# tudocomp/tudocomp

Hardware: AMD Instinct MI355X
Metric: input MB/s end-to-end lcpcomp+huffman (higher is better)
Workload: dtype u32

## Files before the change

include/tdc_gpu.h:

```cpp
#ifndef TDC_GPU_H
#define TDC_GPU_H

#include <stddef.h>
#include <stdint.h>

#ifdef __cplusplus
extern "C" {
#endif

typedef enum {
    TDC_GPU_OK = 0,
    TDC_GPU_ERR_HIP = -1,
    TDC_GPU_ERR_ARG = -2,
    TDC_GPU_ERR_NO_SENTINEL = -3,
    TDC_GPU_ERR_TOO_LARGE = -4,
    TDC_GPU_ERR_OOM = -5,
    TDC_GPU_ERR_UNSUPPORTED = -6,
    TDC_GPU_ERR_INTERNAL = -7
} tdc_gpu_status;

enum { TDC_GPU_CODER_HUFF = 0, TDC_GPU_CODER_GAMMA = 1, TDC_GPU_CODER_ARITH = 2, TDC_GPU_CODER_ASCII = 3, TDC_GPU_CODER_SLE = 4,
       TDC_GPU_CODER_BIT = 5 , TDC_GPU_CODER_DELTA = 6  };
#define TDC_GPU_CODER_SLE_K(K) (TDC_GPU_CODER_SLE | ((K) << 8))
enum { TDC_GPU_COMP_ARRAYS = 0, TDC_GPU_COMP_PLCPPEAKS = 1, TDC_GPU_COMP_MAXLCP = 2, TDC_GPU_COMP_HEAP = 3 };
// ... 45 lines not shown
    uint32_t rebuilds;
    float ms_round_first, ms_round_last, ms_round_tie;
    float reserved1;
} tdc_gpu_stats;

int  tdc_gpu_ctx_create(int device, tdc_gpu_ctx** ctx);
void tdc_gpu_ctx_destroy(tdc_gpu_ctx* ctx);
int tdc_gpu_ctx_set_option(tdc_gpu_ctx* ctx, const char* name, long value);
int tdc_gpu_option_count(void);
const char* tdc_gpu_option_name(int i);
int  tdc_gpu_ctx_reserve(tdc_gpu_ctx* ctx, size_t n);
size_t tdc_gpu_arena_bytes(size_t n);
int  tdc_gpu_device_memory(int device, size_t* free_bytes, size_t* total_bytes);
int  tdc_gpu_ctx_set_profiling(tdc_gpu_ctx* ctx, int enabled);
void tdc_gpu_ctx_reset_profile(tdc_gpu_ctx* ctx);
const char* tdc_gpu_ctx_kernel_profile(const tdc_gpu_ctx* ctx, int idx, double* ms, uint64_t* launches, uint64_t* bytes);
const char* tdc_gpu_strerror(int status);
const char* tdc_gpu_last_error(const tdc_gpu_ctx* ctx);
void tdc_gpu_free(void* p);

int tdc_gpu_lcpcomp_compress(tdc_gpu_ctx* ctx, const uint8_t* text, size_t n, uint32_t threshold, int flatten,
                             int coder, uint8_t** out, size_t* out_len, tdc_gpu_stats* stats);
int tdc_gpu_lcpcomp_compress_comp(tdc_gpu_ctx* ctx, const uint8_t* text, size_t n, uint32_t threshold, int flatten, int coder,
                                  int comp, uint8_t** out, size_t* out_len, tdc_gpu_stats* stats);

int tdc_gpu_lcpcomp_compress_into(tdc_gpu_ctx* ctx, const uint8_t* text, size_t n, uint32_t threshold, int flatten, int coder,
                                  int comp, uint8_t* out, size_t out_cap, size_t* out_len, tdc_gpu_stats* stats);
int tdc_gpu_lcpcomp_compress_keep(tdc_gpu_ctx* ctx, const uint8_t* text, size_t n, uint32_t threshold, int flatten, int coder,
                                  int comp, size_t* out_len, tdc_gpu_stats* stats);
int tdc_gpu_stream_fetch(tdc_gpu_ctx* ctx, uint8_t* dst, size_t cap, size_t* len);
int tdc_gpu_stream_fetch_dev(tdc_gpu_ctx* ctx, void* d_dst, size_t cap, size_t* len);
int tdc_gpu_host_register(void* p, size_t bytes);
int tdc_gpu_host_unregister(void* p);
void* tdc_gpu_host_alloc(size_t bytes);
void  tdc_gpu_host_free(void* p);

int tdc_gpu_lcpcomp_compress_raw(tdc_gpu_ctx* ctx, const uint8_t* data, size_t n, uint32_t threshold, int flatten,
                                 int coder, uint8_t** out, size_t* out_len, tdc_gpu_stats* stats);
int tdc_gpu_lcpcomp_compress_dev(tdc_gpu_ctx* ctx, const void* d_text, size_t n, uint32_t threshold, int flatten,
                                 int coder, void* d_out, size_t out_cap, size_t* out_len, tdc_gpu_stats* stats);
size_t tdc_gpu_lcpcomp_bound(size_t n);
size_t tdc_gpu_lcpcomp_bound_coder(size_t n, int coder);

size_t tdc_gpu_blocks_count(size_t n, size_t block_size);
int tdc_gpu_blocks_compress(const int* devices, int ndev, const uint8_t* data, size_t n, size_t block_size, uint32_t threshold,
                            int flatten, int coder, uint8_t** out, size_t* out_len, tdc_gpu_stats* per_block);
int tdc_gpu_blocks_decompress(tdc_gpu_ctx* ctx, const uint8_t* container, size_t len, int coder, uint8_t** out, size_t* out_len);
int tdc_gpu_device_count(void);

int tdc_gpu_lz78_compress(tdc_gpu_ctx* ctx, const uint8_t* in, size_t n, int coder, uint8_t** out, size_t* out_len,
                          tdc_gpu_stats* stats);

int tdc_gpu_lzss_lcp_compress(tdc_gpu_ctx* ctx, const uint8_t* text, size_t n, uint32_t threshold, int coder,
                              uint8_t** out, size_t* out_len, tdc_gpu_stats* stats);
int tdc_gpu_lzss_lcp_compress_into(tdc_gpu_ctx* ctx, const uint8_t* text, size_t n, uint32_t threshold, int coder,
                                   uint8_t* out, size_t out_cap, size_t* out_len, tdc_gpu_stats* stats);
size_t tdc_gpu_lzss_lcp_bound(size_t n, int coder);
int tdc_gpu_lzss_lcp_decompress(tdc_gpu_ctx* ctx, const uint8_t* stream, size_t len, int coder, uint8_t** out, size_t* out_len,
                                uint64_t* factors, uint32_t* rounds);
int tdc_gpu_lzss_lcp_decompress_into(tdc_gpu_ctx* ctx, const uint8_t* stream, size_t len, int coder, uint8_t* out, size_t out_cap,
                                     size_t* out_len, uint64_t* factors, uint32_t* rounds);
int tdc_gpu_lzss_lcp_factorize(tdc_gpu_ctx* ctx, const uint8_t* text, size_t n, uint32_t threshold,
                               uint32_t** pos, uint32_t** src, uint32_t** len, size_t* z);

int tdc_gpu_sort_pairs_u64(tdc_gpu_ctx* ctx, uint64_t* keys, uint32_t* vals, size_t n, int algo);
int tdc_gpu_suffix_array(tdc_gpu_ctx* ctx, const uint8_t* text, size_t n, uint32_t* sa, uint32_t* isa);
int tdc_gpu_textds(tdc_gpu_ctx* ctx, const uint8_t* text, size_t n, uint32_t* sa, uint32_t* isa, uint32_t* phi,
                   uint32_t* plcp, uint32_t* lcp, uint32_t* maxlcp);
int tdc_gpu_lcpcomp_factorize(tdc_gpu_ctx* ctx, const uint8_t* text, size_t n, uint32_t threshold, int flatten,
                              uint32_t** pos, uint32_t** src, uint32_t** len, size_t* z, tdc_gpu_stats* stats);
int tdc_gpu_flatten(tdc_gpu_ctx* ctx, size_t n, const uint32_t* pos, uint32_t* src, const uint32_t* len, size_t z,
                    uint64_t* num_flattened, uint64_t* max_depth_lb);
int tdc_gpu_prim_scan(tdc_gpu_ctx* ctx, int op, void* data, size_t n, int in_place, void* total);
int tdc_gpu_prim_sort_pairs(tdc_gpu_ctx* ctx, int kind, void* keys, uint32_t* vals, size_t n, int begin_bit, int end_bit);
int tdc_gpu_prim_bucketed_scatter(tdc_gpu_ctx* ctx, const uint32_t* idx, const uint32_t* val, size_t m, uint32_t* dst, size_t n_dst,
                                  uint32_t fill, int permutation, int second_tmp, int offset);
int tdc_gpu_prim_msd_partition(tdc_gpu_ctx* ctx, uint32_t* idx, uint32_t* val, size_t m, int bits, int db);
int tdc_gpu_prim_select(tdc_gpu_ctx* ctx, const uint8_t* cls, uint8_t want, size_t m, const uint32_t* srcA, const uint64_t* srcB,
                        uint32_t fillA, uint64_t fillB, uint32_t* outA, uint64_t* outB, uint32_t* count);
int tdc_gpu_prim_select_counts(tdc_gpu_ctx* ctx, const uint8_t* cls, uint8_t want, size_t m, const uint32_t* srcA, const uint32_t* tile_counts,
                               uint32_t fillA, uint32_t* outA, uint32_t* count);
int tdc_gpu_prim_mark_orbit(tdc_gpu_ctx* ctx, const uint32_t* next, size_t n, uint8_t* mark);
int tdc_gpu_prim_tile_entries(tdc_gpu_ctx* ctx, const uint16_t* exit0, size_t ntiles, uint32_t states, uint16_t* entry0);
int tdc_gpu_prim_arena_fill(tdc_gpu_ctx* ctx, int byte, uint64_t* base, uint64_t* size);

int tdc_gpu_lcpcomp_decompress(tdc_gpu_ctx* ctx, const uint8_t* stream, size_t len, uint8_t** out, size_t* out_len,
                               uint64_t* factors, uint32_t* rounds);
int tdc_gpu_lcpcomp_decompress_coder(tdc_gpu_ctx* ctx, const uint8_t* stream, size_t len, int coder, uint8_t** out, size_t* out_len,
                                     uint64_t* factors, uint32_t* rounds);
int tdc_gpu_lcpcomp_decompress_into(tdc_gpu_ctx* ctx, const uint8_t* stream, size_t len, int coder, uint8_t* out, size_t out_cap,
                                    size_t* out_len, uint64_t* factors, uint32_t* rounds);
int tdc_gpu_ctx_last_decode_on_device(const tdc_gpu_ctx* ctx);

int tdc_gpu_lz78_decompress(tdc_gpu_ctx* ctx, const uint8_t* stream, size_t len, int coder, uint8_t** out, size_t* out_len,
                            uint64_t* phrases, uint32_t* rounds);
int tdc_gpu_lz78_decompress_into(tdc_gpu_ctx* ctx, const uint8_t* stream, size_t len, int coder, uint8_t* out, size_t out_cap,
                                 size_t* out_len, uint64_t* phrases, uint32_t* rounds);

int tdc_gpu_lzw_compress(tdc_gpu_ctx* ctx, const uint8_t* in, size_t n, int coder, uint8_t** out, size_t* out_len,
                         tdc_gpu_stats* stats);
int tdc_gpu_lzw_decompress(tdc_gpu_ctx* ctx, const uint8_t* stream, size_t len, int coder, uint8_t** out, size_t* out_len,
                           uint64_t* codes, uint32_t* rounds);
int tdc_gpu_lzw_decompress_into(tdc_gpu_ctx* ctx, const uint8_t* stream, size_t len, int coder, uint8_t* out, size_t out_cap,
                                size_t* out_len, uint64_t* codes, uint32_t* rounds);

int tdc_gpu_lzss_sw_compress(tdc_gpu_ctx* ctx, const uint8_t* in, size_t n, uint32_t window, uint32_t threshold, int coder,
                             uint8_t** out, size_t* out_len, tdc_gpu_stats* stats);
int tdc_gpu_lzss_sw_compress_into(tdc_gpu_ctx* ctx, const uint8_t* in, size_t n, uint32_t window, uint32_t threshold, int coder,
                                  uint8_t* out, size_t out_cap, size_t* out_len, tdc_gpu_stats* stats);
size_t tdc_gpu_lzss_sw_bound(size_t n, uint32_t window, int coder);
int tdc_gpu_lzss_sw_factorize(tdc_gpu_ctx* ctx, const uint8_t* in, size_t n, uint32_t window, uint32_t threshold,
                              uint32_t** pos, uint32_t** src, uint32_t** len, size_t* z);
int tdc_gpu_lzss_sw_decompress(tdc_gpu_ctx* ctx, const uint8_t* stream, size_t len, int coder, uint32_t window,
                               uint8_t** out, size_t* out_len, uint64_t* factors, uint32_t* rounds);
int tdc_gpu_lzss_sw_decompress_into(tdc_gpu_ctx* ctx, const uint8_t* stream, size_t len, int coder, uint32_t window,
                                    uint8_t* out, size_t out_cap, size_t* out_len, uint64_t* factors, uint32_t* rounds);

int tdc_gpu_lzss_sw_compress_batch(tdc_gpu_ctx* ctx, const uint8_t* in, const uint64_t* in_off, size_t count,
                                   uint32_t window, uint32_t threshold, int coder,
                                   uint8_t* out, size_t out_cap, uint64_t* out_off , uint64_t* out_len ,
                                   int32_t* status , tdc_gpu_stats* stats);
size_t tdc_gpu_lzss_sw_batch_bound(const uint64_t* in_off, size_t count, uint32_t window, int coder);
int tdc_gpu_lzss_sw_decompress_batch(tdc_gpu_ctx* ctx, const uint8_t* streams, const uint64_t* s_off, const uint64_t* s_len,
                                     size_t count, int coder, uint32_t window,
                                     uint8_t* out, size_t out_cap, uint64_t* out_off ,
                                     int32_t* status , tdc_gpu_stats* stats);

int tdc_gpu_lzw_compress_batch(tdc_gpu_ctx* ctx, const uint8_t* in, const uint64_t* in_off, size_t count, int coder,
                               uint8_t* out, size_t out_cap, uint64_t* out_off , uint64_t* out_len ,
                               int32_t* status , tdc_gpu_stats* stats);
int tdc_gpu_lz78_compress_batch(tdc_gpu_ctx* ctx, const uint8_t* in, const uint64_t* in_off, size_t count, int coder,
                                uint8_t* out, size_t out_cap, uint64_t* out_off , uint64_t* out_len ,
                                int32_t* status , tdc_gpu_stats* stats);
size_t tdc_gpu_lzw_batch_bound(const uint64_t* in_off, size_t count, int coder);
size_t tdc_gpu_lz78_batch_bound(const uint64_t* in_off, size_t count, int coder);
int tdc_gpu_lz_parse_batch(tdc_gpu_ctx* ctx, const uint8_t* in, const uint64_t* in_off, size_t count, int lzw,
                           uint32_t* items , uint8_t* chars , uint64_t* item_off , int32_t* status );

int tdc_gpu_lzw_decompress_batch(tdc_gpu_ctx* ctx, const uint8_t* streams, const uint64_t* s_off, const uint64_t* s_len,
                                 size_t count, int coder, uint8_t* out, size_t out_cap, uint64_t* out_off ,
                                 int32_t* status , tdc_gpu_stats* stats);
int tdc_gpu_lz78_decompress_batch(tdc_gpu_ctx* ctx, const uint8_t* streams, const uint64_t* s_off, const uint64_t* s_len,
                                  size_t count, int coder, uint8_t* out, size_t out_cap, uint64_t* out_off ,
                                  int32_t* status , tdc_gpu_stats* stats);

int tdc_gpu_repair_compress(tdc_gpu_ctx* ctx, const uint8_t* in, size_t n, uint64_t max_rules, int coder, uint8_t** out, size_t* out_len,
                            tdc_gpu_stats* stats);
int tdc_gpu_repair_compress_into(tdc_gpu_ctx* ctx, const uint8_t* in, size_t n, uint64_t max_rules, int coder, uint8_t* out, size_t out_cap,
                                 size_t* out_len, tdc_gpu_stats* stats);
size_t tdc_gpu_repair_bound(size_t n, int coder);
int tdc_gpu_repair_grammar(tdc_gpu_ctx* ctx, const uint8_t* in, size_t n, uint64_t max_rules, uint64_t** rules, size_t* nrules,
                           uint32_t** start, size_t* nstart, tdc_gpu_stats* stats);
int tdc_gpu_repair_compress_batch(tdc_gpu_ctx* ctx, const uint8_t* in, const uint64_t* in_off, size_t count, uint64_t max_rules, int coder,
                                  uint8_t* out, size_t out_cap, uint64_t* out_off , uint64_t* out_len ,
                                  int32_t* status , tdc_gpu_stats* stats);
size_t tdc_gpu_repair_batch_bound(const uint64_t* in_off, size_t count, int coder);
int tdc_gpu_repair_grammar_batch(tdc_gpu_ctx* ctx, const uint8_t* in, const uint64_t* in_off, size_t count, uint64_t max_rules,
                                 uint64_t* rules , uint64_t* rule_off ,
                                 uint32_t* start , uint64_t* start_off , int32_t* status );

int tdc_gpu_repair_decompress(tdc_gpu_ctx* ctx, const uint8_t* stream, size_t len, int coder, uint8_t** out, size_t* out_len);
int tdc_gpu_repair_decompress_into(tdc_gpu_ctx* ctx, const uint8_t* stream, size_t len, int coder, uint8_t* out, size_t out_cap, size_t* out_len);
int tdc_gpu_repair_decompress_stats(tdc_gpu_ctx* ctx, const uint8_t* stream, size_t len, int coder, uint8_t* out, size_t out_cap, size_t* out_len,
                                    tdc_gpu_stats* stats);
int tdc_gpu_repair_decompress_batch(tdc_gpu_ctx* ctx, const uint8_t* streams, const uint64_t* s_off, const uint64_t* s_len,
                                    size_t count, int coder, uint8_t* out, size_t out_cap, uint64_t* out_off ,
// ... 77 lines not shown
```

tudocomp_amd/__init__.py:

```python
import ctypes

import numpy as np

from . import _native
from ._native import Stats, Stage, LIB_PATH, SYMBOLS

CODER_HUFF = 0
CODER_GAMMA = 1
CODER_ARITH = 2
CODER_ASCII = 3
CODER_SLE = 4
CODER_BIT = 5
CODER_DELTA = 6
COMP_ARRAYS = 0
COMP_PLCPPEAKS = 1
COMP_MAXLCP = 2
COMP_HEAP = 3
STAGE_BWT = 0
STAGE_RLE = 1
STAGE_MTF = 2
STAGE_HUFF = 3
STAGE_SLE = 4


# ... 786 lines not shown
        v = np.ascontiguousarray(vals, dtype=np.uint32).copy()
        self._check(self._L.tdc_gpu_sort_pairs_u64(self._h, _ptr(k), _ptr(v), len(k), int(algo)))
        return k, v

    _SCAN_OPS = {"sum_u32": (0, np.uint32), "sum_u64": (1, np.uint64), "max_u32": (2, np.uint32)}
    _SORT_KINDS = {"u32": (0, np.uint32), "u64": (1, np.uint64), "distinct": (2, np.uint64)}

    def prim_scan(self, op, data, in_place=False, want_total=True):
        code, dt = self._SCAN_OPS[op]
        a = np.ascontiguousarray(data, dtype=dt).copy()
        tot = np.zeros(1, dtype=dt) if want_total and code != 2 else None
        self._check(self._L.tdc_gpu_prim_scan(self._h, code, _ptr(a), len(a), int(bool(in_place)), _ptr(tot) if tot is not None else None))
        return a, (int(tot[0]) if tot is not None else None)

    def prim_sort_pairs(self, kind, keys, vals, begin_bit, end_bit):
        code, dt = self._SORT_KINDS[kind]
        k = np.ascontiguousarray(keys, dtype=dt).copy()
        v = np.ascontiguousarray(vals, dtype=np.uint32).copy()
        if len(k) != len(v):
            raise ValueError("keys and vals differ in length")
        self._check(self._L.tdc_gpu_prim_sort_pairs(self._h, code, _ptr(k), _ptr(v), len(k), int(begin_bit), int(end_bit)))
        return k, v

    def prim_bucketed_scatter(self, idx, val, n_dst, fill=0xFFFFFFFF, permutation=False, second_tmp=True, offset=0):
        i = np.ascontiguousarray(idx, dtype=np.uint32)
        v = np.ascontiguousarray(val, dtype=np.uint32)
        if len(i) != len(v):
            raise ValueError("idx and val differ in length")
        dst = np.empty(int(n_dst), dtype=np.uint32)
        self._check(self._L.tdc_gpu_prim_bucketed_scatter(self._h, _ptr(i), _ptr(v), len(i), _ptr(dst), int(n_dst), int(fill),
                                                          int(bool(permutation)), int(bool(second_tmp)), int(offset)))
        return dst

    def prim_msd_partition(self, idx, val, bits, db):
        i = np.ascontiguousarray(idx, dtype=np.uint32).copy()
        v = np.ascontiguousarray(val, dtype=np.uint32).copy()
        if len(i) != len(v):
            raise ValueError("idx and val differ in length")
        self._check(self._L.tdc_gpu_prim_msd_partition(self._h, _ptr(i), _ptr(v), len(i), int(bits), int(db)))
        return i, v

    def prim_select(self, cls, want, src_a=None, src_b=None, fill_a=0xFFFFFFFF, fill_b=0xFFFFFFFFFFFFFFFF):
        c = np.ascontiguousarray(cls, dtype=np.uint8)
        m = len(c)
        a = None if src_a is None else np.ascontiguousarray(src_a, dtype=np.uint32)
        b = None if src_b is None else np.ascontiguousarray(src_b, dtype=np.uint64)
        if (a is not None and len(a) != m) or (b is not None and len(b) != m):
            raise ValueError("cls, src_a and src_b differ in length")
        oa = np.empty(m, dtype=np.uint32)
        ob = None if b is None else np.empty(m, dtype=np.uint64)
        cnt = ctypes.c_uint32(0)
        self._check(self._L.tdc_gpu_prim_select(self._h, _ptr(c), int(want), m, None if a is None else _ptr(a), None if b is None else _ptr(b),
                                                int(fill_a), int(fill_b), _ptr(oa), None if ob is None else _ptr(ob), ctypes.byref(cnt)))
        return oa, ob, cnt.value

    def prim_select_counts(self, cls, want, tile_counts, src_a=None, fill_a=0xFFFFFFFF):
        c = np.ascontiguousarray(cls, dtype=np.uint8)
        m = len(c)
        t = np.ascontiguousarray(tile_counts, dtype=np.uint32)
        if len(t) != (m + 2047) // 2048:
            raise ValueError("one count per tile of 2048 classes")
        a = None if src_a is None else np.ascontiguousarray(src_a, dtype=np.uint32)
        if a is not None and len(a) != m:
            raise ValueError("cls and src_a differ in length")
        oa = np.empty(m, dtype=np.uint32)
        cnt = ctypes.c_uint32(0)
        self._check(self._L.tdc_gpu_prim_select_counts(self._h, _ptr(c), int(want), m, None if a is None else _ptr(a), _ptr(t),
                                                       int(fill_a), _ptr(oa), ctypes.byref(cnt)))
        return oa, cnt.value

    def prim_mark_orbit(self, nxt):
        a = np.ascontiguousarray(nxt, dtype=np.uint32)
        mark = np.empty(len(a), dtype=np.uint8)
        self._check(self._L.tdc_gpu_prim_mark_orbit(self._h, _ptr(a), len(a), _ptr(mark)))
        return mark

    def prim_tile_entries(self, exits):
        a = np.ascontiguousarray(exits, dtype=np.uint16)
        ntiles, states = a.shape
        entry = np.empty(ntiles, dtype=np.uint16)
        self._check(self._L.tdc_gpu_prim_tile_entries(self._h, _ptr(a), ntiles, states, _ptr(entry)))
        return entry

    def prim_arena_fill(self, byte=None):
        base, size = ctypes.c_uint64(), ctypes.c_uint64()
        self._check(self._L.tdc_gpu_prim_arena_fill(self._h, -1 if byte is None else int(byte), ctypes.byref(base), ctypes.byref(size)))
        return base.value, size.value

    def suffix_array(self, text):
        a = _u8(text)
        sa = np.empty(len(a), dtype=np.uint32)
        isa = np.empty(len(a), dtype=np.uint32)
        self._check(self._L.tdc_gpu_suffix_array(self._h, _ptr(a), len(a), _ptr(sa), _ptr(isa)))
        return sa, isa

    def textds(self, text):
        a = _u8(text)
        n = len(a)
        arrs = {k: np.empty(n, dtype=np.uint32) for k in ("sa", "isa", "phi", "plcp", "lcp")}
        m = ctypes.c_uint32()
        self._check(self._L.tdc_gpu_textds(self._h, _ptr(a), n, _ptr(arrs["sa"]), _ptr(arrs["isa"]), _ptr(arrs["phi"]),
                                           _ptr(arrs["plcp"]), _ptr(arrs["lcp"]), ctypes.byref(m)))
        arrs["maxlcp"] = m.value
        return arrs

    def lcpcomp_decompress(self, stream, coder=CODER_HUFF):
        a = _u8(stream)
        p, n = ctypes.c_void_p(), ctypes.c_size_t()
        f, r = ctypes.c_uint64(), ctypes.c_uint32()
        self._check(self._L.tdc_gpu_lcpcomp_decompress_coder(self._h, _ptr(a), len(a), coder, ctypes.byref(p), ctypes.byref(n),
                                                             ctypes.byref(f), ctypes.byref(r)))
        return self._take(p, n.value), {"factors": f.value, "rounds": r.value,
                                        "device_parse": int(self._L.tdc_gpu_ctx_last_decode_on_device(self._h))}

    def lcpcomp_decompress_into(self, stream, out, coder=CODER_HUFF):
        a = stream.a if isinstance(stream, PinnedBuffer) else _u8(stream)
        oa = out.a if isinstance(out, PinnedBuffer) else out
        n = ctypes.c_size_t()
        f, r = ctypes.c_uint64(), ctypes.c_uint32()
        self._check(self._L.tdc_gpu_lcpcomp_decompress_into(self._h, _ptr(a), len(a), coder, _ptr(oa), oa.size, ctypes.byref(n),
                                                            ctypes.byref(f), ctypes.byref(r)))
        return n.value, {"factors": f.value, "rounds": r.value, "device_parse": int(self._L.tdc_gpu_ctx_last_decode_on_device(self._h))}

    def lz78_decompress(self, stream, coder=CODER_GAMMA):
        a = stream.a if isinstance(stream, PinnedBuffer) else _u8(stream)
        p, n = ctypes.c_void_p(), ctypes.c_size_t()
        f, r = ctypes.c_uint64(), ctypes.c_uint32()
        self._check(self._L.tdc_gpu_lz78_decompress(self._h, _ptr(a), len(a), coder, ctypes.byref(p), ctypes.byref(n),
                                                    ctypes.byref(f), ctypes.byref(r)))
        return self._take(p, n.value), {"phrases": f.value, "rounds": r.value}

    def lz78_decompress_into(self, stream, out, coder=CODER_GAMMA):
        a = stream.a if isinstance(stream, PinnedBuffer) else _u8(stream)
        oa = out.a if isinstance(out, PinnedBuffer) else out
        n = ctypes.c_size_t()
        f, r = ctypes.c_uint64(), ctypes.c_uint32()
        rc = self._L.tdc_gpu_lz78_decompress_into(self._h, _ptr(a), len(a), coder, _ptr(oa), oa.size, ctypes.byref(n),
                                                  ctypes.byref(f), ctypes.byref(r))
        if rc:
            err = TdcGpuError(rc, self._L.tdc_gpu_last_error(self._h).decode())
            err.required = n.value if rc == -5 else None
            raise err
        return n.value, {"phrases": f.value, "rounds": r.value}

    def lzw_decompress(self, stream, coder=CODER_BIT):
        a = stream.a if isinstance(stream, PinnedBuffer) else _u8(stream)
        p, n = ctypes.c_void_p(), ctypes.c_size_t()
        f, r = ctypes.c_uint64(), ctypes.c_uint32()
        self._check(self._L.tdc_gpu_lzw_decompress(self._h, _ptr(a) if len(a) else None, len(a), coder, ctypes.byref(p), ctypes.byref(n),
                                                   ctypes.byref(f), ctypes.byref(r)))
        return self._take(p, n.value), {"codes": f.value, "rounds": r.value,
                                        "device_parse": int(self._L.tdc_gpu_ctx_last_decode_on_device(self._h))}

    def lzw_decompress_into(self, stream, out, coder=CODER_BIT):
        a = stream.a if isinstance(stream, PinnedBuffer) else _u8(stream)
        oa = out.a if isinstance(out, PinnedBuffer) else out
        n = ctypes.c_size_t()
        f, r = ctypes.c_uint64(), ctypes.c_uint32()
        rc = self._L.tdc_gpu_lzw_decompress_into(self._h, _ptr(a) if len(a) else None, len(a), coder, _ptr(oa), oa.size, ctypes.byref(n),
                                                 ctypes.byref(f), ctypes.byref(r))
        if rc:
            self._raise_required(rc, n.value)
        return n.value, {"codes": f.value, "rounds": r.value, "device_parse": int(self._L.tdc_gpu_ctx_last_decode_on_device(self._h))}

    def _raise_required(self, rc, n):
        err = TdcGpuError(rc, self._L.tdc_gpu_last_error(self._h).decode())
# ... 517 lines not shown
```

tudocomp_amd/_native.py:

```python
import ctypes
import os

_HERE = os.path.dirname(os.path.abspath(__file__))
LIB_PATH = os.environ.get("TDC_GPU_LIB") or os.path.join(_HERE, "lib", "libtdc_gpu.so")

SYMBOLS = [
    "tdc_gpu_ctx_create", "tdc_gpu_ctx_destroy", "tdc_gpu_ctx_reserve", "tdc_gpu_strerror", "tdc_gpu_last_error",
    "tdc_gpu_ctx_set_profiling", "tdc_gpu_ctx_reset_profile", "tdc_gpu_ctx_kernel_profile",
    "tdc_gpu_free", "tdc_gpu_lcpcomp_compress", "tdc_gpu_lcpcomp_compress_raw", "tdc_gpu_lcpcomp_compress_dev",
    "tdc_gpu_lcpcomp_bound", "tdc_gpu_lcpcomp_bound_coder", "tdc_gpu_lcpcomp_compress_into", "tdc_gpu_host_alloc", "tdc_gpu_host_free",
    "tdc_gpu_lz78_compress", "tdc_gpu_lzss_lcp_compress", "tdc_gpu_lzss_lcp_factorize",
    "tdc_gpu_sort_pairs_u64", "tdc_gpu_suffix_array", "tdc_gpu_textds", "tdc_gpu_lcpcomp_factorize", "tdc_gpu_flatten", "tdc_gpu_encode_huff",
    "tdc_gpu_prim_scan", "tdc_gpu_prim_sort_pairs", "tdc_gpu_prim_bucketed_scatter", "tdc_gpu_prim_msd_partition", "tdc_gpu_prim_select", "tdc_gpu_prim_select_counts",
    "tdc_gpu_prim_mark_orbit", "tdc_gpu_prim_tile_entries", "tdc_gpu_prim_arena_fill",
    "tdc_gpu_lcpcomp_decompress",
    "tdc_gpu_lcpcomp_compress_comp",
    "tdc_gpu_encode_arith",
    "tdc_gpu_encode_ascii",
    "tdc_gpu_encode_sle",
    "tdc_gpu_lcpcomp_decompress_coder", "tdc_gpu_ctx_last_decode_on_device", "tdc_gpu_lcpcomp_decompress_into",
    "tdc_gpu_ctx_set_option", "tdc_gpu_option_count", "tdc_gpu_option_name", "tdc_escape", "tdc_unescape", "tdc_lz78_factors", "tdc_huffman_table", "tdc_huffman_selfcheck", "tdc_gpu_blocks_count", "tdc_gpu_blocks_compress", "tdc_gpu_blocks_decompress", "tdc_gpu_device_count", "tdc_gen_english", "tdc_gen_dna",
    "tdc_gpu_arena_bytes", "tdc_gpu_device_memory",
    "tdc_gpu_lcpcomp_compress_keep", "tdc_gpu_stream_fetch", "tdc_gpu_stream_fetch_dev", "tdc_gpu_host_register", "tdc_gpu_host_unregister",
    "tdc_gpu_lz78_decompress", "tdc_gpu_lz78_decompress_into",
    "tdc_gpu_bwt_compress", "tdc_gpu_bwt_compress_into", "tdc_gpu_bwt_decompress", "tdc_gpu_bwt_decompress_into", "tdc_gpu_bwt_inverse_stage",
    "tdc_gpu_pipeline_bound", "tdc_gpu_pipeline_compress", "tdc_gpu_pipeline_compress_into", "tdc_gpu_pipeline_compress_batch", "tdc_gpu_pipeline_batch_bound", "tdc_gpu_pipeline_decompress",
    "tdc_gpu_pipeline_decompress_into", "tdc_gpu_pipeline_decompress_stats", "tdc_rle_decode", "tdc_mtf_decode", "tdc_huff_decode_literals", "tdc_sle_decode",
    "tdc_gpu_lzw_compress", "tdc_gpu_lzw_decompress", "tdc_gpu_lzw_decompress_into", "tdc_lzw_factors", "tdc_lzw_decode",
    "tdc_gpu_lzss_lcp_compress_into", "tdc_gpu_lzss_lcp_bound", "tdc_gpu_lzss_lcp_decompress", "tdc_gpu_lzss_lcp_decompress_into", "tdc_lzss_decode",
    "tdc_gpu_lzss_sw_compress", "tdc_gpu_lzss_sw_compress_into", "tdc_gpu_lzss_sw_bound", "tdc_gpu_lzss_sw_factorize", "tdc_lzss_sw_factors",
    "tdc_lzss_sw_decode", "tdc_gpu_lzss_sw_decompress", "tdc_gpu_lzss_sw_decompress_into",
    "tdc_gpu_lzss_sw_compress_batch", "tdc_gpu_lzss_sw_batch_bound", "tdc_gpu_lzss_sw_decompress_batch",
    "tdc_gpu_lzw_compress_batch", "tdc_gpu_lzw_batch_bound", "tdc_gpu_lz78_compress_batch", "tdc_gpu_lz78_batch_bound", "tdc_gpu_lz_parse_batch",
    "tdc_gpu_lzw_decompress_batch", "tdc_gpu_lz78_decompress_batch",
    "tdc_gpu_repair_compress", "tdc_gpu_repair_compress_into", "tdc_gpu_repair_bound", "tdc_gpu_repair_grammar", "tdc_gpu_repair_decompress",
    "tdc_gpu_repair_decompress_into", "tdc_gpu_repair_decompress_stats", "tdc_repair_grammar", "tdc_repair_decode",
    "tdc_gpu_repair_compress_batch", "tdc_gpu_repair_batch_bound", "tdc_gpu_repair_grammar_batch", "tdc_gpu_repair_decompress_batch",
    "tdc_gpu_bwt_compress_batch", "tdc_gpu_bwt_decompress_batch", "tdc_gpu_suffix_array_batch",
]


class Stats(ctypes.Structure):
    _fields_ = (
        [(k, ctypes.c_uint64) for k in ("n", "out_len", "factors", "maxlcp", "entries", "num_flattened", "max_depth_lb",
                                        "flen_min", "flen_max", "fdist_max", "pushes")] +
        [(k, ctypes.c_uint32) for k in ("sa_rounds", "sa_init_syms", "levels", "mis_rounds", "flatten_rounds", "sigma")] +
        [(k, ctypes.c_uint64) for k in ("sa_sorted_elems", "arena_bytes")] +
        [(k, ctypes.c_float) for k in ("ms_h2d", "ms_sa", "ms_phi", "ms_plcp", "ms_factorize", "ms_flatten", "ms_encode",
                                       "ms_d2h", "ms_total")] +
        [(k, ctypes.c_uint32) for k in ("small_levels", "purges", "window_pass", "window_lcut",
                                        "sa_key_words", "sa_text_rounds", "sa_mode", "sa_overlapped", "eager_levels", "eager_phases", "sa_star_chains",
                                        "probes", "max_push_targets")] +
        [("d2h_early", ctypes.c_uint64)] +
        [("pipe_stages", ctypes.c_uint32), ("pipe_dev", ctypes.c_uint32), ("pipe_len", ctypes.c_uint64 * 8), ("pipe_ms", ctypes.c_float * 8),
         ("ranges_early", ctypes.c_uint32), ("len_rounds", ctypes.c_uint32),
         ("rules", ctypes.c_uint64), ("replaced", ctypes.c_uint64), ("tie_rounds", ctypes.c_uint32), ("rebuilds", ctypes.c_uint32),
         ("ms_round_first", ctypes.c_float), ("ms_round_last", ctypes.c_float), ("ms_round_tie", ctypes.c_float), ("reserved1", ctypes.c_float)])

    def as_dict(self):
        d = {k: getattr(self, k) for k, _ in self._fields_}
        d["pipe_len"] = list(self.pipe_len)[:self.pipe_stages]
        d["pipe_ms"] = list(self.pipe_ms)[:self.pipe_stages]
        return d


class Stage(ctypes.Structure):
    _fields_ = [("kind", ctypes.c_int), ("param", ctypes.c_uint64)]


_lib = None


def load():
    global _lib
    if _lib is not None:
        return _lib
    if not os.path.exists(LIB_PATH):
        raise RuntimeError("tudocomp_amd: %s is missing -- build it with `make -C tudocomp_amd/csrc` "
                           "(there is no CPU fallback)" % LIB_PATH)
    L = ctypes.CDLL(LIB_PATH)
    vp, sz, u32, i32 = ctypes.c_void_p, ctypes.c_size_t, ctypes.c_uint32, ctypes.c_int
    pvp, psz = ctypes.POINTER(vp), ctypes.POINTER(sz)
    L.tdc_gpu_ctx_create.argtypes = [i32, pvp]
    L.tdc_gpu_ctx_destroy.argtypes = [vp]
    L.tdc_gpu_ctx_destroy.restype = None
    L.tdc_gpu_ctx_reserve.argtypes = [vp, sz]
    L.tdc_gpu_ctx_set_profiling.argtypes = [vp, i32]
    L.tdc_gpu_ctx_reset_profile.argtypes = [vp]
    L.tdc_gpu_ctx_reset_profile.restype = None
    L.tdc_gpu_ctx_kernel_profile.argtypes = [vp, i32, ctypes.POINTER(ctypes.c_double), ctypes.POINTER(ctypes.c_uint64),
                                             ctypes.POINTER(ctypes.c_uint64)]
    L.tdc_gpu_ctx_kernel_profile.restype = ctypes.c_char_p
    L.tdc_gpu_strerror.argtypes = [i32]
    L.tdc_gpu_strerror.restype = ctypes.c_char_p
    L.tdc_gpu_last_error.argtypes = [vp]
    L.tdc_gpu_last_error.restype = ctypes.c_char_p
    L.tdc_gpu_free.argtypes = [vp]
    L.tdc_gpu_free.restype = None
    L.tdc_gpu_lcpcomp_compress.argtypes = [vp, vp, sz, u32, i32, i32, pvp, psz, ctypes.POINTER(Stats)]
    L.tdc_gpu_lcpcomp_compress_comp.argtypes = [vp, vp, sz, u32, i32, i32, i32, pvp, psz, ctypes.POINTER(Stats)]
    L.tdc_gpu_lcpcomp_compress_raw.argtypes = [vp, vp, sz, u32, i32, i32, pvp, psz, ctypes.POINTER(Stats)]
    L.tdc_gpu_lcpcomp_compress_dev.argtypes = [vp, vp, sz, u32, i32, i32, vp, sz, psz, ctypes.POINTER(Stats)]
    L.tdc_gpu_lz78_compress.argtypes = [vp, vp, sz, i32, pvp, psz, ctypes.POINTER(Stats)]
    L.tdc_gpu_lzss_lcp_compress.argtypes = [vp, vp, sz, u32, i32, pvp, psz, ctypes.POINTER(Stats)]
    L.tdc_gpu_lzss_lcp_compress_into.argtypes = [vp, vp, sz, u32, i32, vp, sz, psz, ctypes.POINTER(Stats)]
    L.tdc_gpu_lzss_lcp_bound.argtypes = [sz, i32]
    L.tdc_gpu_lzss_lcp_bound.restype = sz
    L.tdc_gpu_lzss_lcp_decompress.argtypes = [vp, vp, sz, i32, pvp, psz, ctypes.POINTER(ctypes.c_uint64), ctypes.POINTER(ctypes.c_uint32)]
    L.tdc_gpu_lzss_lcp_decompress_into.argtypes = [vp, vp, sz, i32, vp, sz, psz, ctypes.POINTER(ctypes.c_uint64), ctypes.POINTER(ctypes.c_uint32)]
    L.tdc_lzss_decode.argtypes = [vp, sz, i32, vp, sz, psz]
    L.tdc_gpu_lzss_lcp_factorize.argtypes = [vp, vp, sz, u32, pvp, pvp, pvp, psz]
    L.tdc_gpu_arena_bytes.argtypes = [sz]
    L.tdc_gpu_arena_bytes.restype = sz
    L.tdc_gpu_device_memory.argtypes = [i32, psz, psz]
    L.tdc_gpu_lcpcomp_bound.argtypes = [sz]
    L.tdc_gpu_lcpcomp_bound.restype = sz
    L.tdc_gpu_lcpcomp_bound_coder.argtypes = [sz, i32]
    L.tdc_gpu_lcpcomp_bound_coder.restype = sz
    L.tdc_gpu_lcpcomp_compress_into.argtypes = [vp, vp, sz, u32, i32, i32, i32, vp, sz, psz, ctypes.POINTER(Stats)]
    L.tdc_gpu_lcpcomp_compress_keep.argtypes = [vp, vp, sz, u32, i32, i32, i32, psz, ctypes.POINTER(Stats)]
    L.tdc_gpu_stream_fetch.argtypes = [vp, vp, sz, psz]
    L.tdc_gpu_stream_fetch_dev.argtypes = [vp, vp, sz, psz]
    L.tdc_gpu_ctx_last_decode_on_device.argtypes = [vp]
    L.tdc_gpu_lcpcomp_decompress_into.argtypes = [vp, vp, sz, i32, vp, sz, psz, ctypes.POINTER(ctypes.c_uint64), ctypes.POINTER(ctypes.c_uint32)]
    L.tdc_gpu_host_register.argtypes = [vp, sz]
    L.tdc_gpu_host_unregister.argtypes = [vp]
    L.tdc_gpu_blocks_count.argtypes = [sz, sz]
    L.tdc_gpu_blocks_count.restype = sz
    L.tdc_gpu_blocks_compress.argtypes = [ctypes.POINTER(i32), i32, vp, sz, sz, u32, i32, i32, pvp, psz, ctypes.POINTER(Stats)]
    L.tdc_gpu_blocks_decompress.argtypes = [vp, vp, sz, i32, pvp, psz]
    L.tdc_gpu_host_alloc.argtypes = [sz]
    L.tdc_gpu_host_alloc.restype = vp
    L.tdc_gpu_host_free.argtypes = [vp]
    L.tdc_gpu_host_free.restype = None
    L.tdc_gpu_sort_pairs_u64.argtypes = [vp, vp, vp, sz, i32]
    L.tdc_gpu_prim_scan.argtypes = [vp, i32, vp, sz, i32, vp]
    L.tdc_gpu_prim_sort_pairs.argtypes = [vp, i32, vp, vp, sz, i32, i32]
    L.tdc_gpu_prim_bucketed_scatter.argtypes = [vp, vp, vp, sz, vp, sz, u32, i32, i32, i32]
    L.tdc_gpu_prim_msd_partition.argtypes = [vp, vp, vp, sz, i32, i32]
    L.tdc_gpu_prim_select.argtypes = [vp, vp, ctypes.c_uint8, sz, vp, vp, u32, ctypes.c_uint64, vp, vp, ctypes.POINTER(u32)]
    L.tdc_gpu_prim_select_counts.argtypes = [vp, vp, ctypes.c_uint8, sz, vp, vp, u32, vp, ctypes.POINTER(u32)]
    L.tdc_gpu_prim_mark_orbit.argtypes = [vp, vp, sz, vp]
    L.tdc_gpu_prim_tile_entries.argtypes = [vp, vp, sz, u32, vp]
    L.tdc_gpu_prim_arena_fill.argtypes = [vp, i32, ctypes.POINTER(ctypes.c_uint64), ctypes.POINTER(ctypes.c_uint64)]
    L.tdc_gpu_suffix_array.argtypes = [vp, vp, sz, vp, vp]
    L.tdc_gpu_textds.argtypes = [vp, vp, sz, vp, vp, vp, vp, vp, ctypes.POINTER(u32)]
    L.tdc_gpu_lcpcomp_factorize.argtypes = [vp, vp, sz, u32, i32, pvp, pvp, pvp, psz, ctypes.POINTER(Stats)]
    L.tdc_gpu_flatten.argtypes = [vp, sz, vp, vp, vp, sz, ctypes.POINTER(ctypes.c_uint64), ctypes.POINTER(ctypes.c_uint64)]
    L.tdc_gpu_encode_huff.argtypes = [vp, vp, sz, vp, vp, vp, sz, pvp, psz]
    L.tdc_gpu_lcpcomp_decompress.argtypes = [vp, vp, sz, pvp, psz, ctypes.POINTER(ctypes.c_uint64), ctypes.POINTER(ctypes.c_uint32)]
    L.tdc_gpu_lz78_decompress.argtypes = [vp, vp, sz, i32, pvp, psz, ctypes.POINTER(ctypes.c_uint64), ctypes.POINTER(ctypes.c_uint32)]
    L.tdc_gpu_lz78_decompress_into.argtypes = [vp, vp, sz, i32, vp, sz, psz, ctypes.POINTER(ctypes.c_uint64), ctypes.POINTER(ctypes.c_uint32)]
    L.tdc_gpu_bwt_compress.argtypes = [vp, vp, sz, pvp, psz, ctypes.POINTER(Stats)]
    L.tdc_gpu_bwt_compress_into.argtypes = [vp, vp, sz, vp, sz, psz, ctypes.POINTER(Stats)]
    L.tdc_gpu_bwt_decompress.argtypes = [vp, vp, sz, pvp, psz, ctypes.POINTER(ctypes.c_uint32)]
    L.tdc_gpu_bwt_decompress_into.argtypes = [vp, vp, sz, vp, sz, psz, ctypes.POINTER(ctypes.c_uint32)]
    L.tdc_gpu_bwt_inverse_stage.argtypes = [vp, vp, sz, u32, u32, vp, vp, ctypes.POINTER(ctypes.c_uint64), ctypes.POINTER(ctypes.c_uint32)]
    pst = ctypes.POINTER(Stage)
    L.tdc_gpu_pipeline_bound.argtypes = [pst, i32, sz]
    L.tdc_gpu_pipeline_bound.restype = sz
    L.tdc_gpu_pipeline_compress.argtypes = [vp, pst, i32, vp, sz, pvp, psz, ctypes.POINTER(Stats)]
    L.tdc_gpu_pipeline_compress_into.argtypes = [vp, pst, i32, vp, sz, vp, sz, psz, ctypes.POINTER(Stats)]
    L.tdc_gpu_pipeline_compress_batch.argtypes = [vp, pst, i32, vp, vp, sz, vp, sz, vp, vp, vp, ctypes.POINTER(Stats)]
    L.tdc_gpu_pipeline_batch_bound.argtypes = [pst, i32, vp, sz]
    L.tdc_gpu_pipeline_batch_bound.restype = sz
    L.tdc_gpu_pipeline_decompress.argtypes = [vp, pst, i32, vp, sz, pvp, psz]
    L.tdc_gpu_pipeline_decompress_into.argtypes = [vp, pst, i32, vp, sz, vp, sz, psz]
    L.tdc_gpu_pipeline_decompress_stats.argtypes = [vp, pst, i32, vp, sz, vp, sz, psz, ctypes.POINTER(Stats)]
    L.tdc_rle_decode.argtypes = [vp, sz, ctypes.c_uint64, vp, sz, psz]
    L.tdc_mtf_decode.argtypes = [vp, sz, vp, sz, psz]
    L.tdc_huff_decode_literals.argtypes = [vp, sz, vp, sz, psz]
    L.tdc_sle_decode.argtypes = [vp, sz, ctypes.c_uint32, vp, sz, psz]
    L.tdc_gpu_lcpcomp_decompress_coder.argtypes = [vp, vp, sz, ctypes.c_int, pvp, psz, ctypes.POINTER(ctypes.c_uint64), ctypes.POINTER(ctypes.c_uint32)]
    L.tdc_gpu_encode_arith.argtypes = [vp, vp, sz, vp, vp, vp, sz, pvp, psz]
    L.tdc_gpu_encode_ascii.argtypes = [vp, vp, sz, vp, vp, vp, sz, pvp, psz]
    L.tdc_gpu_encode_sle.argtypes = [vp, vp, sz, vp, vp, vp, sz, ctypes.c_uint32, pvp, psz]
    L.tdc_escape.argtypes = [vp, sz, vp]
    L.tdc_escape.restype = sz
    L.tdc_unescape.argtypes = [vp, sz, vp]
    L.tdc_unescape.restype = sz
    L.tdc_lz78_factors.argtypes = [vp, sz, pvp, pvp, psz]
    L.tdc_lzw_factors.argtypes = [vp, sz, pvp, psz]
    L.tdc_lzw_decode.argtypes = [vp, sz, i32, vp, sz, psz]
    L.tdc_gpu_lzw_compress.argtypes = [vp, vp, sz, i32, pvp, psz, ctypes.POINTER(Stats)]
    L.tdc_gpu_lzw_decompress.argtypes = [vp, vp, sz, i32, pvp, psz, ctypes.POINTER(ctypes.c_uint64), ctypes.POINTER(ctypes.c_uint32)]
    L.tdc_gpu_lzw_decompress_into.argtypes = [vp, vp, sz, i32, vp, sz, psz, ctypes.POINTER(ctypes.c_uint64), ctypes.POINTER(ctypes.c_uint32)]
    L.tdc_gpu_lzss_sw_compress.argtypes = [vp, vp, sz, u32, u32, i32, pvp, psz, ctypes.POINTER(Stats)]
    L.tdc_gpu_lzss_sw_compress_into.argtypes = [vp, vp, sz, u32, u32, i32, vp, sz, psz, ctypes.POINTER(Stats)]
    L.tdc_gpu_lzss_sw_bound.argtypes = [sz, u32, i32]
    L.tdc_gpu_lzss_sw_bound.restype = sz
    L.tdc_gpu_lzss_sw_factorize.argtypes = [vp, vp, sz, u32, u32, pvp, pvp, pvp, psz]
    L.tdc_lzss_sw_factors.argtypes = [vp, sz, u32, u32, pvp, pvp, pvp, psz]
    L.tdc_lzss_sw_decode.argtypes = [vp, sz, i32, u32, vp, sz, psz]
    u64 = ctypes.c_uint64
    L.tdc_gpu_repair_compress.argtypes = [vp, vp, sz, u64, i32, pvp, psz, ctypes.POINTER(Stats)]
    L.tdc_gpu_repair_compress_into.argtypes = [vp, vp, sz, u64, i32, vp, sz, psz, ctypes.POINTER(Stats)]
    L.tdc_gpu_repair_bound.argtypes = [sz, i32]
    L.tdc_gpu_repair_bound.restype = sz
    L.tdc_gpu_repair_grammar.argtypes = [vp, vp, sz, u64, pvp, psz, pvp, psz, ctypes.POINTER(Stats)]
    L.tdc_gpu_repair_decompress.argtypes = [vp, vp, sz, i32, pvp, psz]
    L.tdc_gpu_repair_decompress_into.argtypes = [vp, vp, sz, i32, vp, sz, psz]
    L.tdc_gpu_repair_decompress_stats.argtypes = [vp, vp, sz, i32, vp, sz, psz, ctypes.POINTER(Stats)]
    L.tdc_repair_grammar.argtypes =[vp, sz, u64, pvp, psz, pvp, psz]
    L.tdc_repair_decode.argtypes = [vp, sz, i32, vp, sz, psz]
    L.tdc_gpu_repair_compress_batch.argtypes = [vp, vp, vp, sz, u64, i32, vp, sz, vp, vp, vp, ctypes.POINTER(Stats)]
    L.tdc_gpu_bwt_compress_batch.argtypes = [vp, vp, vp, sz, vp, sz, vp, ctypes.POINTER(Stats)]
    L.tdc_gpu_bwt_decompress_batch.argtypes = [vp, vp, vp, sz, vp, sz, vp, ctypes.POINTER(Stats)]
    L.tdc_gpu_suffix_array_batch.argtypes = [vp, vp, vp, sz, vp, vp]
    L.tdc_gpu_repair_batch_bound.argtypes = [vp, sz, i32]
    L.tdc_gpu_repair_batch_bound.restype = sz
    L.tdc_gpu_repair_grammar_batch.argtypes = [vp, vp, vp, sz, u64, vp, vp, vp, vp, vp]
    L.tdc_gpu_repair_decompress_batch.argtypes = [vp, vp, vp, vp, sz, i32, vp, sz, vp, vp, ctypes.POINTER(Stats)]
    L.tdc_gpu_lzss_sw_decompress.argtypes = [vp, vp, sz, i32, u32, pvp, psz, ctypes.POINTER(ctypes.c_uint64), ctypes.POINTER(ctypes.c_uint32)]
    L.tdc_gpu_lzss_sw_decompress_into.argtypes = [vp, vp, sz, i32, u32, vp, sz, psz, ctypes.POINTER(ctypes.c_uint64), ctypes.POINTER(ctypes.c_uint32)]
    L.tdc_gpu_lzss_sw_compress_batch.argtypes = [vp, vp, vp, sz, u32, u32, i32, vp, sz, vp, vp, vp, ctypes.POINTER(Stats)]
    L.tdc_gpu_lzss_sw_batch_bound.argtypes = [vp, sz, u32, i32]
    L.tdc_gpu_lzss_sw_batch_bound.restype = sz
    L.tdc_gpu_lzss_sw_decompress_batch.argtypes = [vp, vp, vp, vp, sz, i32, u32, vp, sz, vp, vp, ctypes.POINTER(Stats)]
    for name in ("lzw", "lz78"):
        getattr(L, "tdc_gpu_%s_compress_batch" % name).argtypes = [vp, vp, vp, sz, i32, vp, sz, vp, vp, vp, ctypes.POINTER(Stats)]
        getattr(L, "tdc_gpu_%s_batch_bound" % name).argtypes = [vp, sz, i32]
        getattr(L, "tdc_gpu_%s_batch_bound" % name).restype = sz
        getattr(L, "tdc_gpu_%s_decompress_batch" % name).argtypes = [vp, vp, vp, vp, sz, i32, vp, sz, vp, vp, ctypes.POINTER(Stats)]
    L.tdc_gpu_lz_parse_batch.argtypes = [vp, vp, vp, sz, i32, vp, vp, vp, vp]
    L.tdc_gpu_ctx_set_option.argtypes = [vp, ctypes.c_char_p, ctypes.c_long]
    L.tdc_gpu_option_count.argtypes = []
# ... 8 lines not shown
```

tudocomp_amd/csrc/api_prims.hip:

```cpp
#include "api.hpp"
#include "tile_chain.hpp"

#include <algorithm>
#include <vector>

using namespace tdc;

namespace {
[[noreturn]] void bad(const char* msg) { throw ArgError{TDC_GPU_ERR_ARG, msg}; }

void check_count(size_t n) {
    if (n >= 0xFFFFFFFFull) throw ArgError{TDC_GPU_ERR_TOO_LARGE, "at most 2^32 - 2 elements"};
}

template <typename T>
T* upload(Ctx& c, const T* src, size_t n, size_t offset = 0) {
    T* d = c.arena.get<T>(n + offset + 4) + offset;
    if (n) HIP_TRY(hipMemcpyAsync(d, src, n * sizeof(T), hipMemcpyHostToDevice, c.stream));
    return d;
}
template <typename T>
void download(Ctx& c, T* dst, const T* d_src, size_t n) {
    if (n) HIP_TRY(hipMemcpyAsync(dst, d_src, n * sizeof(T), hipMemcpyDeviceToHost, c.stream));
}
// ... 126 lines not shown
        if (m && ((srcB != nullptr) != (outB != nullptr))) bad("srcB and outB go together");
        check_count(m);
        Ctx& c = ctx->c;
        reserve_arena(c, 32 * m + ((size_t)64 << 20));
        const u8* d_cls = upload(c, cls, m);
        const u32* d_a = srcA ? upload(c, srcA, m) : nullptr;
        const u64* d_b = srcB ? upload(c, srcB, m) : nullptr;
        u32* d_oa = c.arena.get<u32>(m + 4);
        u64* d_ob = srcB ? c.arena.get<u64>(m + 4) : nullptr;
        u32* d_count = c.arena.get<u32>(1);
        fill_u32(c, d_oa, m, fillA);
        if (d_ob) {
            std::vector<u64> f(m, fillB);
            if (m) HIP_TRY(hipMemcpyAsync(d_ob, f.data(), m * 8, hipMemcpyHostToDevice, c.stream));
            HIP_TRY(hipStreamSynchronize(c.stream));
        }
        select_by_class(c, d_cls, want, m, d_a, d_oa, d_b, d_ob, d_count);
        download(c, outA, d_oa, m);
        if (d_ob) download(c, outB, d_ob, m);
        download(c, count, d_count, 1);
        HIP_TRY(hipStreamSynchronize(c.stream));
    });
}

int tdc_gpu_prim_select_counts(tdc_gpu_ctx* ctx, const uint8_t* cls, uint8_t want, size_t m, const uint32_t* srcA, const uint32_t* tile_counts,
                               uint32_t fillA, uint32_t* outA, uint32_t* count) {
    return guarded(ctx, [&] {
        if (m && (!cls || !outA || !tile_counts)) bad("cls/outA/tile_counts is NULL");
        if (!count) bad("count is NULL");
        check_count(m);
        const size_t tiles = (m + SEL_TILE_CLASSES - 1) / SEL_TILE_CLASSES;
        for (size_t t = 0; t < tiles; ++t) {
            const size_t e = std::min(m, (t + 1) * SEL_TILE_CLASSES);
            if ((size_t)std::count(cls + t * SEL_TILE_CLASSES, cls + e, want) != tile_counts[t]) bad("tile_counts[t] is not the count of tile t");
        }
        Ctx& c = ctx->c;
        reserve_arena(c, 32 * m + ((size_t)64 << 20));
        const u8* d_cls = upload(c, cls, m);
        const u32* d_a = srcA ? upload(c, srcA, m) : nullptr;
        const u32* d_tc = upload(c, tile_counts, tiles);
        u32* d_oa = c.arena.get<u32>(m + 4);
        u32* d_count = c.arena.get<u32>(1);
        fill_u32(c, d_oa, m, fillA);
        select_by_class(c, d_cls, want, m, d_a, d_oa, nullptr, nullptr, d_count, d_tc);
        download(c, outA, d_oa, m);
        download(c, count, d_count, 1);
        HIP_TRY(hipStreamSynchronize(c.stream));
    });
}

int tdc_gpu_prim_mark_orbit(tdc_gpu_ctx* ctx, const uint32_t* next, size_t n, uint8_t* mark) {
    return guarded(ctx, [&] {
        if (n && (!next || !mark)) bad("next/mark is NULL");
        check_count(n);
        for (size_t i = 0; i < n; ++i) if (next[i] <= i || next[i] > n) bad("i < next[i] <= n required");
        if (n == 0) return;
        Ctx& c = ctx->c;
        reserve_arena(c, 16 * n + ((size_t)64 << 20));
        const u32* d_next = upload(c, next, n);
        u8* d_mark = c.arena.get<u8>(n + 4);
        u32* s1 = c.arena.get<u32>(n + 4); u32* s2 = c.arena.get<u32>(n + 4);
        mark_orbit_u32(c, d_next, n, d_mark, s1, s2);
        download(c, mark, d_mark, n);
        HIP_TRY(hipStreamSynchronize(c.stream));
    });
}

int tdc_gpu_prim_tile_entries(tdc_gpu_ctx* ctx, const uint16_t* exit0, size_t ntiles, uint32_t states, uint16_t* entry0) {
    return guarded(ctx, [&] {
        if (ntiles && (!exit0 || !entry0)) bad("exit0/entry0 is NULL");
        if (states == 0 || states >= DX_NONE) bad("1 <= states < 0xFFFF required");
        if (ntiles > ((size_t)1 << 27)) throw ArgError{TDC_GPU_ERR_TOO_LARGE, "at most 2^27 tiles"};
        for (size_t i = 0; i < ntiles * states; ++i) if (exit0[i] >= states && exit0[i] != DX_NONE) bad("every exit must be < states or 0xFFFF");
        if (ntiles == 0) return;
        Ctx& c = ctx->c;
        reserve_arena(c, 2 * ntiles * states + dx_entries_scratch((u32)ntiles, states) + ((size_t)64 << 20));
        const u16* d_exit = upload(c, exit0, ntiles * states);
        const u16* d_entry = dx_entries(c, d_exit, (u32)ntiles, states, c.arena.alloc(dx_entries_scratch((u32)ntiles, states)));
        download(c, entry0, d_entry, ntiles);
        HIP_TRY(hipStreamSynchronize(c.stream));
    });
}

int tdc_gpu_prim_arena_fill(tdc_gpu_ctx* ctx, int byte, uint64_t* base, uint64_t* size) {
    return guarded(ctx, [&] {
        if (!base || !size) bad("base/size is NULL");
        if (byte > 255) bad("byte must be 0 .. 255, or negative to fill nothing");
        Ctx& c = ctx->c;
        *base = (uint64_t)(uintptr_t)c.arena.base;
        *size = c.arena.base ? (uint64_t)c.arena.size : 0;
        if (byte < 0 || *size == 0) return;
        HIP_TRY(hipMemsetAsync(c.arena.base, byte, c.arena.size, c.stream));
        HIP_TRY(hipStreamSynchronize(c.stream));
    });
}

}
```

tudocomp_amd/csrc/fused.hip:

```cpp
#include "stages.hpp"
#include "prim.hpp"

#include <type_traits>

namespace tdc {

constexpr int FS_TILE = 4096;
constexpr int FS_ITEMS = 16;
constexpr u32 FS_WMAX = 8192;

struct FSLevel {
    const u32* idx_in; const void* rp_in; const u32* prev_in; const u8* lcp_in;
    u32* idx_out; void* rp_out; u8* lcp_out;
    u32* counts; const u32* blk_seg; const u32* blk_start; const u32* seg_start;
    u32 nseg, R, per_xcd; int shift;
    int lsh;
};
__device__ __forceinline__ bool fs_row(const FSLevel& P, u32 row, size_t& base, u32& cnt) {
    const u32 blk = row / P.R;
    if (blk >= P.blk_start[P.nseg]) return false;
    const u32 s = P.blk_seg[blk];
    const u64 t = (u64)(blk - P.blk_start[s]) * P.R + row % P.R;
    const u32 s0 = P.seg_start[s], s1 = P.seg_start[s + 1];
    const u64 off = t * FS_TILE;
// ... 216 lines not shown
                    if (cf.flen8) *(u32*)(cf.flen8 + q) = 0u; else *(uint4*)(cf.flen + q) = make_uint4(0, 0, 0, 0);
                } else {
                    for (u32 j = 0; j < nv; ++j) {
                        cf.cls[q + j] = (u8)(cw >> (8 * j));
                        if (cf.res8) cf.res8[q + j] = (u8)(rw >> (8 * j));
                        if (cf.flen8) cf.flen8[q + j] = 0; else cf.flen[q + j] = 0;
                    }
                }
            }
            if (cf.tilecnt) {
                const u32 wsum = wave_reduce_sum((u32)__popc(cw));
                if (lane_id() == 0 && wsum) atomicAdd(&cf.tilecnt[q / SEL_TILE_CLASSES], wsum);
            }
        }
        ncand = wave_reduce_sum(ncand);
        if (lane_id() == 0) scf[wave_id()] = ncand;
    }
    mx = wave_reduce_max(mx);
    if (lane_id() == 0) smx[wave_id()] = mx;
    __syncthreads();
    if (wave_id() == 0) {
        u32 v = (lane_id() < FS_IMG_T / 64) ? smx[lane_id()] : 0u;
        v = wave_reduce_max(v);
        if (lane_id() == 0 && v) atomicMax(d_max, v);
    }
    if constexpr (CF) {
        u32* acc = cf.acc + (size_t)(blockIdx.x % CF_COPIES) * CF_ACC;
        if (threadIdx.x < 64) { if (shist[threadIdx.x]) atomicAdd(&acc[threadIdx.x], shist[threadIdx.x]); }
        else if (threadIdx.x == 64) { u32 t = 0; for (int i = 0; i < FS_IMG_T / 64; ++i) t += scf[i]; if (t) atomicAdd(&acc[64], t); }
    }
}
__global__ void fs_cand_fold_kernel(const u32* __restrict__ acc, u32* __restrict__ out) {
    if (threadIdx.x > 64) return;
    u32 t = 0;
    for (u32 k = 0; k < CF_COPIES; ++k) t += acc[(size_t)k * CF_ACC + threadIdx.x];
    out[threadIdx.x] = t;
}

__global__ void fs_first_kernel(const u32* __restrict__ sa, size_t n, u32* __restrict__ isa, u32* __restrict__ phi, u32* __restrict__ plcp, FSCand cf) {
    const u32 p = sa[0];
    isa[p] = 0; if (phi) phi[p] = sa[n - 1]; plcp[p] = 0;
    if (cf.cls) {
        cf.cls[p] = 0;
        if (cf.res8) cf.res8[p] = 0;
        if (cf.flen8) cf.flen8[p] = 0; else cf.flen[p] = 0;
    }
}
__global__ void fs_direct_kernel(const u32* __restrict__ sa, const u8* __restrict__ lcp8, size_t n, u32* __restrict__ isa, u32* __restrict__ phi,
                                 u32* __restrict__ plcp, u32* __restrict__ d_max) {
    const size_t i = (size_t)blockIdx.x * blockDim.x + threadIdx.x;
    u32 l = 0;
    if (i < n) {
        const u32 p = sa[i];
        isa[p] = (u32)i;
        if (phi) phi[p] = (i == 0) ? sa[n - 1] : sa[i - 1];
        l = (i == 0) ? 0u : (u32)lcp8[i];
        plcp[p] = l;
    }
    l = wave_reduce_max(l);
    if (lane_id() == 0 && l) atomicMax(d_max, l);
}

bool fused_scatter_has_image(const Ctx& c, size_t n) { return n >= ((size_t)1 << 20) && c.bucket_scatter; }

void build_isa_phi_plcp_fused(Ctx& c, const u32* sa, const u8* lcp8, size_t n, u32* isa, u32* phi, u32* plcp, u32* d_maxlcp, CandFused* cf) {
    hipStream_t s = c.stream;
    if (cf) cf->filled = false;
    HIP_TRY(hipMemsetAsync(d_maxlcp, 0, sizeof(u32), s));
    if (!n) return;
    const int bits = (int)bits_for(n - 1);
    if (!fused_scatter_has_image(c, n)) {
        Ctx::ProfScope prof(c, K_PHI, (u64)n * 17);
        fs_direct_kernel<<<cdiv(n, 256), 256, 0, s>>>(sa, lcp8, n, isa, phi, plcp, d_maxlcp);
        LAUNCH_CHECK();
        return;
    }
    const size_t mark = c.arena.mark();
    const size_t m = n - 1;
    const int db = (bits - 16 > 13) ? 9 : 8;
    const u32 D = 1u << db;
    u32* idx[2] = { c.arena.get<u32>(m), c.arena.get<u32>(m) };
    const bool wp = phi != nullptr;
    void* rp[2] = { c.arena.alloc(m * (wp ? 8 : 4)), c.arena.alloc(m * (wp ? 8 : 4)) };
    const u32* seg_start = ss_first_segment(c, m);
    u32 nseg = 1;
    for (int l = 0; l < 2; ++l) {
        u32* nstart = c.arena.get<u32>((size_t)nseg * D + 1);
        const size_t lm = c.arena.mark();
        SegTables Tb;
        ss_level_tables(c, seg_start, nseg, m, D, Tb);
        FSLevel P;
        if (l == 0) { P.idx_in = sa + 1; P.rp_in = nullptr; P.prev_in = sa; P.lcp_in = lcp8 + 1; }
        else { P.idx_in = idx[0]; P.rp_in = rp[0]; P.prev_in = nullptr; P.lcp_in = nullptr; }
        P.idx_out = idx[l]; P.rp_out = rp[l]; P.lcp_out = nullptr;
        P.lsh = bits - db;
        P.counts = Tb.counts; P.blk_seg = Tb.blk_seg; P.blk_start = Tb.blk_start; P.seg_start = seg_start;
        P.nseg = nseg; P.R = Tb.R; P.shift = bits - db * (l + 1);
        const u32 rows = Tb.rows;
        P.per_xcd = (c.xcd_remap == 1 && rows >= 64) ? cdiv(rows, 8) : 0u;
        const u32 grid = P.per_xcd ? 8 * P.per_xcd : rows;
        {
            const int pc = c.prof_begin(K_RS_COUNT, (u64)m * 4);
            if (db == 9) fs_count_kernel<9><<<grid, 256, 0, s>>>(P, rows); else fs_count_kernel<8><<<grid, 256, 0, s>>>(P, rows);
            LAUNCH_CHECK();
            c.prof_end(pc);
        }
        ss_level_offsets(c, Tb, seg_start, nseg, D, nstart, m);
        {
            const int ps = c.prof_begin(K_RS_SCATTER_U32, (u64)m * (wp ? (l == 0 ? 5 + 12 : 24) : (l == 0 ? 5 + 8 : 16)));
            const bool pair = (Tb.R % 2) == 0 && c.fs_pair;
            FSLevel P2 = P;
            const u32 groups = pair ? (rows + 1) / 2 : rows;
            P2.per_xcd = (c.xcd_remap == 1 && groups >= 64) ? cdiv(groups, 8) : 0u;
            const u32 grid2 = P2.per_xcd ? 8 * P2.per_xcd : groups;
            auto launch = [&](auto wpc) {
                constexpr bool WPC = decltype(wpc)::value;
                if (pair) {
                    if (l == 0) { if (db == 9) fs_scatter_kernel<9, true, 2, WPC><<<grid2, 512, 0, s>>>(P2, rows); else fs_scatter_kernel<8, true, 2, WPC><<<grid2, 512, 0, s>>>(P2, rows); }
                    else { if (db == 9) fs_scatter_kernel<9, false, 2, WPC><<<grid2, 512, 0, s>>>(P2, rows); else fs_scatter_kernel<8, false, 2, WPC><<<grid2, 512, 0, s>>>(P2, rows); }
                } else {
                    if (l == 0) { if (db == 9) fs_scatter_kernel<9, true, 1, WPC><<<grid, 256, 0, s>>>(P, rows); else fs_scatter_kernel<8, true, 1, WPC><<<grid, 256, 0, s>>>(P, rows); }
                    else { if (db == 9) fs_scatter_kernel<9, false, 1, WPC><<<grid, 256, 0, s>>>(P, rows); else fs_scatter_kernel<8, false, 1, WPC><<<grid, 256, 0, s>>>(P, rows); }
                }
            };
            if (wp) launch(std::true_type{}); else launch(std::false_type{});
            LAUNCH_CHECK();
            c.prof_end(ps);
        }
        c.arena.release(lm);
        seg_start = nstart;
        nseg *= D;
    }
    {
        const u32 W = 1u << (bits - 2 * db);
        if (W > FS_WMAX) throw HipError{hipErrorUnknown, "fused scatter: window larger than the LDS image", (int)__LINE__};
        if (W < 16) throw HipError{hipErrorUnknown, "fused scatter: window smaller than a thread's group of positions", (int)__LINE__};
        FSCand fc{};
        if (cf) {
            if (!cf->cls || !cf->acc || !cf->lvlhist || (!cf->flen8 && !cf->flen) || (cf->lcut && !cf->res8))
                throw HipError{hipErrorUnknown, "fused scatter: candidate arrays missing", (int)__LINE__};
            fc.threshold = cf->threshold; fc.lcut = cf->lcut;
            fc.cls = cf->cls; fc.res8 = cf->lcut ? cf->res8 : nullptr; fc.flen8 = cf->flen8; fc.flen = cf->flen; fc.tilecnt = cf->tilecnt; fc.acc = cf->acc;
            HIP_TRY(hipMemsetAsync(cf->acc, 0, (size_t)CF_COPIES * CF_ACC * sizeof(u32), s));
            if (cf->tilecnt) HIP_TRY(hipMemsetAsync(cf->tilecnt, 0, (size_t)cdiv(n, SEL_TILE_CLASSES) * sizeof(u32), s));
        }
        Ctx::ProfScope prof(c, K_FS_IMAGE, (u64)m * (wp ? 24 : 16) + (cf ? (u64)m * ((cf->lcut ? 2 : 1) + (cf->flen8 ? 1 : 4)) : 0));
        if (cf) {
            if (wp) fs_image_kernel<true, true><<<cdiv(m, W), FS_IMG_T, 0, s>>>(idx[1], rp[1], bits - db, m, W, isa, phi, plcp, d_maxlcp, fc);
            else fs_image_kernel<false, true><<<cdiv(m, W), FS_IMG_T, 0, s>>>(idx[1], rp[1], bits - db, m, W, isa, phi, plcp, d_maxlcp, fc);
        } else {
            if (wp) fs_image_kernel<true, false><<<cdiv(m, W), FS_IMG_T, 0, s>>>(idx[1], rp[1], bits - db, m, W, isa, phi, plcp, d_maxlcp, fc);
            else fs_image_kernel<false, false><<<cdiv(m, W), FS_IMG_T, 0, s>>>(idx[1], rp[1], bits - db, m, W, isa, phi, plcp, d_maxlcp, fc);
        }
        LAUNCH_CHECK();
        fs_first_kernel<<<1, 1, 0, s>>>(sa, n, isa, phi, plcp, fc);
        LAUNCH_CHECK();
        if (cf) {
            fs_cand_fold_kernel<<<1, 128, 0, s>>>(cf->acc, cf->lvlhist);
            LAUNCH_CHECK();
            cf->filled = true;
        }
    }
    c.arena.release(mark);
}

}
```

tudocomp_amd/csrc/prim.hpp:

```cpp
#pragma once
#include "common.hpp"

namespace tdc {

void exclusive_sum_u32(Ctx& c, const u32* in, u32* out, size_t n, u32* d_total);
void exclusive_sum_u64(Ctx& c, const u64* in, u64* out, size_t n, u64* d_total);
void inclusive_max_u32(Ctx& c, const u32* in, u32* out, size_t n);

int radix_sort_pairs_u64(Ctx& c, u64* keys[2], u32* vals[2], size_t n, int begin_bit, int end_bit);
int radix_sort_pairs_u32(Ctx& c, u32* keys[2], u32* vals[2], size_t n, int begin_bit, int end_bit);

struct TextKeyGen { const u8* text; size_t n; u32 sigma; int k, chunk; u64 top ; u8 code[256]; };
int radix_sort_text_keys_u64(Ctx& c, const TextKeyGen& g, u64* keys[2], u32* vals[2], int end_bit);

struct SplitSortStats { u32 levels = 0, range_leaves = 0, samples = 0, units = 0, large_leaves = 0, wide_units = 0; u64 large_pairs = 0; };
bool splitter_sort_applicable(size_t n);
int splitter_sort_pairs_u64(Ctx& c, u64* keys[2], u32* vals[2], size_t n, const TextKeyGen* gen, SplitSortStats* st);

void msd_partition_pairs_u32(Ctx& c, const u32* idx, const u32* val, size_t m, int bits, int db, u32* out_idx, u32* out_val, u32* tmp_idx, u32* tmp_val);

struct SegTables { u32* blk_start; u32* blk_seg; u32* counts; u32* bs; u32 R, blocks_ub, rows; };
struct UnitTables { u32* unit_rng; u32* cls_list; u32* large; u32 cap, large_cap; u32 hc[6];  int wide_classes = 0;  u32 whc[16] = {0, 0, 0, 0, 0, 0, 0, 0, 0, 0, 0, 0, 0, 0, 0, 0};  };
constexpr int WIDE_NCLS = 10;
__host__ __device__ inline u32 wide_class(u32 m) {
    if (m <= 2048u) return m <= 1024u ? 0u : (m - 769u) / 256u;
    if (m <= 4096u) return 5u + (m <= 2560u ? 0u : (m - 2049u) / 512u);
    return 9u;
}
u32* ss_first_segment(Ctx& c, size_t n);
void ss_level_tables(Ctx& c, const u32* seg_start, u32 nseg, size_t n, u32 D, SegTables& T);
void ss_level_offsets(Ctx& c, const SegTables& T, const u32* seg_start, u32 nseg, u32 D, u32* nstart, size_t n);
void ss_level_offsets_sub(Ctx& c, const SegTables& T, u32 nsub, const u32* blk_super, const u32* out_start, u32 nsuper, u32 D, u32* nstart, size_t n);
void ss_build_units(Ctx& c, const u32* leaf_start, u32 nleaf, UnitTables& U, u32 small = 0);
void ss_fanouts(Ctx& c, size_t n, int& L, u32 F[3], u32& os, u32 leaf3 = 0, int wide2 = 0);

struct WKeyGen { const u8* text; size_t n; int b, s, pad; u32 inv ; u8 code[256]; };
struct WSortStats { u32 levels = 0, range_leaves = 0, samples = 0, units = 0, large_leaves = 0, kw = 0, refined_units = 0, trunc_units = 0, longrun_units = 0, leaf_stages = 0, wave_runs = 0; u64 large_pairs = 0; u64 nonheads = 0; };
struct WPre {
    bool begun = false, active = false;
    const u8* text = nullptr; size_t n = 0;
    int KW = 0; WKeyGen g;
    int L = 0; u32 F[3] = { 1, 1, 1 }; u32 os = 0, NLr = 0, NS = 0, S = 0;
    u64* K1[2] = { nullptr, nullptr }; u64* K2[2] = { nullptr, nullptr }; u32* V[2] = { nullptr, nullptr };
    u16* digits = nullptr; u64* sp1 = nullptr; u64* sp2 = nullptr;
    u32 nchunks = 0; size_t chunk_off[33] = {};
    u32* nstart_all = nullptr;
    const u32* dig2_counts[32] = {}; const u32* dig2_blk[32] = {}; u32 dig2_R[32] = {};
    bool dig2 = false; u32 dig2_chunks = 0;
    u32 present[8] = { 0, 0, 0, 0, 0, 0, 0, 0 };
};
bool wsort_pre_begin(Ctx& c, WPre& P, const u8* text, size_t n, const size_t* chunk_off, u32 nchunks, const u32* hist0);
void wsort_pre_chunk(Ctx& c, WPre& P, u32 q);
void wsort_pre_finish(Ctx& c, WPre& P, const u32* hist_full);
bool wsort_applicable(const Ctx& c, size_t n);
void wsort_make_keygen(const Ctx& c, const u8* text, size_t n, u32 sigma, const u8* code, int& KW, WKeyGen& g);
int wsort_result_index(Ctx& c, size_t n);
int wsort_suffixes(Ctx& c, int KW, const WKeyGen& g, u64* K1[2], u64* K2[2], u32* V[2], size_t n, u8* flags, u8* lcp8, WSortStats* st);
void wsort_suffixes_pre(Ctx& c, const WPre& P, u32* v_final, u8* flags, u8* lcp8, WSortStats* st);
int wsort_records(Ctx& c, u64* K1[2], u64* K2[2], u32* V[2], size_t m, int k1_bits, WSortStats* st);
bool wsort_sorted_runs(Ctx& c, const u64* k1, u64* k2, u32* v, size_t m, int k1_bits);
bool wsort_sorted_runs_from_text(Ctx& c, const u32* a_sa, const u32* a_r1, size_t m, const WKeyGen& g, u32 h, u64* k1, u64* k2, u32* v, int k1_bits);

int sort_pairs_u64_distinct(Ctx& c, u64* keys[2], u32* vals[2], size_t n, int begin_bit, int end_bit);

void bucketed_scatter_u32(Ctx& c, const u32* idx, const u32* val, size_t m, u32* dst, size_t n_dst, u32* tmp_idx, u32* tmp_val,
                          u32* tmp_idx2, u32* tmp_val2, bool permutation = false);

constexpr size_t SEL_TILE_CLASSES = 2048;
void select_by_class(Ctx& c, const u8* cls, u8 want, size_t m, const u32* srcA, u32* outA, const u64* srcB, u64* outB,
                     u32* d_count, const u32* tile_counts = nullptr);

void mark_orbit_u32(Ctx& c, const u32* next, size_t n, u8* mark, u32* scratch1, u32* scratch2);

void fill_u32(Ctx& c, u32* p, size_t n, u32 v);
void fill_u8(Ctx& c, u8* p, size_t n, u8 v);

}
```

tudocomp_amd/csrc/ssort.hip:

```cpp
#include "prim.hpp"

#include <vector>

namespace tdc {

constexpr int SS_TILE = 4096;
constexpr int SS_ITEMS = 16;
constexpr int SS_SMALL = 4096;
constexpr int SS_UNIT_MAX = 8192;
constexpr int SS_GEN_HALO = 32;

struct SSLevel {
    const u64* keys_in; const u32* vals_in;
    u64* keys_out; u32* vals_out;
    u32* counts;
    const u32* blk_seg;
    const u32* blk_start;
    const u32* seg_start;
    const u64* sp;
    u16* digits;
    u32 nseg, F, stride, R, D, per_xcd;
};

__device__ __forceinline__ bool ss_row(const SSLevel& P, u32 row, u32& s, size_t& base, u32& cnt) {
// ... 29 lines not shown
    if (LAST) return 2 * lo + (spl[lo] == x ? 1u : 0u);
    return lo;
}

__device__ __forceinline__ void ss_gen_stage(const TextKeyGen& g, size_t t0, const u8* __restrict__ code, u8* __restrict__ sy) {
    const size_t p = t0 + (size_t)threadIdx.x * 16;
    u8 b[16];
    if (p + 16 <= g.n && (((size_t)g.text) & 15) == 0) {
        const uint4 v = *(const uint4*)(g.text + p);
        const u32 wv[4] = { v.x, v.y, v.z, v.w };
#pragma unroll
        for (int i = 0; i < 16; ++i) b[i] = (u8)(wv[i >> 2] >> (8 * (i & 3)));
    } else {
#pragma unroll
        for (int i = 0; i < 16; ++i) b[i] = (p + i < g.n) ? g.text[p + i] : (u8)0;
    }
    u32 o[4] = { 0, 0, 0, 0 };
#pragma unroll
    for (int i = 0; i < 16; ++i) o[i >> 2] |= (u32)((p + i < g.n) ? code[b[i]] : (u8)0) << (8 * (i & 3));
    *(uint4*)(sy + (size_t)threadIdx.x * 16) = make_uint4(o[0], o[1], o[2], o[3]);
    if (threadIdx.x < SS_GEN_HALO) {
        const size_t q = t0 + SS_TILE + threadIdx.x;
        sy[SS_TILE + threadIdx.x] = (q < g.n) ? code[g.text[q]] : (u8)0;
    }
}
__device__ __forceinline__ u64 ss_gen_key(const TextKeyGen& g, const u8* sy, int lb) {
    u64 key = 0;
    for (int j0 = 0; j0 < g.k; j0 += g.chunk) {
        const int len = (g.k - j0 < g.chunk) ? g.k - j0 : g.chunk;
        u32 acc = 0, scale = 1;
        for (int t = 0; t < len; ++t) { acc = acc * g.sigma + sy[lb + j0 + t]; scale *= g.sigma; }
        key = (j0 == 0) ? (u64)acc : key * scale + acc;
    }
    return key;
}

__device__ __forceinline__ size_t ss_sample_pos(u32 i, size_t n) {
    const u64 h = ((u64)i + 1) * 0x9E3779B97F4A7C15ull;
    return (size_t)(((unsigned __int128)(h ^ (h >> 29)) * n) >> 64);
}
template <bool GEN>
__global__ __launch_bounds__(256) void ss_sample_kernel(const u64* __restrict__ keys, TextKeyGen g, size_t n, u32 S, u64* __restrict__ out,
                                                        u32* __restrict__ dummy) {
    __shared__ u8 code[256];
    if (GEN) { code[threadIdx.x] = g.code[threadIdx.x]; __syncthreads(); }
    const u32 i = blockIdx.x * 256 + threadIdx.x;
    if (i >= S) return;
    const size_t p = ss_sample_pos(i, n);
    u64 key;
    if (GEN) {
        key = 0;
        for (int j0 = 0; j0 < g.k; j0 += g.chunk) {
            const int len = (g.k - j0 < g.chunk) ? g.k - j0 : g.chunk;
            u32 acc = 0, scale = 1;
            for (int t = 0; t < len; ++t) {
                const size_t q = p + j0 + t;
                acc = acc * g.sigma + ((q < n) ? code[g.text[q]] : 0u);
                scale *= g.sigma;
            }
            key = (j0 == 0) ? (u64)acc : key * scale + acc;
        }
    } else key = keys[p];
    out[i] = key;
    dummy[i] = i;
}
__global__ void ss_pick_kernel(const u64* __restrict__ sorted, u32 NS, u32 os, u64* __restrict__ sp) {
    const u32 i = blockIdx.x * blockDim.x + threadIdx.x;
    if (i < NS) sp[i] = sorted[(size_t)(i + 1) * os - 1];
    else if (i == NS) sp[i] = ~0ull;
}

__global__ void ss_nblk_kernel(const u32* __restrict__ seg_start, u32 nseg, u32 R, u32* __restrict__ nblk) {
    const u32 s = blockIdx.x * blockDim.x + threadIdx.x;
    if (s > nseg) return;
    if (s == nseg) { nblk[s] = 0; return; }
    const u64 size = seg_start[s + 1] - seg_start[s];
    nblk[s] = (u32)((size + (u64)SS_TILE * R - 1) / ((u64)SS_TILE * R));
}
__global__ void ss_blkseg_kernel(const u32* __restrict__ blk_start, u32 nseg, u32* __restrict__ blk_seg) {
    const u32 s = blockIdx.x * blockDim.x + threadIdx.x;
    if (s >= nseg) return;
    for (u32 b = blk_start[s]; b < blk_start[s + 1]; ++b) blk_seg[b] = s;
}

template <bool GEN, bool LAST>
__global__ __launch_bounds__(256) void ss_count_kernel(SSLevel P, TextKeyGen g, u32 rows) {
    __shared__ u32 hist[512];
    __shared__ u64 spl[256];
    __shared__ u8 code[256];
    __shared__ __align__(16) u8 sy[GEN ? SS_TILE + SS_GEN_HALO : 16];
    const u32 row = xcd_tile(blockIdx.x, P.per_xcd);
    if (row >= rows) return;
    u32 s, cnt; size_t base;
    if (!ss_row(P, row, s, base, cnt)) return;
    for (u32 i = threadIdx.x; i < P.D; i += 256) hist[i] = 0;
    if (cnt == 0) {
        for (u32 i = threadIdx.x; i < P.D; i += 256) P.counts[(size_t)row * P.D + i] = 0;
        return;
    }
    ss_load_splitters<LAST>(P, s, spl);
    if (GEN) code[threadIdx.x] = g.code[threadIdx.x];
    __syncthreads();
    if (GEN) { ss_gen_stage(g, base, code, sy); __syncthreads(); }
    if (GEN) {
        const int lb = wave_id() * (64 * SS_ITEMS) + lane_id() * SS_ITEMS;
        u64 key = ss_gen_key(g, sy, lb);
        u32 pk[SS_ITEMS / 2];
#pragma unroll
        for (int j = 0; j < SS_ITEMS; ++j) {
            const bool valid = (u32)(lb + j) < cnt;
            const u32 d = valid ? ss_digit<LAST>(spl, key) : 0u;
            key = (key - (u64)sy[lb + j] * g.top) * g.sigma + sy[lb + j + g.k];
            pk[j >> 1] = (j & 1) ? (pk[j >> 1] | (d << 16)) : d;
            const u32 d0 = __builtin_amdgcn_readfirstlane(d);
            if (__all(valid && d == d0)) { if (lane_id() == 0) atomicAdd(&hist[d0], 64u); }
            else if (valid) atomicAdd(&hist[d], 1u);
        }
        uint4* dp = (uint4*)(P.digits + base + lb);
        dp[0] = make_uint4(pk[0], pk[1], pk[2], pk[3]);
        dp[1] = make_uint4(pk[4], pk[5], pk[6], pk[7]);
    } else {
        const u32 lb = wave_id() * (64 * SS_ITEMS) + lane_id();
        const u64* kp = P.keys_in + base + lb;
        u16* dgp = P.digits + base + lb;
        u64 kk[SS_ITEMS];
#pragma unroll
        for (int j = 0; j < SS_ITEMS; ++j) kk[j] = (lb + (u32)j * 64 < cnt) ? kp[j * 64] : 0ull;
#pragma unroll 4
        for (int j = 0; j < SS_ITEMS; ++j) {
            const u32 e = lb + (u32)j * 64;
            const bool valid = e < cnt;
            const u32 d = valid ? ss_digit<LAST>(spl, kk[j]) : 0u;
            if (valid) dgp[j * 64] = (u16)d;
            const u32 d0 = __builtin_amdgcn_readfirstlane(d);
            if (__all(valid && d == d0)) { if (lane_id() == 0) atomicAdd(&hist[d0], 64u); }
            else if (valid) atomicAdd(&hist[d], 1u);
        }
    }
    __syncthreads();
    for (u32 i = threadIdx.x; i < P.D; i += 256) P.counts[(size_t)row * P.D + i] = hist[i];
}

__global__ __launch_bounds__(256) void ss_blocksum_kernel(const u32* __restrict__ counts, const u32* __restrict__ blk_start, u32 nseg,
                                                          u32 R, u32 D, u32* __restrict__ bs) {
    const u32 b = blockIdx.x;
    if (b >= blk_start[nseg]) return;
    for (u32 d = threadIdx.x; d < D; d += 256) {
        u32 acc = 0;
        for (u32 r = 0; r < R; ++r) acc += counts[((size_t)b * R + r) * D + d];
        bs[(size_t)b * D + d] = acc;
    }
}
__global__ __launch_bounds__(1024) void ss_segbase_kernel(u32* __restrict__ bs, const u32* __restrict__ blk_start, const u32* __restrict__ seg_start,
                                                          u32 D, u32* __restrict__ next_start) {
    __shared__ u32 part[4][2048];
    __shared__ u32 dstart[2048];
    __shared__ u32 wsum[16];
    const u32 s = blockIdx.x;
    const u32 b0 = blk_start[s], b1 = blk_start[s + 1];
    const u32 t = threadIdx.x & 255u, g = threadIdx.x >> 8;
    const u32 nb = b1 - b0, per = (nb + 3) / 4;
    const u32 lo = b0 + (g * per < nb ? g * per : nb);
    const u32 hi = (lo + per < b1) ? lo + per : b1;
    for (u32 d = t; d < D; d += 256) {
        u32 acc = 0;
        u32 b = lo;
        for (; b + 8 <= hi; b += 8) {
            u32 v[8];
#pragma unroll
            for (int i = 0; i < 8; ++i) v[i] = bs[(size_t)(b + i) * D + d];
#pragma unroll
            for (int i = 0; i < 8; ++i) acc += v[i];
        }
        for (; b < hi; ++b) acc += bs[(size_t)b * D + d];
        part[g][d] = acc;
    }
    __syncthreads();
    const u32 d0 = 2 * threadIdx.x, d1 = d0 + 1;
    const u32 tot0 = d0 < D ? part[0][d0] + part[1][d0] + part[2][d0] + part[3][d0] : 0u;
    const u32 tot1 = d1 < D ? part[0][d1] + part[1][d1] + part[2][d1] + part[3][d1] : 0u;
    const u32 tot = tot0 + tot1;
    u32 inc = wave_inclusive_sum(tot);
    if (lane_id() == 63) wsum[wave_id()] = inc;
    __syncthreads();
    {
        u32 run = 0;
        for (int w = 0; w < wave_id(); ++w) run += wsum[w];
        const u32 st = seg_start[s] + run + inc - tot;
        if (d0 < D) { dstart[d0] = st; next_start[(size_t)s * D + d0] = st; }
        if (d1 < D) { dstart[d1] = st + tot0; next_start[(size_t)s * D + d1] = st + tot0; }
    }
    __syncthreads();
    for (u32 d = t; d < D; d += 256) {
        u32 run = dstart[d];
        for (u32 k = 0; k < g; ++k) run += part[k][d];
        u32 b = lo;
        for (; b + 8 <= hi; b += 8) {
            u32 v[8];
#pragma unroll
            for (int i = 0; i < 8; ++i) v[i] = bs[(size_t)(b + i) * D + d];
#pragma unroll
            for (int i = 0; i < 8; ++i) { bs[(size_t)(b + i) * D + d] = run; run += v[i]; }
        }
        for (; b < hi; ++b) { const u32 v = bs[(size_t)b * D + d]; bs[(size_t)b * D + d] = run; run += v; }
    }
}
__global__ __launch_bounds__(256) void ss_apply_kernel(u32* __restrict__ counts, const u32* __restrict__ blk_start, u32 nseg, u32 R, u32 D,
                                                       const u32* __restrict__ bs) {
    const u32 b = blockIdx.x;
    if (b >= blk_start[nseg]) return;
    for (u32 d = threadIdx.x; d < D; d += 256) {
        u32 run = bs[(size_t)b * D + d];
        for (u32 r = 0; r < R; ++r) {
            const size_t i = ((size_t)b * R + r) * D + d;
            const u32 v = counts[i];
            counts[i] = run;
            run += v;
        }
    }
}
__global__ void ss_set_word_kernel(u32* p, u32 v) { *p = v; }

template <bool GEN, bool LAST>
__global__ __launch_bounds__(256) __attribute__((amdgpu_waves_per_eu(4, 4))) void ss_scatter_kernel(SSLevel P, TextKeyGen g, u32 rows) {
    constexpr int DMAX = LAST ? 512 : 256;
    __shared__ u32 tcnt[DMAX];
    __shared__ u32 gbase[DMAX];
    __shared__ __align__(16) u64 stage[SS_TILE];
    __shared__ u32 scan_sm[5];
    __shared__ u8 code[GEN ? 256 : 4];
    const int lane = lane_id(), w = wave_id();
    const u32 row = xcd_tile(blockIdx.x, P.per_xcd);
    if (row >= rows) return;
    u32 s, cnt; size_t base;
    if (!ss_row(P, row, s, base, cnt) || cnt == 0) return;
    u8* sy = (u8*)stage;
    u16* stage_d = (u16*)(stage + 2048);
    u32* stage32 = (u32*)stage;
    for (int i = threadIdx.x; i < DMAX; i += 256) tcnt[i] = 0;
    if (GEN) code[threadIdx.x] = g.code[threadIdx.x];
    __syncthreads();
    if (GEN) { ss_gen_stage(g, base, code, sy); __syncthreads(); }

    u64 k[SS_ITEMS];
    u32 v[SS_ITEMS];
    u32 ld[SS_ITEMS];
    const u32 lbs = GEN ? (u32)(w * (64 * SS_ITEMS) + lane * SS_ITEMS) : (u32)(w * (64 * SS_ITEMS) + lane);
    u64 gkey = 0;
    u32 pk[SS_ITEMS / 2];
    if (GEN) {
        gkey = ss_gen_key(g, sy, (int)lbs);
        const uint4* dp = (const uint4*)(P.digits + base + lbs);
        const uint4 q0 = dp[0], q1 = dp[1];
        pk[0] = q0.x; pk[1] = q0.y; pk[2] = q0.z; pk[3] = q0.w; pk[4] = q1.x; pk[5] = q1.y; pk[6] = q1.z; pk[7] = q1.w;
    }
    const u64* kp = GEN ? nullptr : P.keys_in + base + lbs;
    const u32* vp = GEN ? nullptr : P.vals_in + base + lbs;
    const u16* dgp = P.digits + base + lbs;
#pragma unroll
    for (int j = 0; j < SS_ITEMS; ++j) {
        const u32 e = GEN ? lbs + (u32)j : lbs + (u32)j * 64;
        const bool valid = e < cnt;
        if (GEN) {
            k[j] = gkey; v[j] = (u32)(base + e);
            gkey = (gkey - (u64)sy[lbs + j] * g.top) * g.sigma + sy[lbs + j + g.k];
            ld[j] = (pk[j >> 1] >> (16 * (j & 1))) & 0xFFFFu;
        } else {
            k[j] = valid ? kp[j * 64] : 0ull;
            v[j] = valid ? vp[j * 64] : 0u;
            ld[j] = valid ? (u32)dgp[j * 64] : 0u;
        }
    }
#pragma unroll
    for (int j = 0; j < SS_ITEMS; ++j) {
        const u32 e = GEN ? lbs + (u32)j : lbs + (u32)j * 64;
        const bool valid = e < cnt;
        const u32 d = valid ? ld[j] : 0u;
        u32 rank = 0;
        {
            u64 rem = __ballot(valid);
            bool done = !valid;
#pragma unroll
            for (int it = 0; it < 2; ++it) {
                if (!rem) break;
                const int lead = __ffsll((long long)rem) - 1;
                const u32 dl = __shfl(d, lead, 64);
                const u64 grp = __ballot(!done && d == dl);
                const u32 c = (u32)__popcll(grp);
                if (c < 8) break;
                u32 b0 = 0;
                if (lane == lead) b0 = atomicAdd(&tcnt[dl], c);
                b0 = __shfl(b0, lead, 64);
                if ((grp >> lane) & 1ull) { rank = b0 + (u32)__popcll(grp & ((1ull << lane) - 1)); done = true; }
                rem &= ~grp;
            }
            if (!done) rank = atomicAdd(&tcnt[d], 1u);
        }
        ld[j] = (d << 16) | rank;
    }
    __syncthreads();
    {
        const u32 t = threadIdx.x;
        u32 tot[DMAX / 256], sum = 0;
#pragma unroll
// ... 210 lines not shown
        else if (valid) atomicAdd(&hist[d], 1u);
    }
    __syncthreads();
    for (u32 i = threadIdx.x; i < D; i += 256) P.counts[(size_t)row * D + i] = hist[i];
}
template <int DB>
__global__ __launch_bounds__(256) __attribute__((amdgpu_waves_per_eu(4, 4))) void ps_scatter_kernel(PSLevel P, u32 rows) {
    constexpr u32 D = 1u << DB;
    __shared__ u32 tcnt[D];
    __shared__ u32 gbase[D];
    __shared__ u32 stage_i[SS_TILE];
    __shared__ u32 stage_v[SS_TILE];
    __shared__ u32 scan_sm[5];
    const int lane = lane_id();
    const u32 row = xcd_tile(blockIdx.x, P.per_xcd);
    if (row >= rows) return;
    size_t base; u32 cnt;
    if (!ps_row(P, row, base, cnt) || cnt == 0) return;
    for (u32 i = threadIdx.x; i < D; i += 256) tcnt[i] = 0;
    __syncthreads();
    const u32 lb = wave_id() * (64 * SS_ITEMS) + lane;
    const u32* ip = P.idx_in + base + lb;
    const u32* vp = P.val_in + base + lb;
    u32 k[SS_ITEMS], v[SS_ITEMS], ld[SS_ITEMS];
#pragma unroll
    for (int j = 0; j < SS_ITEMS; ++j) {
        const bool valid = lb + (u32)j * 64 < cnt;
        k[j] = valid ? ip[j * 64] : 0u;
        v[j] = valid ? vp[j * 64] : 0u;
    }
#pragma unroll
    for (int j = 0; j < SS_ITEMS; ++j) {
        const bool valid = lb + (u32)j * 64 < cnt;
        const u32 d = (k[j] >> P.shift) & (D - 1);
        const u32 d0 = __builtin_amdgcn_readfirstlane(d);
        u32 rank = 0;
        if (__all(valid && d == d0)) {
            if (lane == 0) rank = atomicAdd(&tcnt[d0], 64u);
            rank = __builtin_amdgcn_readfirstlane(rank) + (u32)lane;
        } else if (valid) rank = atomicAdd(&tcnt[d], 1u);
        ld[j] = rank;
    }
    __syncthreads();
    {
        const u32 t = threadIdx.x;
        u32 tot[D / 256], sum = 0;
#pragma unroll
        for (u32 q = 0; q < D / 256; ++q) { tot[q] = tcnt[t * (D / 256) + q]; sum += tot[q]; }
        u32 total;
        u32 start = block_exclusive_sum<u32, 4>(sum, scan_sm, total);
#pragma unroll
        for (u32 q = 0; q < D / 256; ++q) {
            const u32 d = t * (D / 256) + q;
            tcnt[d] = start;
            gbase[d] = P.counts[(size_t)row * D + d] - start;
            start += tot[q];
        }
    }
    __syncthreads();
#pragma unroll
    for (int j = 0; j < SS_ITEMS; ++j) {
        if (lb + (u32)j * 64 < cnt) {
            const u32 pos = ld[j] + tcnt[(k[j] >> P.shift) & (D - 1)];
            stage_i[pos] = k[j]; stage_v[pos] = v[j];
        }
    }
    __syncthreads();
#pragma unroll
    for (int r = 0; r < SS_ITEMS; ++r) {
        const u32 sp = (u32)r * 256 + threadIdx.x;
        if (sp < cnt) {
            const u32 key = stage_i[sp];
            const u32 dst = gbase[(key >> P.shift) & (D - 1)] + sp;
            P.idx_out[dst] = key;
            P.val_out[dst] = stage_v[sp];
        }
    }
}

void msd_partition_pairs_u32(Ctx& c, const u32* idx, const u32* val, size_t m, int bits, int db, u32* out_idx, u32* out_val, u32* tmp_idx, u32* tmp_val) {
    hipStream_t s = c.stream;
    const size_t mark = c.arena.mark();
    const u32 D = 1u << db;
    u32* seg_start = c.arena.get<u32>(2);
    ss_set_word_kernel<<<1, 1, 0, s>>>(seg_start, 0u);
    LAUNCH_CHECK();
    ss_set_word_kernel<<<1, 1, 0, s>>>(seg_start + 1, (u32)m);
    LAUNCH_CHECK();
    u32 nseg = 1;
    const u64 tiles = (m + SS_TILE - 1) / SS_TILE;
    for (int l = 0; l < 2; ++l) {
        u32 R = 128;
        while (R > 1 && (u64)nseg * R > tiles / 8 + 64) R >>= 1;
        const u32 blocks_ub = (u32)((tiles + R - 1) / R) + nseg;
        const u32 rows = blocks_ub * R;
        u32* nstart = c.arena.get<u32>((size_t)nseg * D + 1);
        const size_t lm = c.arena.mark();
        u32* blk_start = c.arena.get<u32>((size_t)nseg + 1);
        u32* blk_seg = c.arena.get<u32>(blocks_ub);
        u32* counts = c.arena.get<u32>((size_t)rows * D);
        u32* bs = c.arena.get<u32>((size_t)blocks_ub * D);
        ss_nblk_kernel<<<cdiv((size_t)nseg + 1, 256), 256, 0, s>>>(seg_start, nseg, R, blk_start);
        LAUNCH_CHECK();
        exclusive_sum_u32(c, blk_start, blk_start, (size_t)nseg + 1, nullptr);
        ss_blkseg_kernel<<<cdiv(nseg, 256), 256, 0, s>>>(blk_start, nseg, blk_seg);
        LAUNCH_CHECK();
        PSLevel P;
        P.idx_in = l == 0 ? idx : tmp_idx; P.val_in = l == 0 ? val : tmp_val;
        P.idx_out = l == 0 ? tmp_idx : out_idx; P.val_out = l == 0 ? tmp_val : out_val;
        P.counts = counts; P.blk_seg = blk_seg; P.blk_start = blk_start; P.seg_start = seg_start;
        P.nseg = nseg; P.R = R; P.shift = bits - db * (l + 1);
        P.per_xcd = (c.xcd_remap == 1 && rows >= 64) ? cdiv(rows, 8) : 0u;
        const u32 grid = P.per_xcd ? 8 * P.per_xcd : rows;
        {
            const int pc = c.prof_begin(K_RS_COUNT, (u64)m * 4);
            if (db == 9) ps_count_kernel<9><<<grid, 256, 0, s>>>(P, rows); else ps_count_kernel<8><<<grid, 256, 0, s>>>(P, rows);
            LAUNCH_CHECK();
            c.prof_end(pc);
        }
        {
            Ctx::ProfScope prof(c, K_SCAN, (u64)rows * D * 12);
            ss_blocksum_kernel<<<blocks_ub, 256, 0, s>>>(counts, blk_start, nseg, R, D, bs);
            LAUNCH_CHECK();
            ss_segbase_kernel<<<nseg, 1024, 0, s>>>(bs, blk_start, seg_start, D, nstart);
            LAUNCH_CHECK();
            ss_set_word_kernel<<<1, 1, 0, s>>>(nstart + (size_t)nseg * D, (u32)m);
            LAUNCH_CHECK();
            ss_apply_kernel<<<blocks_ub, 256, 0, s>>>(counts, blk_start, nseg, R, D, bs);
            LAUNCH_CHECK();
        }
        {
            const int ps = c.prof_begin(K_RS_SCATTER_U32, (u64)m * 16);
            if (db == 9) ps_scatter_kernel<9><<<grid, 256, 0, s>>>(P, rows); else ps_scatter_kernel<8><<<grid, 256, 0, s>>>(P, rows);
            LAUNCH_CHECK();
            c.prof_end(ps);
        }
        c.arena.release(lm);
        seg_start = nstart;
        nseg *= D;
    }
    c.arena.release(mark);
}

__device__ __forceinline__ u32 ss_leaf_class(const u32* __restrict__ leaf_start, u32 l, u32 small = SS_SMALL) {
    const u32 size = leaf_start[l + 1] - leaf_start[l];
    if (size <= small) return 0;
    if (l & 1u) return 2;
    return size <= SS_UNIT_MAX ? 1u : 3u;
}
__device__ __forceinline__ bool ss_unit_first(const u32* __restrict__ leaf_start, u32 l, u32 cls, u32 small = SS_SMALL) {
    if (cls == 1) return true;
    if (cls != 0) return false;
    if (l == 0) return true;
    return ss_leaf_class(leaf_start, l - 1, small) != 0 || (leaf_start[l] / small) != (leaf_start[l - 1] / small);
}
__global__ void ss_unit_flag_kernel(const u32* __restrict__ leaf_start, u32 nleaf, u32* __restrict__ flag, u32* __restrict__ large_list,
                                    u32* __restrict__ large_count, u32 large_cap, u32 small = SS_SMALL) {
    const u32 l = blockIdx.x * blockDim.x + threadIdx.x;
    if (l >= nleaf) return;
    const u32 cls = ss_leaf_class(leaf_start, l, small);
    flag[l] = ss_unit_first(leaf_start, l, cls, small) ? 1u : 0u;
    if (cls == 3) { const u32 i = atomicAdd(large_count, 1u); if (i < large_cap) large_list[i] = l; }
}
__global__ void ss_unit_fill_kernel(const u32* __restrict__ leaf_start, u32 nleaf, const u32* __restrict__ uidx, u32* __restrict__ unit_rng, u32 small = SS_SMALL) {
    const u32 l = blockIdx.x * blockDim.x + threadIdx.x;
    if (l >= nleaf) return;
    const u32 cls = ss_leaf_class(leaf_start, l, small);
    if (cls > 1) return;
    const bool first = ss_unit_first(leaf_start, l, cls, small);
    const u32 u = uidx[l] - (first ? 0u : 1u);
    if (first) unit_rng[2 * u] = leaf_start[l];
    bool last = (cls == 1) || (l + 1 == nleaf);
    if (!last) {
        const u32 c2 = ss_leaf_class(leaf_start, l + 1, small);
        last = c2 != 0 || (leaf_start[l + 1] / small) != (leaf_start[l] / small);
    }
    if (last) unit_rng[2 * u + 1] = leaf_start[l + 1];
}

constexpr int LS_NW = 8;
__device__ __forceinline__ u32 ls_rank(u32 d, bool valid, u32* mycnt, unsigned long long* M, u64 lanebit, u64 lt_mask) {
    const u64 peers = wave_match_lds(M, d, valid, lanebit);
    const u32 prefix = lds_load(&mycnt[d]);
    const u32 rank = (u32)__popcll(peers & lt_mask);
    if (valid && rank == 0) lds_store(&mycnt[d], prefix + (u32)__popcll(peers));
    return prefix + rank;
}
__device__ __forceinline__ void ls_digit_starts(u32 (*wcnt)[256], int lane) {
    uint4 c[LS_NW];
    u32 t0 = 0, t1 = 0, t2 = 0, t3 = 0;
#pragma unroll
    for (int i = 0; i < LS_NW; ++i) {
        c[i] = *(const uint4*)&wcnt[i][4 * lane];
        t0 += c[i].x; t1 += c[i].y; t2 += c[i].z; t3 += c[i].w;
    }
    const u32 sum = t0 + t1 + t2 + t3;
    u32 r0 = wave_inclusive_sum(sum) - sum;
    u32 r1 = r0 + t0, r2 = r1 + t1, r3 = r2 + t2;
#pragma unroll
    for (int i = 0; i < LS_NW; ++i) {
        *(uint4*)&wcnt[i][4 * lane] = make_uint4(r0, r1, r2, r3);
        r0 += c[i].x; r1 += c[i].y; r2 += c[i].z; r3 += c[i].w;
    }
}
template <int ROWS>
__global__ __launch_bounds__(LS_NW * 64) __attribute__((amdgpu_waves_per_eu(4, 4))) void ss_leaf_comp_kernel(u64* __restrict__ keys, u32* __restrict__ vals, const u32* __restrict__ unit_rng,
                                                                   const u32* __restrict__ list, u32 count, u32* __restrict__ d_err, u32* __restrict__ wide_list) {
    __shared__ __align__(16) u32 wcnt[LS_NW][256];
    __shared__ u64 stage[ROWS * LS_NW * 64];
    __shared__ u64 red[2][LS_NW];
    if (blockIdx.x >= count) return;
    const u32 u = list[blockIdx.x];
    const u32 a = unit_rng[2 * u], b = unit_rng[2 * u + 1];
// ... 130 lines not shown
    }
}

constexpr int UC_T = 1024;
__global__ __launch_bounds__(UC_T) void ss_unit_class_kernel(const u32* __restrict__ unit_rng, const u32* __restrict__ d_nunits, u32* __restrict__ cls_count,
                                                            u32* __restrict__ cls_list, u32 cap, int wide = 0) {
    __shared__ u32 wcnt[UC_T / 64][16];
    __shared__ u32 wbase[16];
    const u32 u = blockIdx.x * blockDim.x + threadIdx.x;
    const u32 ncls = wide ? (u32)WIDE_NCLS : 4u;
    u32 c = 15u;
    if (u < *d_nunits) {
        const u32 m = unit_rng[2 * u + 1] - unit_rng[2 * u];
        if (m > 1 && m <= SS_UNIT_MAX) c = wide ? wide_class(m) : (m - 1) / 2048;
    }
    const int lane = lane_id(), w = wave_id();
    u32 below = 0;
    for (u32 q = 0; q < ncls; ++q) {
        const u64 mask = __ballot(c == q);
        if (lane == 0) wcnt[w][q] = (u32)__popcll(mask);
        if (c == q) below = (u32)__popcll(mask & ((1ull << lane) - 1));
    }
    __syncthreads();
    if (threadIdx.x < ncls) {
        const u32 q = threadIdx.x;
        u32 tot = 0;
        for (int i = 0; i < UC_T / 64; ++i) { const u32 t = wcnt[i][q]; wcnt[i][q] = tot; tot += t; }
        wbase[q] = tot ? atomicAdd(&cls_count[q], tot) : 0u;
    }
    __syncthreads();
    if (c < ncls) cls_list[(size_t)c * cap + wbase[c] + wcnt[w][c] + below] = u;
}

static u32 pow2_ceil(u64 x) { u32 p = 1; while ((u64)p < x) p <<= 1; return p; }

bool splitter_sort_applicable(size_t n) { return n >= ((size_t)1 << 20) && n < ((size_t)1 << 32); }

int splitter_sort_pairs_u64(Ctx& c, u64* keys[2], u32* vals[2], size_t n, const TextKeyGen* gen, SplitSortStats* st) {
    SplitSortStats local;
    if (!st) st = &local;
    *st = SplitSortStats();
    hipStream_t s = c.stream;
    const size_t mark = c.arena.mark();
    TextKeyGen g;
    if (gen) g = *gen; else memset(&g, 0, sizeof(g));

    int L = n <= (size_t)256 * 3072 ? 1 : ((n + 65535) / 65536 <= 4352 ? 2 : 3);
    if (c.ssort_levels >= 1 && c.ssort_levels <= 3) L = c.ssort_levels;
    u32 F[3] = { 1, 1, 1 };
    u32 os;
    {
        const u32 cap = L == 1 ? 256u : (L == 2 ? 65536u : (1u << 24));
        u32 nl = pow2_ceil((n + (L == 3 ? 2047 : 3071)) / (L == 3 ? 2048 : 3072));
        if (nl > cap) nl = cap;
        if (nl < (2u << (L - 1))) nl = 2u << (L - 1);
        const u32 lastF = nl > 256 ? 256u : (L == 1 ? nl : nl >> (L - 1));
        F[L - 1] = lastF;
        u32 rest = nl / lastF;
        if (L == 2) F[0] = rest;
        if (L == 3) { F[0] = 1; while ((u64)F[0] * F[0] < rest) F[0] <<= 1; F[1] = rest / F[0]; if (F[1] < 2) { F[1] = 2; } }
        const u64 avg = (n + nl - 1) / nl;
        os = avg > 3072 ? 64 : (avg > 2304 ? 32 : 16);
    }
    const u32 NLr = F[0] * F[1] * F[2];
    const u32 NS = NLr - 1;
    const u32 S = os * NLr;
    st->levels = (u32)L; st->range_leaves = NLr; st->samples = S;

    u64* sp = c.arena.get<u64>((size_t)NS + 1);
    {
        const size_t m2 = c.arena.mark();
        u64* sk[2] = { c.arena.get<u64>(S), c.arena.get<u64>(S) };
        u32* sv[2] = { c.arena.get<u32>(S), c.arena.get<u32>(S) };
        if (gen) ss_sample_kernel<true><<<cdiv(S, 256), 256, 0, s>>>(nullptr, g, n, S, sk[0], sv[0]);
        else ss_sample_kernel<false><<<cdiv(S, 256), 256, 0, s>>>(keys[0], g, n, S, sk[0], sv[0]);
        LAUNCH_CHECK();
        const int x = radix_sort_pairs_u64(c, sk, sv, S, 0, 64);
        ss_pick_kernel<<<cdiv((size_t)NS + 1, 256), 256, 0, s>>>(sk[x], NS, os, sp);
        LAUNCH_CHECK();
        c.arena.release(m2);
    }

    u16* digits = c.arena.get<u16>(align_up(n, SS_TILE) + SS_TILE);
    u32* seg_start = c.arena.get<u32>(2);
    ss_set_word_kernel<<<1, 1, 0, s>>>(seg_start, 0u);
    LAUNCH_CHECK();
    ss_set_word_kernel<<<1, 1, 0, s>>>(seg_start + 1, (u32)n);
    LAUNCH_CHECK();
    u32 nseg = 1;
    int cur = gen ? -1 : 0;
    for (int l = 0; l < L; ++l) {
        const bool last = (l == L - 1);
        const bool gl = gen && l == 0;
        const u32 D = last ? 2 * F[l] : F[l];
        u32 stride = 1;
        for (int q = l + 1; q < L; ++q) stride *= F[q];
        const u64 tiles = (n + SS_TILE - 1) / SS_TILE;
        u32 R = 128;
        while (R > 1 && (u64)nseg * R > tiles / 8 + 64) R >>= 1;
        const u32 blocks_ub = (u32)((tiles + R - 1) / R) + nseg;
        const u32 rows = blocks_ub * R;
        u32* nstart = c.arena.get<u32>((size_t)nseg * D + 1);
        const size_t lm2 = c.arena.mark();
        u32* blk_start = c.arena.get<u32>((size_t)nseg + 1);
        u32* blk_seg = c.arena.get<u32>(blocks_ub);
        u32* counts = c.arena.get<u32>((size_t)rows * D);
        u32* bs = c.arena.get<u32>((size_t)blocks_ub * D);
        ss_nblk_kernel<<<cdiv((size_t)nseg + 1, 256), 256, 0, s>>>(seg_start, nseg, R, blk_start);
        LAUNCH_CHECK();
        exclusive_sum_u32(c, blk_start, blk_start, (size_t)nseg + 1, nullptr);
        ss_blkseg_kernel<<<cdiv(nseg, 256), 256, 0, s>>>(blk_start, nseg, blk_seg);
        LAUNCH_CHECK();
        SSLevel P;
        P.keys_in = cur >= 0 ? keys[cur] : nullptr; P.vals_in = cur >= 0 ? vals[cur] : nullptr;
        const int nxt = cur < 0 ? 0 : (cur ^ 1);
        P.keys_out = keys[nxt]; P.vals_out = vals[nxt];
        P.digits = digits;
        P.counts = counts; P.blk_seg = blk_seg; P.blk_start = blk_start; P.seg_start = seg_start; P.sp = sp;
        P.nseg = nseg; P.F = F[l]; P.stride = stride; P.R = R; P.D = D;
        P.per_xcd = (c.xcd_remap == 1 && rows >= 64) ? cdiv(rows, 8) : 0u;
        const u32 grid = P.per_xcd ? 8 * P.per_xcd : rows;
        {
            const int pc = c.prof_begin(K_RS_COUNT, (u64)n * (gl ? 1 : 8));
            if (gl && last) ss_count_kernel<true, true><<<grid, 256, 0, s>>>(P, g, rows);
            else if (gl) ss_count_kernel<true, false><<<grid, 256, 0, s>>>(P, g, rows);
            else if (last) ss_count_kernel<false, true><<<grid, 256, 0, s>>>(P, g, rows);
            else ss_count_kernel<false, false><<<grid, 256, 0, s>>>(P, g, rows);
            LAUNCH_CHECK();
            c.prof_end(pc);
        }
        {
            Ctx::ProfScope prof(c, K_SCAN, (u64)rows * D * 12);
            ss_blocksum_kernel<<<blocks_ub, 256, 0, s>>>(counts, blk_start, nseg, R, D, bs);
            LAUNCH_CHECK();
            ss_segbase_kernel<<<nseg, 1024, 0, s>>>(bs, blk_start, seg_start, D, nstart);
            LAUNCH_CHECK();
            ss_set_word_kernel<<<1, 1, 0, s>>>(nstart + (size_t)nseg * D, (u32)n);
            LAUNCH_CHECK();
            ss_apply_kernel<<<blocks_ub, 256, 0, s>>>(counts, blk_start, nseg, R, D, bs);
            LAUNCH_CHECK();
        }
        {
            const int ps = c.prof_begin(K_RS_SCATTER_U64, (u64)n * (gl ? 13 : 24));
            if (gl && last) ss_scatter_stable_kernel<true, true><<<grid, 256, 0, s>>>(P, g, rows);
            else if (gl) ss_scatter_kernel<true, false><<<grid, 256, 0, s>>>(P, g, rows);
            else if (last) ss_scatter_stable_kernel<false, true><<<grid, 256, 0, s>>>(P, g, rows);
            else ss_scatter_kernel<false, false><<<grid, 256, 0, s>>>(P, g, rows);
            LAUNCH_CHECK();
            c.prof_end(ps);
        }
        c.arena.release(lm2);
        seg_start = nstart;
        nseg = nseg * D;
        cur = nxt;
    }
    const u32 nleaf = nseg;
    const u32* leaf_start = seg_start;

    constexpr u32 LARGE_CAP = 1024;
    u32* flag = c.arena.get<u32>((size_t)nleaf + 1);
    u32* unit_rng = c.arena.get<u32>(2 * ((size_t)nleaf + 1));
    u32* large = c.arena.get<u32>(LARGE_CAP + 6);
    u32* wide_list = c.arena.get<u32>((size_t)nleaf + 2);
    u32* cls_list = c.arena.get<u32>(4 * ((size_t)nleaf + 1));
    HIP_TRY(hipMemsetAsync(large, 0, 6 * sizeof(u32), s));
    HIP_TRY(hipMemsetAsync(wide_list, 0, sizeof(u32), s));
    ss_unit_flag_kernel<<<cdiv(nleaf, 256), 256, 0, s>>>(leaf_start, nleaf, flag, large + 6, large, LARGE_CAP);
    LAUNCH_CHECK();
    exclusive_sum_u32(c, flag, flag, nleaf, large + 1);
    ss_unit_fill_kernel<<<cdiv(nleaf, 256), 256, 0, s>>>(leaf_start, nleaf, flag, unit_rng);
    LAUNCH_CHECK();
    ss_unit_class_kernel<<<cdiv((size_t)nleaf + 1, UC_T), UC_T, 0, s>>>(unit_rng, large + 1, large + 2, cls_list, nleaf + 1);
    LAUNCH_CHECK();
    u32 hc[6];
    c.read_n(large, hc, 6);
    const u32 nlarge = hc[0], nunits = hc[1];
    st->units = nunits; st->large_leaves = nlarge;
    {
        Ctx::ProfScope prof(c, K_SS_LEAF, (u64)n * 24);
        u64* K = keys[cur]; u32* V = vals[cur];
        const u32 cap = nleaf + 1;
        if (hc[2]) { ss_leaf_comp_kernel<4><<<hc[2], LS_NW * 64, 0, s>>>(K, V, unit_rng, cls_list, hc[2], c.d_err, wide_list); LAUNCH_CHECK(); }
        if (hc[3]) { ss_leaf_comp_kernel<8><<<hc[3], LS_NW * 64, 0, s>>>(K, V, unit_rng, cls_list + (size_t)cap, hc[3], c.d_err, wide_list); LAUNCH_CHECK(); }
        if (hc[4]) { ss_leaf_comp_kernel<12><<<hc[4], LS_NW * 64, 0, s>>>(K, V, unit_rng, cls_list + 2 * (size_t)cap, hc[4], c.d_err, wide_list); LAUNCH_CHECK(); }
        if (hc[5]) { ss_leaf_comp_kernel<16><<<hc[5], LS_NW * 64, 0, s>>>(K, V, unit_rng, cls_list + 3 * (size_t)cap, hc[5], c.d_err, wide_list); LAUNCH_CHECK(); }
        const u32 nwide = (hc[2] | hc[3] | hc[4] | hc[5]) ? c.read(wide_list) : 0u;
        if (nwide) {
            ss_leaf_wide_kernel<<<nwide, LS_NW * 64, 0, s>>>(K, V, unit_rng, wide_list, nwide, c.d_err);
            LAUNCH_CHECK();
            st->wide_units = nwide;
        }
    }
    if (nlarge) {
        if (nlarge > LARGE_CAP) throw HipError{hipErrorUnknown, "splitter sort: too many oversized leaves", (int)__LINE__};
        std::vector<u32> ll(nlarge), ls((size_t)nleaf + 1);
        HIP_TRY(hipMemcpyAsync(ll.data(), large + 6, nlarge * sizeof(u32), hipMemcpyDeviceToHost, s));
        HIP_TRY(hipMemcpyAsync(ls.data(), leaf_start, ((size_t)nleaf + 1) * sizeof(u32), hipMemcpyDeviceToHost, s));
        HIP_TRY(hipStreamSynchronize(s));
        for (u32 i = 0; i < nlarge; ++i) {
            const size_t a = ls[ll[i]], b = ls[ll[i] + 1];
            u64* kk[2] = { keys[cur] + a, keys[cur ^ 1] + a };
            u32* vv[2] = { vals[cur] + a, vals[cur ^ 1] + a };
            const int y = radix_sort_pairs_u64(c, kk, vv, b - a, 0, 64);
            if (y == 1) {
                HIP_TRY(hipMemcpyAsync(kk[0], kk[1], (b - a) * sizeof(u64), hipMemcpyDeviceToDevice, s));
                HIP_TRY(hipMemcpyAsync(vv[0], vv[1], (b - a) * sizeof(u32), hipMemcpyDeviceToDevice, s));
            }
            st->large_pairs += b - a;
        }
    }
    c.arena.release(mark);
    return cur;
}

void ss_level_tables(Ctx& c, const u32* seg_start, u32 nseg, size_t n, u32 D, SegTables& T) {
    hipStream_t s = c.stream;
    const u64 tiles = (n + SS_TILE - 1) / SS_TILE;
    u32 R = 128;
    while (R > 1 && (u64)nseg * R > tiles / 8 + 64) R >>= 1;
    T.R = R;
    T.blocks_ub = (u32)((tiles + R - 1) / R) + nseg;
    T.rows = T.blocks_ub * R;
    T.blk_start = c.arena.get<u32>((size_t)nseg + 1);
    T.blk_seg = c.arena.get<u32>(T.blocks_ub);
    T.counts = c.arena.get<u32>((size_t)T.rows * D);
    T.bs = c.arena.get<u32>((size_t)T.blocks_ub * D);
    ss_nblk_kernel<<<cdiv((size_t)nseg + 1, 256), 256, 0, s>>>(seg_start, nseg, R, T.blk_start);
    LAUNCH_CHECK();
    exclusive_sum_u32(c, T.blk_start, T.blk_start, (size_t)nseg + 1, nullptr);
    ss_blkseg_kernel<<<cdiv(nseg, 256), 256, 0, s>>>(T.blk_start, nseg, T.blk_seg);
    LAUNCH_CHECK();
}
void ss_level_offsets(Ctx& c, const SegTables& T, const u32* seg_start, u32 nseg, u32 D, u32* nstart, size_t n) {
    hipStream_t s = c.stream;
    Ctx::ProfScope prof(c, K_SCAN, (u64)T.rows * D * 12);
    ss_blocksum_kernel<<<T.blocks_ub, 256, 0, s>>>(T.counts, T.blk_start, nseg, T.R, D, T.bs);
    LAUNCH_CHECK();
    ss_segbase_kernel<<<nseg, 1024, 0, s>>>(T.bs, T.blk_start, seg_start, D, nstart);
    LAUNCH_CHECK();
    ss_set_word_kernel<<<1, 1, 0, s>>>(nstart + (size_t)nseg * D, (u32)n);
    LAUNCH_CHECK();
    ss_apply_kernel<<<T.blocks_ub, 256, 0, s>>>(T.counts, T.blk_start, nseg, T.R, D, T.bs);
    LAUNCH_CHECK();
}
void ss_level_offsets_sub(Ctx& c, const SegTables& T, u32 nsub, const u32* blk_super, const u32* out_start, u32 nsuper, u32 D, u32* nstart, size_t n) {
    hipStream_t s = c.stream;
    Ctx::ProfScope prof(c, K_SCAN, (u64)T.rows * D * 12);
    ss_blocksum_kernel<<<T.blocks_ub, 256, 0, s>>>(T.counts, T.blk_start, nsub, T.R, D, T.bs);
    LAUNCH_CHECK();
    ss_segbase_kernel<<<nsuper, 1024, 0, s>>>(T.bs, blk_super, out_start, D, nstart);
    LAUNCH_CHECK();
    ss_set_word_kernel<<<1, 1, 0, s>>>(nstart + (size_t)nsuper * D, (u32)n);
    LAUNCH_CHECK();
    ss_apply_kernel<<<T.blocks_ub, 256, 0, s>>>(T.counts, T.blk_start, nsub, T.R, D, T.bs);
    LAUNCH_CHECK();
}
u32* ss_first_segment(Ctx& c, size_t n) {
    u32* seg_start = c.arena.get<u32>(2);
    ss_set_word_kernel<<<1, 1, 0, c.stream>>>(seg_start, 0u);
    LAUNCH_CHECK();
    ss_set_word_kernel<<<1, 1, 0, c.stream>>>(seg_start + 1, (u32)n);
    LAUNCH_CHECK();
    return seg_start;
}
void ss_build_units(Ctx& c, const u32* leaf_start, u32 nleaf, UnitTables& U, u32 small) {
    if (small == 0) small = SS_SMALL;
    hipStream_t s = c.stream;
    constexpr u32 LARGE_CAP = 1024;
    U.large_cap = LARGE_CAP;
    u32* flag = c.arena.get<u32>((size_t)nleaf + 1);
    U.unit_rng = c.arena.get<u32>(2 * ((size_t)nleaf + 1));
    U.large = c.arena.get<u32>(LARGE_CAP + 6);
    U.cls_list = c.arena.get<u32>((U.wide_classes ? (size_t)WIDE_NCLS : 4) * ((size_t)nleaf + 1));
    u32* wcnt = U.wide_classes ? c.arena.get<u32>(16) : nullptr;
    if (wcnt) HIP_TRY(hipMemsetAsync(wcnt, 0, 16 * sizeof(u32), s));
    U.cap = nleaf + 1;
    HIP_TRY(hipMemsetAsync(U.large, 0, 6 * sizeof(u32), s));
    ss_unit_flag_kernel<<<cdiv(nleaf, 256), 256, 0, s>>>(leaf_start, nleaf, flag, U.large + 6, U.large, LARGE_CAP, small);
    LAUNCH_CHECK();
    exclusive_sum_u32(c, flag, flag, nleaf, U.large + 1);
    ss_unit_fill_kernel<<<cdiv(nleaf, 256), 256, 0, s>>>(leaf_start, nleaf, flag, U.unit_rng, small);
    LAUNCH_CHECK();
    ss_unit_class_kernel<<<cdiv((size_t)nleaf + 1, UC_T), UC_T, 0, s>>>(U.unit_rng, U.large + 1, wcnt ? wcnt : U.large + 2, U.cls_list, nleaf + 1, U.wide_classes);
    LAUNCH_CHECK();
    c.read_n(U.large, U.hc, 6);
    if (wcnt) c.read_n(wcnt, U.whc, 16);
}
void ss_fanouts(Ctx& c, size_t n, int& L, u32 F[3], u32& os, u32 leaf3, int wide2) {
    L = n <= (size_t)256 * 3072 ? 1 : ((n + 65535) / 65536 <= 3584 ? 2 : 3);
    if (c.ssort_levels >= 1 && c.ssort_levels <= 3) L = c.ssort_levels;
    F[0] = F[1] = F[2] = 1;
    if (leaf3 == 0) leaf3 = 2048;
    if ((wide2 == 1 && L == 3) || wide2 == 2) {
        u32 nl2 = pow2_ceil((n + leaf3 - 1) / leaf3);
        if (nl2 <= (1u << 20) && nl2 >= 2048u) {
            L = 2;
            F[1] = 1024u;
            F[0] = nl2 / F[1];
            const u64 avg2 = (n + nl2 - 1) / nl2;
            os = avg2 > 3072 ? 64 : (avg2 > 2304 ? 32 : 16);
            return;
        }
    }
    const u32 cap = L == 1 ? 256u : (L == 2 ? 65536u : (1u << 24));
    u32 nl = pow2_ceil((n + (L == 3 ? leaf3 - 1 : 3071)) / (L == 3 ? leaf3 : 3072));
    if (nl > cap) nl = cap;
    if (nl < (2u << (L - 1))) nl = 2u << (L - 1);
    const u32 lastF = nl > 256 ? 256u : (L == 1 ? nl : nl >> (L - 1));
    F[L - 1] = lastF;
    u32 rest = nl / lastF;
    if (L == 2) F[0] = rest;
    if (L == 3) { F[0] = 1; while ((u64)F[0] * F[0] < rest) F[0] <<= 1; F[1] = rest / F[0]; if (F[1] < 2) { F[1] = 2; } }
    const u64 avg = (n + nl - 1) / nl;
    os = avg > 3072 ? 64 : (avg > 2304 ? 32 : 16);
}

}
```

tudocomp_amd/csrc/wsort.hip:

```cpp
#include "prim.hpp"

#include <vector>
#include <algorithm>
#include <stdlib.h>

namespace tdc {

constexpr int WS_TILE = 4096;
constexpr int WS_ITEMS = 16;
constexpr int WS_HALO = 64;
#ifndef TDC_WS_PEEL
#define TDC_WS_PEEL 0
#endif
#ifndef TDC_WS_CMAX
#define TDC_WS_CMAX 64
#endif
constexpr u32 WS_CMAX = TDC_WS_CMAX;
constexpr u32 WS_WAVE_MAX = 1024;

struct WSLevel {
    const u64* k1_in; const u64* k2_in; const u32* v_in;
    u64* k1_out; u64* k2_out; u32* v_out;
    u32* counts;
    const u32* blk_seg; const u32* blk_start; const u32* seg_start;
// ... 1269 lines not shown
    if (q >= H.chunks) return;
    const u32 t = (blk - blk_start[s]) * R + row % R;
    const u32 lb0 = H.blk[q][b], lb1 = H.blk[q][b + 1], Rq = H.R[q];
    const bool in = t < (lb1 - lb0) * Rq;
    const u32* src = H.counts[q] + ((size_t)lb0 * Rq + t) * D;
    for (u32 d = threadIdx.x; d < D; d += 64) counts[(size_t)row * D + d] = in ? src[d] : 0u;
}

void wsort_make_keygen(const Ctx& c, const u8* text, size_t n, u32 sigma, const u8* code, int& KW, WKeyGen& g) {
    const int b = (int)bits_for(sigma > 1 ? sigma - 1 : 1);
    const int per_word = 64 / b;
    KW = c.wsort_kw ? c.wsort_kw : (per_word < 16 ? 2 : 1);
    g.text = text; g.n = n; g.b = b;
    g.s = (64 * KW) / b; if (g.s > 64) g.s = 64;
    if (c.wsort_syms > 0 && g.s > c.wsort_syms) g.s = c.wsort_syms;
    g.pad = 64 * KW - g.s * b;
    g.inv = (65536u + (u32)b - 1) / (u32)b;
    memcpy(g.code, code, 256);
}
bool wsort_applicable(const Ctx& c, size_t n) { return c.wsort && n >= c.wsort_min && n < ((size_t)1 << 32); }
int wsort_result_index(Ctx& c, size_t n) {
    int L; u32 F[3], os;
    ss_fanouts(c, n, L, F, os, (u32)c.wsort_leaf, c.wsort_two);
    if (c.wsort_order == 1 && L == 3) std::swap(F[0], F[2]);
    return (L - 1) & 1;
}

namespace {
struct WPlan { int L; u32 F[3]; u32 os, NLr, NS, S; };

template <int KW, bool GEN>
void ws_splitters(Ctx& c, const WPlan& pl, const u64* k1, const u64* k2, const WKeyGen& g, size_t n, u64* sp1, u64* sp2) {
    hipStream_t s = c.stream;
    const size_t m2 = c.arena.mark();
    const u32 S = pl.S;
    u64* a1[2] = { c.arena.get<u64>(S), c.arena.get<u64>(S) };
    u64* a2[2] = { nullptr, nullptr };
    if (KW == 2) { a2[0] = c.arena.get<u64>(S); a2[1] = c.arena.get<u64>(S); }
    u32* iv[2] = { c.arena.get<u32>(S), c.arena.get<u32>(S) };
    ws_sample_kernel<KW, GEN><<<cdiv(S, 256), 256, 0, s>>>(k1, k2, g, n, S, a1[0], a2[0], iv[0]);
    LAUNCH_CHECK();
    if (KW == 1) {
        const int x = radix_sort_pairs_u64(c, a1, iv, S, 0, 64);
        ws_pick_kernel<<<cdiv((size_t)pl.NS + 1, 256), 256, 0, s>>>(a1[x], nullptr, pl.NS, pl.os, sp1, nullptr);
        LAUNCH_CHECK();
    } else {
        ws_lsd_sort_wide(c, a1, a2, nullptr, S, 64);
        ws_pick_kernel<<<cdiv((size_t)pl.NS + 1, 256), 256, 0, s>>>(a1[1], a2[1], pl.NS, pl.os, sp1, sp2);
        LAUNCH_CHECK();
    }
    c.arena.release(m2);
}

template <int KW, bool GEN, bool PAIRS>
int ws_sort_impl(Ctx& c, const WKeyGen* gen, u64* K1[2], u64* K2[2], u32* V[2], size_t n, int k1_bits, u8* flags, u8* lcp8, WSortStats* st,
                 const WPre* pre = nullptr, u32* v_final = nullptr) {
    hipStream_t s = c.stream;
    const size_t mark = c.arena.mark();
    WKeyGen g;
    if (gen) g = *gen; else memset(&g, 0, sizeof(g));
    WPlan pl;
    u64* sp1; u64* sp2;
    if (pre) {
        pl.L = pre->L; pl.F[0] = pre->F[0]; pl.F[1] = pre->F[1]; pl.F[2] = pre->F[2]; pl.os = pre->os;
        pl.NLr = pre->NLr; pl.NS = pre->NS; pl.S = pre->S;
        sp1 = pre->sp1; sp2 = pre->sp2;
    } else {
        ss_fanouts(c, n, pl.L, pl.F, pl.os, (u32)c.wsort_leaf, c.wsort_two);
        if (c.wsort_order == 1 && pl.L == 3) std::swap(pl.F[0], pl.F[2]);
        pl.NLr = pl.F[0] * pl.F[1] * pl.F[2]; pl.NS = pl.NLr - 1; pl.S = pl.os * pl.NLr;
        sp1 = c.arena.get<u64>((size_t)pl.NS + 1);
        sp2 = KW == 2 ? c.arena.get<u64>((size_t)pl.NS + 1) : nullptr;
        ws_splitters<KW, GEN>(c, pl, K1[0], KW == 2 ? K2[0] : nullptr, g, n, sp1, sp2);
    }
    const int L = pl.L;
    st->levels = (u32)L; st->range_leaves = pl.NLr; st->samples = pl.S; st->kw = KW;

    unsigned long long* d_nonheads = (unsigned long long*)c.arena.get<u64>(1);
    HIP_TRY(hipMemsetAsync(d_nonheads, 0, sizeof(u64), s));
    if (PAIRS) flags = c.arena.get<u8>(n + 8);
    HIP_TRY(hipMemsetAsync(flags, 0, n, s));

    u16* digits = pre ? pre->digits : c.arena.get<u16>(align_up(n, WS_TILE) + WS_TILE);
    const u32* seg_start = pre ? nullptr : ss_first_segment(c, n);
    u32 nseg = 1;
    int cur = GEN ? -1 : 0;
    u32* Vlast = nullptr;
    if (pre) {
        const int l = 1;
        const bool last = (l == L - 1);
        const u32 F0 = pl.F[0], nch = pre->nchunks, nsub = F0 * nch;
        const u32 D = last ? 2 * pl.F[l] : pl.F[l];
        u32 stride = 1;
        for (int q = l + 1; q < L; ++q) stride *= pl.F[q];
        u32* nstart = c.arena.get<u32>((size_t)F0 * D + 1);
        const size_t lm2 = c.arena.mark();
        u32* seg_begin = c.arena.get<u32>(nsub + 1);
        u32* seg_end = c.arena.get<u32>(nsub + 1);
        u32* out_start = c.arena.get<u32>(F0 + 1);
        ws_sub_tables_kernel<<<1, 1024, 0, s>>>(pre->nstart_all, F0, nch, seg_begin, seg_end, out_start);
        LAUNCH_CHECK();
        SegTables Tb;
        {
            const u64 tiles = (n + WS_TILE - 1) / WS_TILE;
            u32 R = 128;
            while (R > 1 && (u64)nsub * R > tiles / 8 + 64) R >>= 1;
            Tb.R = R; Tb.blocks_ub = (u32)((tiles + R - 1) / R) + nsub; Tb.rows = Tb.blocks_ub * R;
            Tb.blk_start = c.arena.get<u32>((size_t)nsub + 1);
            Tb.blk_seg = c.arena.get<u32>(Tb.blocks_ub);
            Tb.counts = c.arena.get<u32>((size_t)Tb.rows * D);
            Tb.bs = c.arena.get<u32>((size_t)Tb.blocks_ub * D);
            ws_sub_nblk_kernel<<<cdiv((size_t)nsub + 1, 256), 256, 0, s>>>(seg_begin, seg_end, nsub, R, Tb.blk_start);
            LAUNCH_CHECK();
            exclusive_sum_u32(c, Tb.blk_start, Tb.blk_start, (size_t)nsub + 1, nullptr);
            ws_blkseg_kernel<<<cdiv(nsub, 256), 256, 0, s>>>(Tb.blk_start, nsub, Tb.blk_seg);
            LAUNCH_CHECK();
        }
        u32* blk_super = c.arena.get<u32>(F0 + 1);
        ws_blk_super_kernel<<<cdiv(F0 + 1, 256), 256, 0, s>>>(Tb.blk_start, F0, nch, blk_super);
        LAUNCH_CHECK();
        WSLevel P;
        P.k1_in = pre->K1[0]; P.k2_in = KW == 2 ? pre->K2[0] : nullptr; P.v_in = pre->V[0];
        Vlast = last ? v_final : pre->V[1];
        P.k1_out = pre->K1[1]; P.k2_out = KW == 2 ? pre->K2[1] : nullptr; P.v_out = Vlast;
        P.digits = digits;
        P.counts = Tb.counts; P.blk_seg = Tb.blk_seg; P.blk_start = Tb.blk_start; P.seg_start = seg_begin; P.seg_end = seg_end; P.sub = nch;
        P.sp1 = sp1; P.sp2 = sp2;
        P.nseg = nsub; P.F = pl.F[l]; P.stride = stride; P.R = Tb.R; P.D = D;
        P.pre_digits = pre->dig2 ? pre->dig2_chunks : 0u;
        P.pre_counts = (pre->dig2 && c.wsort_prehist) ? pre->dig2_chunks : 0u;
        P.gen_off = 0; P.gen_len = n;
        const u32 rows = Tb.rows;
        P.per_xcd = (c.xcd_remap == 1 && rows >= 64) ? cdiv(rows, 8) : 0u;
        const u32 grid = P.per_xcd ? 8 * P.per_xcd : rows;
        if (P.pre_counts) {
            WPreHist H;
            for (u32 q = 0; q < 32; ++q) { H.counts[q] = pre->dig2_counts[q]; H.blk[q] = pre->dig2_blk[q]; H.R[q] = pre->dig2_R[q]; }
            H.nch = nch; H.chunks = P.pre_counts;
            ws_pre_hist_kernel<<<Tb.rows, 64, 0, s>>>(H, Tb.blk_start, Tb.blk_seg, nsub, Tb.R, D, Tb.rows, Tb.counts);
            LAUNCH_CHECK();
        }
        {
            const int pc = c.prof_begin(K_RS_COUNT, (u64)n * 8 * KW);
            if (last) { if (P.F > 256) ws_count_kernel<KW, false, true, 1024><<<grid, 256, 0, s>>>(P, g, rows); else if (P.F > 64) ws_count_kernel<KW, false, true, 256><<<grid, 256, 0, s>>>(P, g, rows); else ws_count_kernel<KW, false, true, 64><<<grid, 256, 0, s>>>(P, g, rows); }
            else { if (P.F > 256) ws_count_kernel<KW, false, false, 1024><<<grid, 256, 0, s>>>(P, g, rows); else if (P.F > 64) ws_count_kernel<KW, false, false, 256><<<grid, 256, 0, s>>>(P, g, rows); else ws_count_kernel<KW, false, false, 64><<<grid, 256, 0, s>>>(P, g, rows); }
            LAUNCH_CHECK();
            c.prof_end(pc);
        }
        ss_level_offsets_sub(c, Tb, nsub, blk_super, out_start, F0, D, nstart, n);
        {
            const int ps = c.prof_begin(K_RS_SCATTER_U64, (u64)n * (2 * (4 + 8 * KW) + 2));
            if (last) { if (P.F > 256) ws_scatter_kernel<KW, false, true, 1024><<<grid, 256, 0, s>>>(P, g, rows); else ws_scatter_kernel<KW, false, true, 256><<<grid, 256, 0, s>>>(P, g, rows); }
            else { if (P.F > 256) ws_scatter_kernel<KW, false, false, 1024><<<grid, 256, 0, s>>>(P, g, rows); else ws_scatter_kernel<KW, false, false, 256><<<grid, 256, 0, s>>>(P, g, rows); }
            LAUNCH_CHECK();
            c.prof_end(ps);
        }
        c.arena.release(lm2);
        seg_start = nstart;
        nseg = F0 * D;
        cur = 1;
        K1 = const_cast<u64**>(pre->K1); K2 = const_cast<u64**>(pre->K2); V = const_cast<u32**>(pre->V);
    }
    for (int l = pre ? 2 : 0; l < L; ++l) {
        const bool last = (l == L - 1);
        const bool gl = GEN && l == 0;
        const u32 D = last ? 2 * pl.F[l] : pl.F[l];
        u32 stride = 1;
        for (int q = l + 1; q < L; ++q) stride *= pl.F[q];
        u32* nstart = c.arena.get<u32>((size_t)nseg * D + 1);
        const size_t lm2 = c.arena.mark();
        SegTables Tb;
        ss_level_tables(c, seg_start, nseg, n, D, Tb);
        WSLevel P;
        P.k1_in = cur >= 0 ? K1[cur] : nullptr; P.k2_in = (cur >= 0 && KW == 2) ? K2[cur] : nullptr;
        P.v_in = pre ? Vlast : (cur >= 0 ? V[cur] : nullptr);
        const int nxt = cur < 0 ? 0 : (cur ^ 1);
        P.k1_out = K1[nxt]; P.k2_out = KW == 2 ? K2[nxt] : nullptr;
        P.v_out = (pre && last) ? v_final : V[nxt];
        Vlast = P.v_out;
        P.digits = digits;
        P.counts = Tb.counts; P.blk_seg = Tb.blk_seg; P.blk_start = Tb.blk_start; P.seg_start = seg_start; P.sp1 = sp1; P.sp2 = sp2;
        P.seg_end = seg_start + 1; P.sub = 1;
        P.nseg = nseg; P.F = pl.F[l]; P.stride = stride; P.R = Tb.R; P.D = D;
        P.gen_off = 0; P.gen_len = n;
        const u32 rows = Tb.rows;
        P.per_xcd = (c.xcd_remap == 1 && rows >= 64) ? cdiv(rows, 8) : 0u;
        const u32 grid = P.per_xcd ? 8 * P.per_xcd : rows;
        {
            const int pc = c.prof_begin(K_RS_COUNT, (u64)n * (gl ? 1 : 8 * KW));
            if (gl && last) { if (P.F > 256) ws_count_kernel<KW, GEN, true, 1024><<<grid, 256, 0, s>>>(P, g, rows); else ws_count_kernel<KW, GEN, true, 256><<<grid, 256, 0, s>>>(P, g, rows); }
            else if (gl) { if (P.F > 256) ws_count_kernel<KW, GEN, false, 1024><<<grid, 256, 0, s>>>(P, g, rows); else ws_count_kernel<KW, GEN, false, 256><<<grid, 256, 0, s>>>(P, g, rows); }
            else if (last) { if (P.F > 256) ws_count_kernel<KW, false, true, 1024><<<grid, 256, 0, s>>>(P, g, rows); else if (P.F > 64) ws_count_kernel<KW, false, true, 256><<<grid, 256, 0, s>>>(P, g, rows); else ws_count_kernel<KW, false, true, 64><<<grid, 256, 0, s>>>(P, g, rows); }
            else { if (P.F > 256) ws_count_kernel<KW, false, false, 1024><<<grid, 256, 0, s>>>(P, g, rows); else if (P.F > 64) ws_count_kernel<KW, false, false, 256><<<grid, 256, 0, s>>>(P, g, rows); else ws_count_kernel<KW, false, false, 64><<<grid, 256, 0, s>>>(P, g, rows); }
            LAUNCH_CHECK();
            c.prof_end(pc);
        }
        ss_level_offsets(c, Tb, seg_start, nseg, D, nstart, n);
        {
            const int ps = c.prof_begin(K_RS_SCATTER_U64, (u64)n * (gl ? 3 + 4 + 8 * KW : 2 * (4 + 8 * KW) + 2));
            if (gl && last) { if (P.F > 256) ws_scatter_kernel<KW, GEN, true, 1024><<<grid, 256, 0, s>>>(P, g, rows); else ws_scatter_kernel<KW, GEN, true, 256><<<grid, 256, 0, s>>>(P, g, rows); }
            else if (gl) { if (P.F > 256) ws_scatter_kernel<KW, GEN, false, 1024><<<grid, 256, 0, s>>>(P, g, rows); else ws_scatter_kernel<KW, GEN, false, 256><<<grid, 256, 0, s>>>(P, g, rows); }
            else if (last) { if (P.F > 256) ws_scatter_kernel<KW, false, true, 1024><<<grid, 256, 0, s>>>(P, g, rows); else ws_scatter_kernel<KW, false, true, 256><<<grid, 256, 0, s>>>(P, g, rows); }
            else { if (P.F > 256) ws_scatter_kernel<KW, false, false, 1024><<<grid, 256, 0, s>>>(P, g, rows); else ws_scatter_kernel<KW, false, false, 256><<<grid, 256, 0, s>>>(P, g, rows); }
            LAUNCH_CHECK();
            c.prof_end(ps);
        }
        c.arena.release(lm2);
        seg_start = nstart;
        nseg = nseg * D;
        cur = nxt;
    }
    const u32 nleaf = nseg;
    const u32* leaf_start = seg_start;

    UnitTables U;
    U.wide_classes = 1;
    ss_build_units(c, leaf_start, nleaf, U, (u32)c.wsort_pack);
    const u32 nlarge = U.hc[0];
    st->units = U.hc[1]; st->large_leaves = nlarge;
    WLeaf A;
    A.k1 = K1[cur]; A.k2 = KW == 2 ? K2[cur] : nullptr; A.v = Vlast; A.unit_rng = U.unit_rng; A.flags = flags; A.lcp = lcp8;
    A.d_err = c.d_err; A.inv = g.b ? (65536u + (u32)g.b - 1) / (u32)g.b : 65536u;
    A.cmax = c.wsort_small ? 1u : (c.wsort_cmax < 1 ? 1u : (c.wsort_cmax > (int)WS_CMAX ? WS_CMAX : (u32)c.wsort_cmax));
    {
        const u32* cur_rng = U.unit_rng;
        const u32* cur_cls = U.cls_list;
        size_t cur_cap = U.cap;
        constexpr int NB = WIDE_NCLS;
        u32 cur_cnt[NB];
        for (int q = 0; q < NB; ++q) cur_cnt[q] = U.whc[q];
        u32 wave_cnt[4] = { 0, 0, 0, 0 };
        u64 wave_recs = 0;
        const u32* wave_list = nullptr;
        const u32 ediv = A.cmax + 1;
        const u32 ecap2 = (u32)(n / ediv + 2);
        u32* e_rng[2] = { c.arena.get<u32>(2 * (size_t)ecap2), c.arena.get<u32>(2 * (size_t)ecap2) };
        u32* e_cls[2] = { c.arena.get<u32>(EC_NCLS * (size_t)ecap2), c.arena.get<u32>(EC_NCLS * (size_t)ecap2) };
        u32* lc = c.arena.get<u32>(64);
        for (int stage = 0; stage < 8; ++stage) {
            if (wave_cnt[0] | wave_cnt[1] | wave_cnt[2] | wave_cnt[3]) {
                Ctx::ProfScope prof(c, K_WS_RUN, wave_recs * 18);
                A.unit_rng = cur_rng;
                const u32* l0 = wave_list, *l1 = wave_list + cur_cap, *l2 = wave_list + 2 * cur_cap, *l3 = wave_list + 3 * cur_cap;
                const bool fork = c.wsort_run_streams && c.aux_stream && (wave_cnt[0] + wave_cnt[1] + wave_cnt[2] + wave_cnt[3]) >= 4096;
                hipStream_t sl = fork ? c.copy_stream : s, sw = fork ? c.aux_stream : s;
                if (fork) { c.wait_for(sl, s); c.wait_for(sw, s); }
                if (wave_cnt[3]) { ws_run_wave_kernel<1024, PAIRS><<<cdiv(wave_cnt[3], 4), 256, 0, s>>>(A, l3, wave_cnt[3]); LAUNCH_CHECK(); }
                if (wave_cnt[2]) { ws_run_wave_kernel<256, PAIRS><<<cdiv(wave_cnt[2], 4), 256, 0, sw>>>(A, l2, wave_cnt[2]); LAUNCH_CHECK(); }
                if (wave_cnt[0]) { ws_run_lane_kernel<32, PAIRS><<<cdiv(wave_cnt[0], 8), 256, 0, sl>>>(A, l0, wave_cnt[0]); LAUNCH_CHECK(); }
                if (wave_cnt[1]) { ws_run_lane_kernel<64, PAIRS><<<cdiv(wave_cnt[1], 4), 256, 0, sl>>>(A, l1, wave_cnt[1]); LAUNCH_CHECK(); }
                if (fork) { c.wait_for(s, sl); c.wait_for(s, sw); }
                st->wave_runs += wave_cnt[0] + wave_cnt[1] + wave_cnt[2] + wave_cnt[3];
                wave_cnt[0] = wave_cnt[1] = wave_cnt[2] = wave_cnt[3] = 0;
            }
            { u32 any = 0; for (int q = 0; q < NB; ++q) any |= cur_cnt[q]; if (!any) break; }
// ... 122 lines not shown
            st->nonheads = nh;
        }
    }
#ifdef TDC_WL_PROF
    if (!PAIRS) {
        unsigned long long hp[16];
        HIP_TRY(hipStreamSynchronize(s));
        HIP_TRY(hipMemcpyFromSymbol(hp, HIP_SYMBOL(wl_prof), sizeof(hp)));
        fprintf(stderr, "[wl_prof] wgs %llu records %llu passes %llu | ticks: load %llu lsd %llu heads %llu pos %llu k2 %llu count %llu fin %llu nofuse %llu\n", hp[15], hp[14], hp[13],
                hp[0], hp[1], hp[2], hp[3], hp[4], hp[5], hp[6], hp[7]);
        memset(hp, 0, sizeof(hp));
        HIP_TRY(hipMemcpyToSymbol(HIP_SYMBOL(wl_prof), hp, sizeof(hp)));
    }
#endif
    c.arena.release(mark);
    return cur;
}
}

int wsort_suffixes(Ctx& c, int KW, const WKeyGen& g, u64* K1[2], u64* K2[2], u32* V[2], size_t n, u8* flags, u8* lcp8, WSortStats* st) {
    WSortStats local;
    if (!st) st = &local;
    *st = WSortStats();
    if (KW == 2) return ws_sort_impl<2, true, false>(c, &g, K1, K2, V, n, 64, flags, lcp8, st);
    return ws_sort_impl<1, true, false>(c, &g, K1, K2, V, n, 64, flags, lcp8, st);
}

void wsort_suffixes_pre(Ctx& c, const WPre& P, u32* v_final, u8* flags, u8* lcp8, WSortStats* st) {
    WSortStats local;
    if (!st) st = &local;
    *st = WSortStats();
    u64* K1[2] = { P.K1[0], P.K1[1] }; u64* K2[2] = { P.K2[0], P.K2[1] }; u32* V[2] = { P.V[0], P.V[1] };
    if (P.KW == 2) (void)ws_sort_impl<2, true, false>(c, &P.g, K1, K2, V, P.n, 64, flags, lcp8, st, &P, v_final);
    else (void)ws_sort_impl<1, true, false>(c, &P.g, K1, K2, V, P.n, 64, flags, lcp8, st, &P, v_final);
}

bool wsort_pre_begin(Ctx& c, WPre& P, const u8* text, size_t n, const size_t* chunk_off, u32 nchunks, const u32* hist0) {
    P = WPre();
    if (!c.wsort_overlap || !wsort_applicable(c, n) || nchunks < 2 || nchunks > 32 || chunk_off[1] < ((size_t)1 << 22)) return false;
    for (u32 q = 0; q < nchunks; ++q) if (chunk_off[q] % WS_TILE != 0 || chunk_off[q] > chunk_off[q + 1]) return false;
    if (chunk_off[0] != 0 || chunk_off[nchunks] != n) return false;
    u8 code[256];
    u32 sigma = 0;
    for (int i = 0; i < 256; ++i) {
        code[i] = (u8)sigma;
        if (i == 0 || hist0[i]) { ++sigma; P.present[i >> 5] |= 1u << (i & 31); }
    }
    P.text = text; P.n = n; P.nchunks = nchunks;
    for (u32 q = 0; q <= nchunks; ++q) P.chunk_off[q] = chunk_off[q];
    wsort_make_keygen(c, text, n, sigma, code, P.KW, P.g);
    ss_fanouts(c, n, P.L, P.F, P.os, (u32)c.wsort_leaf, c.wsort_two);
    if (c.wsort_order == 1 && P.L == 3) std::swap(P.F[0], P.F[2]);
    if (P.L < 2) return false;
    P.NLr = P.F[0] * P.F[1] * P.F[2]; P.NS = P.NLr - 1; P.S = P.os * P.NLr;
    Arena& A = c.arena;
    P.K1[0] = A.get_top<u64>(n); P.K1[1] = A.get_top<u64>(n);
    if (P.KW == 2) { P.K2[0] = A.get_top<u64>(n); P.K2[1] = A.get_top<u64>(n); }
    P.V[0] = A.get_top<u32>(n); P.V[1] = A.get_top<u32>(n);
    P.digits = A.get_top<u16>(align_up(n, WS_TILE) + WS_TILE);
    P.sp1 = A.get_top<u64>((size_t)P.NS + 1);
    P.sp2 = P.KW == 2 ? A.get_top<u64>((size_t)P.NS + 1) : nullptr;
    P.nstart_all = A.get_top<u32>((size_t)nchunks * (P.F[0] + 1));
    P.dig2 = c.wsort_predig != 0 && c.aux_stream != nullptr;
    P.dig2_chunks = P.dig2 ? (nchunks > (u32)c.wsort_predig_skip ? nchunks - (u32)c.wsort_predig_skip : 0u) : 0u;
    WPlan pl;
    pl.L = P.L; pl.F[0] = P.F[0]; pl.F[1] = P.F[1]; pl.F[2] = P.F[2]; pl.os = P.os; pl.NLr = P.NLr; pl.NS = P.NS; pl.S = P.S;
    const size_t n_sample = chunk_off[1] - 64;
    if (P.KW == 2) ws_splitters<2, true>(c, pl, nullptr, nullptr, P.g, n_sample, P.sp1, P.sp2);
    else ws_splitters<1, true>(c, pl, nullptr, nullptr, P.g, n_sample, P.sp1, nullptr);
    P.begun = true;
    return true;
}

void wsort_pre_chunk(Ctx& c, WPre& P, u32 q) {
    if (!P.begun) return;
    hipStream_t s = c.stream;
    const size_t off = P.chunk_off[q];
    if (off >= P.n) {
        ws_set2_kernel<<<1, 1, 0, s>>>(P.nstart_all + (size_t)q * (P.F[0] + 1), (u32)P.n, (u32)P.n);
        return;
    }
    const size_t len = P.chunk_off[q + 1] - off;
    const size_t mark = c.arena.mark();
    u32* seg2 = c.arena.get<u32>(2);
    ws_set2_kernel<<<1, 1, 0, s>>>(seg2, (u32)off, (u32)(off + len));
    LAUNCH_CHECK();
    const u32 D = P.F[0];
    SegTables Tb;
    ss_level_tables(c, seg2, 1, len, D, Tb);
    WSLevel Lv;
    Lv.k1_in = nullptr; Lv.k2_in = nullptr; Lv.v_in = nullptr;
    Lv.k1_out = P.K1[0]; Lv.k2_out = P.KW == 2 ? P.K2[0] : nullptr; Lv.v_out = P.V[0];
    Lv.digits = P.digits;
    Lv.counts = Tb.counts; Lv.blk_seg = Tb.blk_seg; Lv.blk_start = Tb.blk_start; Lv.seg_start = seg2; Lv.seg_end = seg2 + 1; Lv.sub = 1;
    Lv.sp1 = P.sp1; Lv.sp2 = P.sp2;
    Lv.nseg = 1; Lv.F = P.F[0]; Lv.stride = P.F[1] * P.F[2]; Lv.R = Tb.R; Lv.D = D;
    Lv.gen_off = 0; Lv.gen_len = P.n;
    const u32 rows = Tb.rows;
    Lv.per_xcd = (c.xcd_remap == 1 && rows >= 64) ? cdiv(rows, 8) : 0u;
    const u32 grid = Lv.per_xcd ? 8 * Lv.per_xcd : rows;
    {
        const int pc = c.prof_begin(K_RS_COUNT, (u64)len);
        if (P.KW == 2) { if (Lv.F > 256) ws_count_kernel<2, true, false, 1024><<<grid, 256, 0, s>>>(Lv, P.g, rows); else ws_count_kernel<2, true, false, 256><<<grid, 256, 0, s>>>(Lv, P.g, rows); }
        else { if (Lv.F > 256) ws_count_kernel<1, true, false, 1024><<<grid, 256, 0, s>>>(Lv, P.g, rows); else ws_count_kernel<1, true, false, 256><<<grid, 256, 0, s>>>(Lv, P.g, rows); }
        LAUNCH_CHECK();
        c.prof_end(pc);
    }
    ss_level_offsets(c, Tb, seg2, 1, D, P.nstart_all + (size_t)q * (P.F[0] + 1), off + len);
    {
        const int ps = c.prof_begin(K_RS_SCATTER_U64, (u64)len * (3 + 4 + 8 * P.KW));
        if (P.KW == 2) { if (Lv.F > 256) ws_scatter_kernel<2, true, false, 1024><<<grid, 256, 0, s>>>(Lv, P.g, rows); else ws_scatter_kernel<2, true, false, 256><<<grid, 256, 0, s>>>(Lv, P.g, rows); }
        else { if (Lv.F > 256) ws_scatter_kernel<1, true, false, 1024><<<grid, 256, 0, s>>>(Lv, P.g, rows); else ws_scatter_kernel<1, true, false, 256><<<grid, 256, 0, s>>>(Lv, P.g, rows); }
        LAUNCH_CHECK();
        c.prof_end(ps);
    }
    c.arena.release(mark);
    if (P.dig2 && q < P.dig2_chunks) {
        c.wait_for(c.aux_stream, c.stream);
        StreamSwap swap(c, c.aux_stream);
        hipStream_t s = c.stream;
        const u32* seg_start = P.nstart_all + (size_t)q * (P.F[0] + 1);
        const bool last2 = (P.L == 2);
        const u32 nseg = P.F[0], D2 = last2 ? 2 * P.F[1] : P.F[1];
        SegTables T2;
        ss_level_tables(c, seg_start, nseg, len, D2, T2);
        P.dig2_counts[q] = T2.counts; P.dig2_blk[q] = T2.blk_start; P.dig2_R[q] = T2.R;
        WSLevel L2;
        L2.k1_in = P.K1[0]; L2.k2_in = P.KW == 2 ? P.K2[0] : nullptr; L2.v_in = P.V[0];
        L2.k1_out = nullptr; L2.k2_out = nullptr; L2.v_out = nullptr;
        L2.digits = P.digits;
        L2.counts = T2.counts; L2.blk_seg = T2.blk_seg; L2.blk_start = T2.blk_start; L2.seg_start = seg_start; L2.seg_end = seg_start + 1; L2.sub = 1;
        L2.sp1 = P.sp1; L2.sp2 = P.sp2;
        L2.nseg = nseg; L2.F = P.F[1]; L2.stride = last2 ? 1u : P.F[2]; L2.R = T2.R; L2.D = D2;
        L2.gen_off = 0; L2.gen_len = P.n;
        const u32 rows2 = T2.rows;
        L2.per_xcd = (c.xcd_remap == 1 && rows2 >= 64) ? cdiv(rows2, 8) : 0u;
        const u32 grid2 = L2.per_xcd ? 8 * L2.per_xcd : rows2;
        const int pc = c.prof_begin(K_RS_COUNT, (u64)len * 8 * P.KW);
        auto launch = [&](auto kw, auto lastc) {
            constexpr int KWc = decltype(kw)::value; constexpr bool LASTc = decltype(lastc)::value;
            if (L2.F > 256) ws_count_kernel<KWc, false, LASTc, 1024><<<grid2, 256, 0, s>>>(L2, P.g, rows2);
            else if (L2.F > 64) ws_count_kernel<KWc, false, LASTc, 256><<<grid2, 256, 0, s>>>(L2, P.g, rows2);
            else ws_count_kernel<KWc, false, LASTc, 64><<<grid2, 256, 0, s>>>(L2, P.g, rows2);
        };
        if (P.KW == 2) { if (last2) launch(std::integral_constant<int, 2>{}, std::true_type{}); else launch(std::integral_constant<int, 2>{}, std::false_type{}); }
        else { if (last2) launch(std::integral_constant<int, 1>{}, std::true_type{}); else launch(std::integral_constant<int, 1>{}, std::false_type{}); }
        LAUNCH_CHECK();
        c.prof_end(pc);
        HIP_TRY(hipEventRecord(c.ev_dig2, c.aux_stream));
    }
}

void wsort_pre_finish(Ctx& c, WPre& P, const u32* hist_full) {
    P.active = false;
    if (!P.begun) return;
    if (P.dig2) HIP_TRY(hipStreamWaitEvent(c.stream, c.ev_dig2, 0));
    for (int i = 1; i < 256; ++i) {
        const bool in_map = (P.present[i >> 5] >> (i & 31)) & 1u;
        if ((hist_full[i] != 0) != in_map) return;
    }
    P.active = true;
}

#ifndef TDC_SG_MAXG
#define TDC_SG_MAXG 16
#endif
#ifndef TDC_SG_T
#define TDC_SG_T 1024
#endif
constexpr u32 SG_T = TDC_SG_T, SG_H = TDC_SG_MAXG, SG_MAXG = TDC_SG_MAXG, SG_BIG_CAP = 1u << 16;
constexpr u32 SG_EDIV = SG_MAXG + 1;
struct SegCounters { u32 overflow, nbig, big_recs, pad; };
// ... 231 lines not shown
```

Before: 8926.

## Fuse segment table construction and rework level offset scan into chunked passes

Replaces the separate nblk/exclusive-sum/blkseg launches with a single-block tables kernel that also writes the first segment bounds, removing the tiny set-word kernels. Rewrites the per-level offset computation as vectorized blocksum, a chunked in-LDS prefix scan across row blocks, a segment-base pass and an apply pass. Also adds a level-offsets test primitive. This cuts launch count and serial per-segment scanning in the suffix sort, at the cost of more complex kernels and a single-block table kernel that may serialize on large segment counts.

```diff
diff --git a/include/tdc_gpu.h b/include/tdc_gpu.h
--- a/include/tdc_gpu.h
+++ b/include/tdc_gpu.h
@@ -151,6 +151,8 @@
                                uint32_t fillA, uint32_t* outA, uint32_t* count);
 int tdc_gpu_prim_mark_orbit(tdc_gpu_ctx* ctx, const uint32_t* next, size_t n, uint8_t* mark);
 int tdc_gpu_prim_tile_entries(tdc_gpu_ctx* ctx, const uint16_t* exit0, size_t ntiles, uint32_t states, uint16_t* entry0);
+int tdc_gpu_prim_level_offsets(tdc_gpu_ctx* ctx, const uint32_t* seg_start, uint32_t nseg, size_t n, uint32_t D, uint32_t nsuper,
+                               const uint32_t* tile_counts, uint32_t* offsets_out, uint32_t* nstart_out);
 int tdc_gpu_prim_arena_fill(tdc_gpu_ctx* ctx, int byte, uint64_t* base, uint64_t* size);
 
 int tdc_gpu_lcpcomp_decompress(tdc_gpu_ctx* ctx, const uint8_t* stream, size_t len, uint8_t** out, size_t* out_len,
diff --git a/tudocomp_amd/__init__.py b/tudocomp_amd/__init__.py
--- a/tudocomp_amd/__init__.py
+++ b/tudocomp_amd/__init__.py
@@ -892,6 +892,18 @@
         self._check(self._L.tdc_gpu_prim_tile_entries(self._h, _ptr(a), ntiles, states, _ptr(entry)))
         return entry
 
+    def prim_level_offsets(self, seg_start, D, tile_counts, nsuper=0):
+        s = np.ascontiguousarray(seg_start, dtype=np.uint32)
+        t = np.ascontiguousarray(tile_counts, dtype=np.uint32).reshape(-1)
+        nseg = len(s) - 1
+        tiles = int(((np.diff(s.astype(np.int64)) + 4095) // 4096).sum())
+        if len(t) != tiles * int(D):
+            raise ValueError("D counts per 4096-record tile of every segment")
+        off = np.empty(len(t), dtype=np.uint32)
+        nstart = np.empty((int(nsuper) if nsuper else nseg) * int(D) + 1, dtype=np.uint32)
+        self._check(self._L.tdc_gpu_prim_level_offsets(self._h, _ptr(s), nseg, int(s[-1]), int(D), int(nsuper), _ptr(t), _ptr(off), _ptr(nstart)))
+        return off, nstart
+
     def prim_arena_fill(self, byte=None):
         base, size = ctypes.c_uint64(), ctypes.c_uint64()
         self._check(self._L.tdc_gpu_prim_arena_fill(self._h, -1 if byte is None else int(byte), ctypes.byref(base), ctypes.byref(size)))
diff --git a/tudocomp_amd/_native.py b/tudocomp_amd/_native.py
--- a/tudocomp_amd/_native.py
+++ b/tudocomp_amd/_native.py
@@ -12,7 +12,7 @@
     "tdc_gpu_lz78_compress", "tdc_gpu_lzss_lcp_compress", "tdc_gpu_lzss_lcp_factorize",
     "tdc_gpu_sort_pairs_u64", "tdc_gpu_suffix_array", "tdc_gpu_textds", "tdc_gpu_lcpcomp_factorize", "tdc_gpu_flatten", "tdc_gpu_encode_huff",
     "tdc_gpu_prim_scan", "tdc_gpu_prim_sort_pairs", "tdc_gpu_prim_bucketed_scatter", "tdc_gpu_prim_msd_partition", "tdc_gpu_prim_select", "tdc_gpu_prim_select_counts",
-    "tdc_gpu_prim_mark_orbit", "tdc_gpu_prim_tile_entries", "tdc_gpu_prim_arena_fill",
+    "tdc_gpu_prim_mark_orbit", "tdc_gpu_prim_tile_entries", "tdc_gpu_prim_level_offsets", "tdc_gpu_prim_arena_fill",
     "tdc_gpu_lcpcomp_decompress",
     "tdc_gpu_lcpcomp_compress_comp",
     "tdc_gpu_encode_arith",
@@ -142,6 +142,7 @@
     L.tdc_gpu_prim_select_counts.argtypes = [vp, vp, ctypes.c_uint8, sz, vp, vp, u32, vp, ctypes.POINTER(u32)]
     L.tdc_gpu_prim_mark_orbit.argtypes = [vp, vp, sz, vp]
     L.tdc_gpu_prim_tile_entries.argtypes = [vp, vp, sz, u32, vp]
+    L.tdc_gpu_prim_level_offsets.argtypes = [vp, vp, u32, sz, u32, u32, vp, vp, vp]
     L.tdc_gpu_prim_arena_fill.argtypes = [vp, i32, ctypes.POINTER(ctypes.c_uint64), ctypes.POINTER(ctypes.c_uint64)]
     L.tdc_gpu_suffix_array.argtypes = [vp, vp, sz, vp, vp]
     L.tdc_gpu_textds.argtypes = [vp, vp, sz, vp, vp, vp, vp, vp, ctypes.POINTER(u32)]
diff --git a/tudocomp_amd/csrc/api_prims.hip b/tudocomp_amd/csrc/api_prims.hip
--- a/tudocomp_amd/csrc/api_prims.hip
+++ b/tudocomp_amd/csrc/api_prims.hip
@@ -232,6 +232,65 @@
     });
 }
 
+int tdc_gpu_prim_level_offsets(tdc_gpu_ctx* ctx, const uint32_t* seg_start, uint32_t nseg, size_t n, uint32_t D, uint32_t nsuper,
+                               const uint32_t* tile_counts, uint32_t* offsets_out, uint32_t* nstart_out) {
+    return guarded(ctx, [&] {
+        constexpr size_t TILE = 4096;
+        if (!seg_start || !nstart_out) bad("seg_start/nstart_out is NULL");
+        if (nseg == 0 || nseg > (1u << 20)) bad("1 <= nseg <= 2^20 required");
+        if (D == 0 || D > 2048) bad("1 <= D <= 2048 required");
+        if (nsuper && nseg % nsuper) bad("nsuper must divide nseg");
+        check_count(n);
+        if (seg_start[0] != 0 || seg_start[nseg] != n) bad("seg_start[0] = 0 and seg_start[nseg] = n required");
+        size_t tiles = 0;
+        for (uint32_t s = 0; s < nseg; ++s) {
+            if (seg_start[s + 1] < seg_start[s]) bad("seg_start must not decrease");
+            tiles += ((size_t)seg_start[s + 1] - seg_start[s] + TILE - 1) / TILE;
+        }
+        if (tiles && (!tile_counts || !offsets_out)) bad("tile_counts/offsets_out is NULL");
+        Ctx& c = ctx->c;
+        reserve_arena(c, (2 * tiles + 2 * (size_t)nseg + 256) * D * 4 * 2 + (size_t)nseg * 64 + ((size_t)64 << 20));
+        const u32 nsg = nsuper ? nsuper : nseg, gsz = nseg / nsg;
+        const u32* d_seg = upload(c, seg_start, (size_t)nseg + 1);
+        u32* d_nstart = c.arena.get<u32>((size_t)nsg * D + 1);
+        SegTables T;
+        ss_level_tables(c, d_seg, nseg, n, D, T);
+        std::vector<u32> blk((size_t)nseg + 1);
+        download(c, blk.data(), T.blk_start, (size_t)nseg + 1);
+        HIP_TRY(hipStreamSynchronize(c.stream));
+        const size_t R = T.R, real_rows = (size_t)blk[nseg] * R;
+        if (blk[0] != 0 || blk[nseg] > T.blocks_ub) throw ArgError{TDC_GPU_ERR_INTERNAL, "level tables: row blocks out of range"};
+        std::vector<u32> tab(real_rows * D + 4, 0u);
+        {
+            size_t t0 = 0;
+            for (uint32_t s = 0; s < nseg; ++s) {
+                const size_t ts = ((size_t)seg_start[s + 1] - seg_start[s] + TILE - 1) / TILE;
+                if ((size_t)blk[s + 1] - blk[s] != (ts + R - 1) / R || blk[s + 1] < blk[s]) throw ArgError{TDC_GPU_ERR_INTERNAL, "level tables: wrong row blocks of a segment"};
+                std::copy(tile_counts + t0 * D, tile_counts + (t0 + ts) * D, tab.begin() + (size_t)blk[s] * R * D);
+                t0 += ts;
+            }
+        }
+        if (real_rows) HIP_TRY(hipMemcpyAsync(T.counts, tab.data(), real_rows * D * sizeof(u32), hipMemcpyHostToDevice, c.stream));
+        if (nsuper) {
+            std::vector<u32> bsup((size_t)nsuper + 1), ostart((size_t)nsuper + 1);
+            for (uint32_t S = 0; S <= nsuper; ++S) { bsup[S] = blk[(size_t)S * gsz]; ostart[S] = seg_start[(size_t)S * gsz]; }
+            const u32* d_bsup = upload(c, bsup.data(), (size_t)nsuper + 1);
+            const u32* d_ostart = upload(c, ostart.data(), (size_t)nsuper + 1);
+            HIP_TRY(hipStreamSynchronize(c.stream));
+            ss_level_offsets_sub(c, T, nseg, d_bsup, d_ostart, nsuper, D, d_nstart, n);
+        } else ss_level_offsets(c, T, d_seg, nseg, D, d_nstart, n);
+        download(c, tab.data(), T.counts, real_rows * D);
+        download(c, nstart_out, d_nstart, (size_t)nsg * D + 1);
+        HIP_TRY(hipStreamSynchronize(c.stream));
+        size_t t0 = 0;
+        for (uint32_t s = 0; s < nseg; ++s) {
+            const size_t ts = ((size_t)seg_start[s + 1] - seg_start[s] + TILE - 1) / TILE;
+            std::copy(tab.begin() + (size_t)blk[s] * R * D, tab.begin() + ((size_t)blk[s] * R + ts) * D, offsets_out + t0 * D);
+            t0 += ts;
+        }
+    });
+}
+
 int tdc_gpu_prim_arena_fill(tdc_gpu_ctx* ctx, int byte, uint64_t* base, uint64_t* size) {
     return guarded(ctx, [&] {
         if (!base || !size) bad("base/size is NULL");
diff --git a/tudocomp_amd/csrc/fused.hip b/tudocomp_amd/csrc/fused.hip
--- a/tudocomp_amd/csrc/fused.hip
+++ b/tudocomp_amd/csrc/fused.hip
@@ -322,13 +322,14 @@
     u32* idx[2] = { c.arena.get<u32>(m), c.arena.get<u32>(m) };
     const bool wp = phi != nullptr;
     void* rp[2] = { c.arena.alloc(m * (wp ? 8 : 4)), c.arena.alloc(m * (wp ? 8 : 4)) };
-    const u32* seg_start = ss_first_segment(c, m);
+    const u32* seg_start = ss_first_segment(c);
+    const u32 first[2] = { 0u, (u32)m };
     u32 nseg = 1;
     for (int l = 0; l < 2; ++l) {
         u32* nstart = c.arena.get<u32>((size_t)nseg * D + 1);
         const size_t lm = c.arena.mark();
         SegTables Tb;
-        ss_level_tables(c, seg_start, nseg, m, D, Tb);
+        ss_level_tables(c, seg_start, nseg, m, D, Tb, l == 0 ? first : nullptr);
         FSLevel P;
         if (l == 0) { P.idx_in = sa + 1; P.rp_in = nullptr; P.prev_in = sa; P.lcp_in = lcp8 + 1; }
         else { P.idx_in = idx[0]; P.rp_in = rp[0]; P.prev_in = nullptr; P.lcp_in = nullptr; }
diff --git a/tudocomp_amd/csrc/prim.hpp b/tudocomp_amd/csrc/prim.hpp
--- a/tudocomp_amd/csrc/prim.hpp
+++ b/tudocomp_amd/csrc/prim.hpp
@@ -27,8 +27,8 @@
     if (m <= 4096u) return 5u + (m <= 2560u ? 0u : (m - 2049u) / 512u);
     return 9u;
 }
-u32* ss_first_segment(Ctx& c, size_t n);
-void ss_level_tables(Ctx& c, const u32* seg_start, u32 nseg, size_t n, u32 D, SegTables& T);
+u32* ss_first_segment(Ctx& c);
+void ss_level_tables(Ctx& c, const u32* seg_start, u32 nseg, size_t n, u32 D, SegTables& T, const u32* first = nullptr);
 void ss_level_offsets(Ctx& c, const SegTables& T, const u32* seg_start, u32 nseg, u32 D, u32* nstart, size_t n);
 void ss_level_offsets_sub(Ctx& c, const SegTables& T, u32 nsub, const u32* blk_super, const u32* out_start, u32 nsuper, u32 D, u32* nstart, size_t n);
 void ss_build_units(Ctx& c, const u32* leaf_start, u32 nleaf, UnitTables& U, u32 small = 0);
diff --git a/tudocomp_amd/csrc/ssort.hip b/tudocomp_amd/csrc/ssort.hip
--- a/tudocomp_amd/csrc/ssort.hip
+++ b/tudocomp_amd/csrc/ssort.hip
@@ -135,6 +135,46 @@
     if (s >= nseg) return;
     for (u32 b = blk_start[s]; b < blk_start[s + 1]; ++b) blk_seg[b] = s;
 }
+constexpr u32 LT_MAX = 65537;
+constexpr u32 LT_SLAB = 8192;
+constexpr u32 LT_FILL = 1024;
+__global__ __launch_bounds__(1024) void ss_tables_kernel(u32* __restrict__ seg_start, u32 nseg, u32 R, u32 set_first, u32 first_lo, u32 first_hi,
+                                                         u32* __restrict__ blk_start, u32* __restrict__ blk_seg) {
+    __shared__ u32 nb[LT_SLAB];
+    __shared__ u32 wsum[16];
+    const u32 t = threadIdx.x;
+    if (set_first && t == 0) { seg_start[0] = first_lo; seg_start[1] = first_hi; }
+    u32 run = 0;
+    for (u32 slab = 0; slab <= nseg; slab += LT_SLAB) {
+        const u32 m = nseg + 1 - slab < LT_SLAB ? nseg + 1 - slab : LT_SLAB;
+        for (u32 i = t; i < m; i += 1024) {
+            const u32 s = slab + i;
+            u32 v = 0;
+            if (s < nseg) {
+                const u64 size = set_first ? first_hi - first_lo : seg_start[s + 1] - seg_start[s];
+                v = (u32)((size + (u64)SS_TILE * R - 1) / ((u64)SS_TILE * R));
+            }
+            nb[i] = v;
+        }
+        __syncthreads();
+        u32 sum = 0;
+        for (u32 k = 0; k < 8; ++k) if (t * 8 + k < m) sum += nb[t * 8 + k];
+        const u32 inc = wave_inclusive_sum(sum);
+        if (lane_id() == 63) wsum[wave_id()] = inc;
+        __syncthreads();
+        u32 pre = 0, tot = 0;
+        for (int w = 0; w < 16; ++w) { if (w < wave_id()) pre += wsum[w]; tot += wsum[w]; }
+        u32 o = run + pre + inc - sum;
+        for (u32 k = 0; k < 8; ++k) if (t * 8 + k < m) { const u32 v = nb[t * 8 + k]; nb[t * 8 + k] = o; o += v; }
+        run += tot;
+        __syncthreads();
+        for (u32 i = t; i < m; i += 1024) blk_start[slab + i] = nb[i];
+        __syncthreads();
+    }
+    if (nseg >= LT_FILL) return;
+    for (u32 s = wave_id(); s < nseg; s += 16)
+        for (u32 b = blk_start[s] + lane_id(); b < blk_start[s + 1]; b += 64) blk_seg[b] = s;
+}
 
 template <bool GEN, bool LAST>
 __global__ __launch_bounds__(256) void ss_count_kernel(SSLevel P, TextKeyGen g, u32 rows) {
@@ -194,44 +234,135 @@
     for (u32 i = threadIdx.x; i < P.D; i += 256) P.counts[(size_t)row * P.D + i] = hist[i];
 }
 
-__global__ __launch_bounds__(256) void ss_blocksum_kernel(const u32* __restrict__ counts, const u32* __restrict__ blk_start, u32 nseg,
-                                                          u32 R, u32 D, u32* __restrict__ bs) {
-    const u32 b = blockIdx.x;
-    if (b >= blk_start[nseg]) return;
-    for (u32 d = threadIdx.x; d < D; d += 256) {
-        u32 acc = 0;
-        for (u32 r = 0; r < R; ++r) acc += counts[((size_t)b * R + r) * D + d];
-        bs[(size_t)b * D + d] = acc;
-    }
-}
-__global__ __launch_bounds__(1024) void ss_segbase_kernel(u32* __restrict__ bs, const u32* __restrict__ blk_start, const u32* __restrict__ seg_start,
-                                                          u32 D, u32* __restrict__ next_start) {
-    __shared__ u32 part[4][2048];
-    __shared__ u32 dstart[2048];
+constexpr u32 LO_K = 8;
+constexpr u32 LO_TILE = 8192;
+constexpr u32 LO_DMAX = 2048;
+__host__ __device__ inline u32 lo_chunk_len(u32 D) { const u32 c = LO_TILE / D; return c > 32u ? 32u : c; }
+
+template <int V> struct LoVec { u32 v[V]; };
+template <int V> __device__ __forceinline__ LoVec<V> lo_load(const u32* p) {
+    LoVec<V> a;
+    if constexpr (V == 4) { const uint4 q = *(const uint4*)p; a.v[0] = q.x; a.v[1] = q.y; a.v[2] = q.z; a.v[3] = q.w; }
+    else a.v[0] = *p;
+    return a;
+}
+template <int V> __device__ __forceinline__ void lo_store(u32* p, const LoVec<V>& a) {
+    if constexpr (V == 4) *(uint4*)p = make_uint4(a.v[0], a.v[1], a.v[2], a.v[3]);
+    else *p = a.v[0];
+}
+
+template <int V>
+__global__ __launch_bounds__(256) void lo_blocksum_kernel(const u32* __restrict__ counts, const u32* __restrict__ seg_blk, u32 nsg, u32 R, u32 D,
+                                                          u32* __restrict__ bs) {
+    __shared__ u32 part[256 * V];
+    const u32 b = blockIdx.x, t = threadIdx.x, NT = blockDim.x;
+    if (b >= seg_blk[nsg]) return;
+    for (u32 col0 = 0; col0 < D; col0 += NT * V) {
+        const u32 left = (D - col0) / V;
+        const u32 W = left < NT ? left : NT, G = NT / W;
+        const u32 rg = t / W, cg = t % W;
+        const u32* p = counts + (size_t)b * R * D + col0 + cg * V;
+        LoVec<V> acc;
+#pragma unroll
+        for (int i = 0; i < V; ++i) acc.v[i] = 0;
+        if (rg < G) {
+            for (u32 r = rg; r < R; r += G * LO_K) {
+                LoVec<V> x[LO_K];
+#pragma unroll
+                for (u32 k = 0; k < LO_K; ++k) {
+                    const u32 rr = r + k * G;
+                    if (rr < R) x[k] = lo_load<V>(p + (size_t)rr * D);
+                    else for (int i = 0; i < V; ++i) x[k].v[i] = 0;
+                }
+#pragma unroll
+                for (u32 k = 0; k < LO_K; ++k)
+                    for (int i = 0; i < V; ++i) acc.v[i] += x[k].v[i];
+            }
+        }
+        if (G > 1) {
+#pragma unroll
+            for (int i = 0; i < V; ++i) part[t * V + i] = acc.v[i];
+            __syncthreads();
+            if (rg == 0)
+                for (u32 g = 1; g < G; ++g)
+                    for (int i = 0; i < V; ++i) acc.v[i] += part[(g * W + cg) * V + i];
+            __syncthreads();
+        }
+        if (rg == 0) lo_store<V>(bs + (size_t)b * D + col0 + cg * V, acc);
+    }
+}
+
+__global__ __launch_bounds__(256) void lo_chunk_kernel(u32* __restrict__ bs, const u32* __restrict__ seg_blk, u32 nsg, const u32* __restrict__ blk_seg,
+                                                       u32 gsz, u32 D, u32 C) {
+    __shared__ u32 tile[LO_TILE];
+    __shared__ u32 rs[32];
+    const u32 t = threadIdx.x;
+    const u32 nb = seg_blk[nsg], lo = blockIdx.x * C;
+    if (lo >= nb) return;
+    const u32 hi = lo + C < nb ? lo + C : nb, rows = hi - lo, words = rows * D;
+    if (t < rows) { const u32 f = seg_blk[blk_seg[lo + t] / gsz]; rs[t] = f > lo ? f - lo : 0u; }
+    u32* g_tile = bs + (size_t)lo * D;
+    for (u32 i = t; i < words; i += 256) tile[i] = g_tile[i];
+    __syncthreads();
+    const bool wide = D >= 256;
+    const u32 G = wide ? 1u : 256u / D, g = wide ? 0u : t / D;
+    const u32 per = (rows + G - 1) / G;
+    const u32 r0 = g * per < rows ? g * per : rows, r1 = r0 + per < rows ? r0 + per : rows;
+    if (g < G)
+        for (u32 d = wide ? t : t % D; d < D; d += 256) {
+            u32 run = 0;
+            for (u32 r = r0; r < r1; ++r) { run += tile[r * D + d]; tile[r * D + d] = run; }
+        }
+    if (G > 1) {
+        __syncthreads();
+        u32 add = 0;
+        const u32 d = t % D;
+        if (g < G) for (u32 k = 0; k < g; ++k) { const u32 e = (k + 1) * per < rows ? (k + 1) * per : rows; if (e > k * per) add += tile[(e - 1) * D + d]; }
+        __syncthreads();
+        if (g < G) for (u32 r = r0; r < r1; ++r) tile[r * D + d] += add;
+    }
+    __syncthreads();
+    const u32 rstep = 256u / D, dstep = 256u - rstep * D;
+    u32 r = t / D, d = t - r * D;
+    for (u32 i = t; i < words; i += 256) {
+        const u32 f = rs[r];
+        g_tile[i] = tile[i] - (f ? tile[(f - 1) * D + d] : 0u);
+        r += rstep; d += dstep;
+        if (d >= D) { d -= D; ++r; }
+    }
+}
+
+__global__ __launch_bounds__(1024) void lo_segbase_kernel(const u32* __restrict__ bs, const u32* __restrict__ seg_blk, const u32* __restrict__ seg_out,
+                                                          u32 nsg, u32 D, u32 C, u32* __restrict__ carry, u32* __restrict__ next_start, u32 n_total) {
+    __shared__ u32 part[4][LO_DMAX];
+    __shared__ u32 dstart[LO_DMAX];
     __shared__ u32 wsum[16];
     const u32 s = blockIdx.x;
-    const u32 b0 = blk_start[s], b1 = blk_start[s + 1];
-    const u32 t = threadIdx.x & 255u, g = threadIdx.x >> 8;
-    const u32 nb = b1 - b0, per = (nb + 3) / 4;
-    const u32 lo = b0 + (g * per < nb ? g * per : nb);
-    const u32 hi = (lo + per < b1) ? lo + per : b1;
+    if (s == 0 && threadIdx.x == 0) next_start[(size_t)nsg * D] = n_total;
+    const u32 b0 = seg_blk[s], b1 = seg_blk[s + 1];
+    const u32 t = threadIdx.x & 255u, g = threadIdx.x >> 8, NG = blockDim.x >> 8;
+    const u32 c0 = b0 / C, nch = b1 > b0 ? (b1 - 1) / C - c0 + 1 : 0u;
+    const u32 per = (nch + NG - 1) / NG;
+    const u32 lo = g * per < nch ? g * per : nch;
+    const u32 hi = lo + per < nch ? lo + per : nch;
+    auto end_row = [&](u32 j) -> size_t { const u32 e = (c0 + j + 1) * C; return (size_t)((e < b1 ? e : b1) - 1); };
     for (u32 d = t; d < D; d += 256) {
         u32 acc = 0;
-        u32 b = lo;
-        for (; b + 8 <= hi; b += 8) {
+        u32 j = lo;
+        for (; j + 8 <= hi; j += 8) {
             u32 v[8];
 #pragma unroll
-            for (int i = 0; i < 8; ++i) v[i] = bs[(size_t)(b + i) * D + d];
-#pragma unroll
-            for (int i = 0; i < 8; ++i) acc += v[i];
-        }
-        for (; b < hi; ++b) acc += bs[(size_t)b * D + d];
+            for (u32 i = 0; i < 8; ++i) v[i] = bs[end_row(j + i) * D + d];
+#pragma unroll
+            for (u32 i = 0; i < 8; ++i) acc += v[i];
+        }
+        for (; j < hi; ++j) acc += bs[end_row(j) * D + d];
         part[g][d] = acc;
     }
     __syncthreads();
     const u32 d0 = 2 * threadIdx.x, d1 = d0 + 1;
-    const u32 tot0 = d0 < D ? part[0][d0] + part[1][d0] + part[2][d0] + part[3][d0] : 0u;
-    const u32 tot1 = d1 < D ? part[0][d1] + part[1][d1] + part[2][d1] + part[3][d1] : 0u;
+    u32 tot0 = 0, tot1 = 0;
+    for (u32 k = 0; k < NG; ++k) { if (d0 < D) tot0 += part[k][d0]; if (d1 < D) tot1 += part[k][d1]; }
     const u32 tot = tot0 + tot1;
     u32 inc = wave_inclusive_sum(tot);
     if (lane_id() == 63) wsum[wave_id()] = inc;
@@ -239,40 +370,95 @@
     {
         u32 run = 0;
         for (int w = 0; w < wave_id(); ++w) run += wsum[w];
-        const u32 st = seg_start[s] + run + inc - tot;
+        const u32 st = seg_out[s] + run + inc - tot;
         if (d0 < D) { dstart[d0] = st; next_start[(size_t)s * D + d0] = st; }
         if (d1 < D) { dstart[d1] = st + tot0; next_start[(size_t)s * D + d1] = st + tot0; }
     }
+    if (nch < 2) return;
     __syncthreads();
     for (u32 d = t; d < D; d += 256) {
         u32 run = dstart[d];
         for (u32 k = 0; k < g; ++k) run += part[k][d];
-        u32 b = lo;
-        for (; b + 8 <= hi; b += 8) {
+        u32 j = lo;
+        for (; j + 8 <= hi; j += 8) {
             u32 v[8];
 #pragma unroll
-            for (int i = 0; i < 8; ++i) v[i] = bs[(size_t)(b + i) * D + d];
-#pragma unroll
-            for (int i = 0; i < 8; ++i) { bs[(size_t)(b + i) * D + d] = run; run += v[i]; }
-        }
-        for (; b < hi; ++b) { const u32 v = bs[(size_t)b * D + d]; bs[(size_t)b * D + d] = run; run += v; }
-    }
-}
-__global__ __launch_bounds__(256) void ss_apply_kernel(u32* __restrict__ counts, const u32* __restrict__ blk_start, u32 nseg, u32 R, u32 D,
-                                                       const u32* __restrict__ bs) {
-    const u32 b = blockIdx.x;
-    if (b >= blk_start[nseg]) return;
-    for (u32 d = threadIdx.x; d < D; d += 256) {
-        u32 run = bs[(size_t)b * D + d];
-        for (u32 r = 0; r < R; ++r) {
-            const size_t i = ((size_t)b * R + r) * D + d;
-            const u32 v = counts[i];
-            counts[i] = run;
-            run += v;
-        }
-    }
-}
-__global__ void ss_set_word_kernel(u32* p, u32 v) { *p = v; }
+            for (u32 i = 0; i < 8; ++i) v[i] = bs[end_row(j + i) * D + d];
+#pragma unroll
+            for (u32 i = 0; i < 8; ++i) { if (j + i) carry[(size_t)(c0 + j + i) * D + d] = run; run += v[i]; }
+        }
+        for (; j < hi; ++j) { if (j) carry[(size_t)(c0 + j) * D + d] = run; run += bs[end_row(j) * D + d]; }
+    }
+}
+
+template <int V>
+__global__ __launch_bounds__(256) void lo_apply_kernel(u32* __restrict__ counts, const u32* __restrict__ seg_blk, u32 nsg, const u32* __restrict__ blk_seg,
+                                                       u32 gsz, u32 R, u32 D, u32 C, const u32* __restrict__ bs, const u32* __restrict__ carry,
+                                                       const u32* __restrict__ dig_start) {
+    __shared__ u32 part[2][256 * V];
+    const u32 b = blockIdx.x, t = threadIdx.x, NT = blockDim.x;
+    if (b >= seg_blk[nsg]) return;
+    const u32 S = blk_seg[b] / gsz, b0 = seg_blk[S], clo = b / C * C;
+    const u32* basep = b0 < clo ? carry + (size_t)(b / C) * D : dig_start + (size_t)S * D;
+    const bool prev = b > (b0 > clo ? b0 : clo);
+    u32 buf = 0;
+    for (u32 col0 = 0; col0 < D; col0 += NT * V) {
+        const u32 left = (D - col0) / V;
+        const u32 W = left < NT ? left : NT, G = NT / W;
+        const u32 rg = t / W, cg = t % W;
+        const bool active = rg < G;
+        const u32 col = col0 + cg * V;
+        u32* p = counts + (size_t)b * R * D + col;
+        LoVec<V> run;
+#pragma unroll
+        for (int i = 0; i < V; ++i) run.v[i] = 0;
+        if (active) {
+#pragma unroll
+            for (int i = 0; i < V; ++i) run.v[i] = basep[col + i];
+            if (prev) { const LoVec<V> q = lo_load<V>(bs + (size_t)(b - 1) * D + col); for (int i = 0; i < V; ++i) run.v[i] += q.v[i]; }
+        }
+        const u32 need = (R + G - 1) / G;
+        const u32 K = need < LO_K ? need : LO_K;
+        for (u32 r0 = 0; r0 < R; r0 += G * K) {
+            const u32 r = r0 + rg * K;
+            LoVec<V> x[LO_K], sum;
+#pragma unroll
+            for (int i = 0; i < V; ++i) sum.v[i] = 0;
+#pragma unroll
+            for (u32 k = 0; k < LO_K; ++k) {
+                if (active && k < K && r + k < R) x[k] = lo_load<V>(p + (size_t)(r + k) * D);
+                else for (int i = 0; i < V; ++i) x[k].v[i] = 0;
+            }
+#pragma unroll
+            for (u32 k = 0; k < LO_K; ++k)
+                for (int i = 0; i < V; ++i) sum.v[i] += x[k].v[i];
+            LoVec<V> o = run;
+            if (G > 1) {
+#pragma unroll
+                for (int i = 0; i < V; ++i) part[buf][t * V + i] = sum.v[i];
+                __syncthreads();
+                for (u32 g = 0; g < G; ++g)
+                    for (int i = 0; i < V; ++i) {
+                        const u32 v = part[buf][(g * W + cg) * V + i];
+                        run.v[i] += v;
+                        if (g < rg) o.v[i] += v;
+                    }
+                buf ^= 1u;
+            } else {
+#pragma unroll
+                for (int i = 0; i < V; ++i) run.v[i] += sum.v[i];
+            }
+#pragma unroll
+            for (u32 k = 0; k < LO_K; ++k) {
+                if (active && k < K && r + k < R) {
+                    lo_store<V>(p + (size_t)(r + k) * D, o);
+                    for (int i = 0; i < V; ++i) o.v[i] += x[k].v[i];
+                }
+            }
+        }
+        if (G > 1) __syncthreads();
+    }
+}
 
 template <bool GEN, bool LAST>
 __global__ __launch_bounds__(256) __attribute__((amdgpu_waves_per_eu(4, 4))) void ss_scatter_kernel(SSLevel P, TextKeyGen g, u32 rows) {
@@ -649,29 +835,16 @@
     hipStream_t s = c.stream;
     const size_t mark = c.arena.mark();
     const u32 D = 1u << db;
-    u32* seg_start = c.arena.get<u32>(2);
-    ss_set_word_kernel<<<1, 1, 0, s>>>(seg_start, 0u);
-    LAUNCH_CHECK();
-    ss_set_word_kernel<<<1, 1, 0, s>>>(seg_start + 1, (u32)m);
-    LAUNCH_CHECK();
+    u32* seg_start = ss_first_segment(c);
+    const u32 first[2] = { 0u, (u32)m };
     u32 nseg = 1;
-    const u64 tiles = (m + SS_TILE - 1) / SS_TILE;
     for (int l = 0; l < 2; ++l) {
-        u32 R = 128;
-        while (R > 1 && (u64)nseg * R > tiles / 8 + 64) R >>= 1;
-        const u32 blocks_ub = (u32)((tiles + R - 1) / R) + nseg;
-        const u32 rows = blocks_ub * R;
         u32* nstart = c.arena.get<u32>((size_t)nseg * D + 1);
         const size_t lm = c.arena.mark();
-        u32* blk_start = c.arena.get<u32>((size_t)nseg + 1);
-        u32* blk_seg = c.arena.get<u32>(blocks_ub);
-        u32* counts = c.arena.get<u32>((size_t)rows * D);
-        u32* bs = c.arena.get<u32>((size_t)blocks_ub * D);
-        ss_nblk_kernel<<<cdiv((size_t)nseg + 1, 256), 256, 0, s>>>(seg_start, nseg, R, blk_start);
-        LAUNCH_CHECK();
-        exclusive_sum_u32(c, blk_start, blk_start, (size_t)nseg + 1, nullptr);
-        ss_blkseg_kernel<<<cdiv(nseg, 256), 256, 0, s>>>(blk_start, nseg, blk_seg);
-        LAUNCH_CHECK();
+        SegTables T;
+        ss_level_tables(c, seg_start, nseg, m, D, T, l == 0 ? first : nullptr);
+        const u32 R = T.R, rows = T.rows;
+        u32* counts = T.counts; u32* blk_start = T.blk_start; u32* blk_seg = T.blk_seg;
         PSLevel P;
         P.idx_in = l == 0 ? idx : tmp_idx; P.val_in = l == 0 ? val : tmp_val;
         P.idx_out = l == 0 ? tmp_idx : out_idx; P.val_out = l == 0 ? tmp_val : out_val;
@@ -685,17 +858,7 @@
             LAUNCH_CHECK();
             c.prof_end(pc);
         }
-        {
-            Ctx::ProfScope prof(c, K_SCAN, (u64)rows * D * 12);
-            ss_blocksum_kernel<<<blocks_ub, 256, 0, s>>>(counts, blk_start, nseg, R, D, bs);
-            LAUNCH_CHECK();
-            ss_segbase_kernel<<<nseg, 1024, 0, s>>>(bs, blk_start, seg_start, D, nstart);
-            LAUNCH_CHECK();
-            ss_set_word_kernel<<<1, 1, 0, s>>>(nstart + (size_t)nseg * D, (u32)m);
-            LAUNCH_CHECK();
-            ss_apply_kernel<<<blocks_ub, 256, 0, s>>>(counts, blk_start, nseg, R, D, bs);
-            LAUNCH_CHECK();
-        }
+        ss_level_offsets(c, T, seg_start, nseg, D, nstart, m);
         {
             const int ps = c.prof_begin(K_RS_SCATTER_U32, (u64)m * 16);
             if (db == 9) ps_scatter_kernel<9><<<grid, 256, 0, s>>>(P, rows); else ps_scatter_kernel<8><<<grid, 256, 0, s>>>(P, rows);
@@ -992,11 +1155,8 @@
     }
 
     u16* digits = c.arena.get<u16>(align_up(n, SS_TILE) + SS_TILE);
-    u32* seg_start = c.arena.get<u32>(2);
-    ss_set_word_kernel<<<1, 1, 0, s>>>(seg_start, 0u);
-    LAUNCH_CHECK();
-    ss_set_word_kernel<<<1, 1, 0, s>>>(seg_start + 1, (u32)n);
-    LAUNCH_CHECK();
+    u32* seg_start = ss_first_segment(c);
+    const u32 first[2] = { 0u, (u32)n };
     u32 nseg = 1;
     int cur = gen ? -1 : 0;
     for (int l = 0; l < L; ++l) {
@@ -1005,22 +1165,12 @@
         const u32 D = last ? 2 * F[l] : F[l];
         u32 stride = 1;
         for (int q = l + 1; q < L; ++q) stride *= F[q];
-        const u64 tiles = (n + SS_TILE - 1) / SS_TILE;
-        u32 R = 128;
-        while (R > 1 && (u64)nseg * R > tiles / 8 + 64) R >>= 1;
-        const u32 blocks_ub = (u32)((tiles + R - 1) / R) + nseg;
-        const u32 rows = blocks_ub * R;
         u32* nstart = c.arena.get<u32>((size_t)nseg * D + 1);
         const size_t lm2 = c.arena.mark();
-        u32* blk_start = c.arena.get<u32>((size_t)nseg + 1);
-        u32* blk_seg = c.arena.get<u32>(blocks_ub);
-        u32* counts = c.arena.get<u32>((size_t)rows * D);
-        u32* bs = c.arena.get<u32>((size_t)blocks_ub * D);
-        ss_nblk_kernel<<<cdiv((size_t)nseg + 1, 256), 256, 0, s>>>(seg_start, nseg, R, blk_start);
-        LAUNCH_CHECK();
-        exclusive_sum_u32(c, blk_start, blk_start, (size_t)nseg + 1, nullptr);
-        ss_blkseg_kernel<<<cdiv(nseg, 256), 256, 0, s>>>(blk_start, nseg, blk_seg);
-        LAUNCH_CHECK();
+        SegTables T;
+        ss_level_tables(c, seg_start, nseg, n, D, T, l == 0 ? first : nullptr);
+        const u32 R = T.R, rows = T.rows;
+        u32* counts = T.counts; u32* blk_start = T.blk_start; u32* blk_seg = T.blk_seg;
         SSLevel P;
         P.keys_in = cur >= 0 ? keys[cur] : nullptr; P.vals_in = cur >= 0 ? vals[cur] : nullptr;
         const int nxt = cur < 0 ? 0 : (cur ^ 1);
@@ -1039,17 +1189,7 @@
             LAUNCH_CHECK();
             c.prof_end(pc);
         }
-        {
-            Ctx::ProfScope prof(c, K_SCAN, (u64)rows * D * 12);
-            ss_blocksum_kernel<<<blocks_ub, 256, 0, s>>>(counts, blk_start, nseg, R, D, bs);
-            LAUNCH_CHECK();
-            ss_segbase_kernel<<<nseg, 1024, 0, s>>>(bs, blk_start, seg_start, D, nstart);
-            LAUNCH_CHECK();
-            ss_set_word_kernel<<<1, 1, 0, s>>>(nstart + (size_t)nseg * D, (u32)n);
-            LAUNCH_CHECK();
-            ss_apply_kernel<<<blocks_ub, 256, 0, s>>>(counts, blk_start, nseg, R, D, bs);
-            LAUNCH_CHECK();
-        }
+        ss_level_offsets(c, T, seg_start, nseg, D, nstart, n);
         {
             const int ps = c.prof_begin(K_RS_SCATTER_U64, (u64)n * (gl ? 13 : 24));
             if (gl && last) ss_scatter_stable_kernel<true, true><<<grid, 256, 0, s>>>(P, g, rows);
@@ -1123,7 +1263,7 @@
     return cur;
 }
 
-void ss_level_tables(Ctx& c, const u32* seg_start, u32 nseg, size_t n, u32 D, SegTables& T) {
+void ss_level_tables(Ctx& c, const u32* seg_start, u32 nseg, size_t n, u32 D, SegTables& T, const u32* first) {
     hipStream_t s = c.stream;
     const u64 tiles = (n + SS_TILE - 1) / SS_TILE;
     u32 R = 128;
@@ -1135,44 +1275,51 @@
     T.blk_seg = c.arena.get<u32>(T.blocks_ub);
     T.counts = c.arena.get<u32>((size_t)T.rows * D);
     T.bs = c.arena.get<u32>((size_t)T.blocks_ub * D);
+    if (first && nseg != 1) throw HipError{hipErrorUnknown, "level tables: a first segment goes with nseg = 1", (int)__LINE__};
+    if ((size_t)nseg + 1 <= LT_MAX) {
+        ss_tables_kernel<<<1, 1024, 0, s>>>(const_cast<u32*>(seg_start), nseg, R, first ? 1u : 0u, first ? first[0] : 0u, first ? first[1] : 0u,
+                                           T.blk_start, T.blk_seg);
+        LAUNCH_CHECK();
+        if (nseg >= LT_FILL) { ss_blkseg_kernel<<<cdiv(nseg, 256), 256, 0, s>>>(T.blk_start, nseg, T.blk_seg); LAUNCH_CHECK(); }
+        return;
+    }
     ss_nblk_kernel<<<cdiv((size_t)nseg + 1, 256), 256, 0, s>>>(seg_start, nseg, R, T.blk_start);
     LAUNCH_CHECK();
     exclusive_sum_u32(c, T.blk_start, T.blk_start, (size_t)nseg + 1, nullptr);
     ss_blkseg_kernel<<<cdiv(nseg, 256), 256, 0, s>>>(T.blk_start, nseg, T.blk_seg);
     LAUNCH_CHECK();
 }
+static void ss_offsets_passes(Ctx& c, const SegTables& T, const u32* seg_blk, const u32* seg_out, u32 nsg, u32 gsz, u32 D, u32* nstart, size_t n) {
+    if (D == 0 || D > LO_DMAX) throw HipError{hipErrorUnknown, "level offsets: 1 <= D <= 2048 required", (int)__LINE__};
+    hipStream_t s = c.stream;
+    const u32 C = lo_chunk_len(D), nchunks = cdiv(T.blocks_ub, C);
+    const size_t mark = c.arena.mark();
+    u32* carry = c.arena.get<u32>((size_t)nchunks * D);
+    const u64 table = (u64)T.rows * D * 4, blocks = (u64)T.blocks_ub * D * 4;
+    Ctx::ProfScope prof(c, K_SCAN, 3 * table + 4 * blocks + 3 * (u64)nchunks * D * 4);
+    const bool vec = D % 4 == 0;
+    if (vec) lo_blocksum_kernel<4><<<T.blocks_ub, 256, 0, s>>>(T.counts, seg_blk, nsg, T.R, D, T.bs);
+    else lo_blocksum_kernel<1><<<T.blocks_ub, 256, 0, s>>>(T.counts, seg_blk, nsg, T.R, D, T.bs);
+    LAUNCH_CHECK();
+    lo_chunk_kernel<<<nchunks, 256, 0, s>>>(T.bs, seg_blk, nsg, T.blk_seg, gsz, D, C);
+    LAUNCH_CHECK();
+    lo_segbase_kernel<<<nsg, (nsg >= 256 && D <= 512) ? 256 : 1024, 0, s>>>(T.bs, seg_blk, seg_out, nsg, D, C, carry, nstart, (u32)n);
+    LAUNCH_CHECK();
+    const u32 W = D / (vec ? 4 : 1);
+    const u32 nt = (T.blocks_ub >= 2048 && W >= 64) ? (W < 256 ? W / 64 * 64 : 256u) : 256u;
+    if (vec) lo_apply_kernel<4><<<T.blocks_ub, nt, 0, s>>>(T.counts, seg_blk, nsg, T.blk_seg, gsz, T.R, D, C, T.bs, carry, nstart);
+    else lo_apply_kernel<1><<<T.blocks_ub, nt, 0, s>>>(T.counts, seg_blk, nsg, T.blk_seg, gsz, T.R, D, C, T.bs, carry, nstart);
+    LAUNCH_CHECK();
+    c.arena.release(mark);
+}
 void ss_level_offsets(Ctx& c, const SegTables& T, const u32* seg_start, u32 nseg, u32 D, u32* nstart, size_t n) {
-    hipStream_t s = c.stream;
-    Ctx::ProfScope prof(c, K_SCAN, (u64)T.rows * D * 12);
-    ss_blocksum_kernel<<<T.blocks_ub, 256, 0, s>>>(T.counts, T.blk_start, nseg, T.R, D, T.bs);
-    LAUNCH_CHECK();
-    ss_segbase_kernel<<<nseg, 1024, 0, s>>>(T.bs, T.blk_start, seg_start, D, nstart);
-    LAUNCH_CHECK();
-    ss_set_word_kernel<<<1, 1, 0, s>>>(nstart + (size_t)nseg * D, (u32)n);
-    LAUNCH_CHECK();
-    ss_apply_kernel<<<T.blocks_ub, 256, 0, s>>>(T.counts, T.blk_start, nseg, T.R, D, T.bs);
-    LAUNCH_CHECK();
+    ss_offsets_passes(c, T, T.blk_start, seg_start, nseg, 1, D, nstart, n);
 }
 void ss_level_offsets_sub(Ctx& c, const SegTables& T, u32 nsub, const u32* blk_super, const u32* out_start, u32 nsuper, u32 D, u32* nstart, size_t n) {
-    hipStream_t s = c.stream;
-    Ctx::ProfScope prof(c, K_SCAN, (u64)T.rows * D * 12);
-    ss_blocksum_kernel<<<T.blocks_ub, 256, 0, s>>>(T.counts, T.blk_start, nsub, T.R, D, T.bs);
-    LAUNCH_CHECK();
-    ss_segbase_kernel<<<nsuper, 1024, 0, s>>>(T.bs, blk_super, out_start, D, nstart);
-    LAUNCH_CHECK();
-    ss_set_word_kernel<<<1, 1, 0, s>>>(nstart + (size_t)nsuper * D, (u32)n);
-    LAUNCH_CHECK();
-    ss_apply_kernel<<<T.blocks_ub, 256, 0, s>>>(T.counts, T.blk_start, nsub, T.R, D, T.bs);
-    LAUNCH_CHECK();
-}
-u32* ss_first_segment(Ctx& c, size_t n) {
-    u32* seg_start = c.arena.get<u32>(2);
-    ss_set_word_kernel<<<1, 1, 0, c.stream>>>(seg_start, 0u);
-    LAUNCH_CHECK();
-    ss_set_word_kernel<<<1, 1, 0, c.stream>>>(seg_start + 1, (u32)n);
-    LAUNCH_CHECK();
-    return seg_start;
-}
+    if (nsuper == 0 || nsub % nsuper) throw HipError{hipErrorUnknown, "level offsets: pieces do not divide into the super-segments", (int)__LINE__};
+    ss_offsets_passes(c, T, blk_super, out_start, nsuper, nsub / nsuper, D, nstart, n);
+}
+u32* ss_first_segment(Ctx& c) { return c.arena.get<u32>(2); }
 void ss_build_units(Ctx& c, const u32* leaf_start, u32 nleaf, UnitTables& U, u32 small) {
     if (small == 0) small = SS_SMALL;
     hipStream_t s = c.stream;
diff --git a/tudocomp_amd/csrc/wsort.hip b/tudocomp_amd/csrc/wsort.hip
--- a/tudocomp_amd/csrc/wsort.hip
+++ b/tudocomp_amd/csrc/wsort.hip
@@ -1375,7 +1375,8 @@
     HIP_TRY(hipMemsetAsync(flags, 0, n, s));
 
     u16* digits = pre ? pre->digits : c.arena.get<u16>(align_up(n, WS_TILE) + WS_TILE);
-    const u32* seg_start = pre ? nullptr : ss_first_segment(c, n);
+    const u32* seg_start = pre ? nullptr : ss_first_segment(c);
+    const u32 first[2] = { 0u, (u32)n };
     u32 nseg = 1;
     int cur = GEN ? -1 : 0;
     u32* Vlast = nullptr;
@@ -1463,7 +1464,7 @@
         u32* nstart = c.arena.get<u32>((size_t)nseg * D + 1);
         const size_t lm2 = c.arena.mark();
         SegTables Tb;
-        ss_level_tables(c, seg_start, nseg, n, D, Tb);
+        ss_level_tables(c, seg_start, nseg, n, D, Tb, l == 0 ? first : nullptr);
         WSLevel P;
         P.k1_in = cur >= 0 ? K1[cur] : nullptr; P.k2_in = (cur >= 0 && KW == 2) ? K2[cur] : nullptr;
         P.v_in = pre ? Vlast : (cur >= 0 ? V[cur] : nullptr);
@@ -1752,12 +1753,11 @@
     }
     const size_t len = P.chunk_off[q + 1] - off;
     const size_t mark = c.arena.mark();
-    u32* seg2 = c.arena.get<u32>(2);
-    ws_set2_kernel<<<1, 1, 0, s>>>(seg2, (u32)off, (u32)(off + len));
-    LAUNCH_CHECK();
+    u32* seg2 = ss_first_segment(c);
+    const u32 first[2] = { (u32)off, (u32)(off + len) };
     const u32 D = P.F[0];
     SegTables Tb;
-    ss_level_tables(c, seg2, 1, len, D, Tb);
+    ss_level_tables(c, seg2, 1, len, D, Tb, first);
     WSLevel Lv;
     Lv.k1_in = nullptr; Lv.k2_in = nullptr; Lv.v_in = nullptr;
     Lv.k1_out = P.K1[0]; Lv.k2_out = P.KW == 2 ? P.K2[0] : nullptr; Lv.v_out = P.V[0];
```

Result: no change. 8842 (-0.9%).
